# podtyazhki1337/3d-mask-r-cnn

Hardware: AMD Instinct MI355X
Metric: volumes/sec fwd+bwd @128³ & 256³, 1/2/4/8 MI355X; 3D ROIAlign GB/s vs HBM peak (higher is better)
Workload: dtype f32; 1 GPU; configs[1]: RPN training step, ResNet50-3D+FPN+RPN fwd+bwd+SGD + ProposalLayer(3D NMS 15000->6000), 128^3 x1 volume per GPU; size=128, batch_per_gpu=1, parallelism=dp1, anchors=523776, hip_graph=True

## Files before the change

### 3d-mask-r-cnn_amd/csrc/conv3d.hip

```cpp
#include "common.h"
#include <stdlib.h>

namespace m3d {

typedef float floatx16 __attribute__((ext_vector_type(16)));
typedef float floatx4 __attribute__((ext_vector_type(4)));

struct ConvP {
    const float* a;
    int B, H, W, D, C;
    int OH, OW, OD;
    int kh, kw, kd;
    int sy, sx, sz;
    int py, px, pz;
    int64_t M;
    int K;
    const float* w;
    int N;
    int flip;
    int64_t bsa, bsw, bsy;
    int dly = 1, dlx = 1, dlz = 1;
    int nbatch = 1;
    const float* halo = nullptr;
    int hnlo = 0, hdl = 0, hr = 0;
// ... 691 lines not shown
                            const float4 o = pf ? pre[u] : ld4(e.y + m * e.ldy + n);
                            t.x += o.x; t.y += o.y; t.z += o.z; t.w += o.w;
                        }
                        epi_bnbwd4(e, m, n, t, fy4[u], fz4[u], fbn4, fs);
                    } else if (pf) {
                        epi_store4_pre(p, e, m, n, v, pre[u]);
                    } else {
                        epi_store4(p, e, m, n, v);
                    }
                }
            }
        }
        e.y = y_next;
    }
    if constexpr (FBN) {
        if (e.fpart) {
            __syncthreads();
            float* red = Ts;
#pragma unroll
            for (int a = 0; a < 3; ++a)
#pragma unroll
                for (int q = 0; q < 4; ++q) red[tid * 12 + a * 4 + q] = fs[a][q];
            __syncthreads();
            if (tid < C4T) {
                float r[12];
#pragma unroll
                for (int k = 0; k < 12; ++k) r[k] = red[tid * 12 + k];
                for (int o = tid + C4T; o < 256; o += C4T)
#pragma unroll
                    for (int k = 0; k < 12; ++k) r[k] += red[o * 12 + k];
                const int n = n0c + tid * 4;
                const int64_t row = m0c / BM;
                if (n < p.N)
#pragma unroll
                    for (int a = 0; a < 3; ++a)
                        st4(e.fpart + ((int64_t)a * e.fprows + row) * p.N + n,
                            make_float4(r[a * 4], r[a * 4 + 1], r[a * 4 + 2], r[a * 4 + 3]));
            }
        }
    }
    if (!more) break;
    L = Ln;
    __syncthreads();
    store_tile(0);
    __syncthreads();
    }
}

struct WgOut {
    float* part;
    int64_t pstride;
    int plain;
    int store;
};

__device__ __forceinline__ void wg_put(const WgOut& o, float* C, float* P, int64_t idx, float v) {
    if (P) P[idx] = v;
    else if (o.store) C[idx] = v;
    else if (o.plain) C[idx] += v;
    else unsafeAtomicAdd(C + idx, v);
}

__global__ __launch_bounds__(256) void wg_reduce_kernel(const float* __restrict__ part, int splits,
                                                        int64_t pstride, int64_t kn, int64_t bsc,
                                                        float* __restrict__ C) {
    const int64_t i = (int64_t)blockIdx.x * 256 + threadIdx.x;
    if (i >= pstride) return;
    float s = part[i];
    for (int q = 1; q < splits; ++q) s += part[q * pstride + i];
    const int64_t b = i / kn, r = i - b * kn;
    C[b * bsc + r] += s;
}

static WgOut wg_out(int64_t& splits, int64_t nbatch, int64_t K, int64_t N) {
    WgOut o{nullptr, 0, 0, 0};
    const DetState d = det();
    if (!d.on) return o;
    const int64_t per = nbatch * K * N;
    const int64_t fit = (int64_t)(d.bytes / sizeof(float)) / per;
    if (splits <= 1 || fit < 2) {
        splits = 1;
        o.plain = 1;
        return o;
    }
    if (splits > fit) splits = fit;
    o.part = static_cast<float*>(d.scratch);
    o.pstride = per;
    return o;
}

static void wg_finish(const WgOut& o, int64_t splits, int64_t nbatch, int64_t K, int64_t N, int64_t bsc,
                      float* C, hipStream_t s) {
    if (!o.part) return;
    hipLaunchKernelGGL(wg_reduce_kernel, dim3(grid_for(o.pstride, 256)), dim3(256), 0, s, o.part, (int)splits,
                       o.pstride, K * N, nbatch > 1 ? bsc : K * N, C);
}

static hipError_t wg_settle(WgOut& o, int64_t splits, bool fresh, float* C, int64_t nbatch, int64_t K, int64_t N,
                            hipStream_t s) {
    if (!fresh) return hipSuccess;
    if (splits == 1 && !o.part) {
        o.store = 1;
        return hipSuccess;
    }
    return hipMemsetAsync(C, 0, sizeof(float) * (size_t)(nbatch * K * N), s);
}

template <int BI, int BJ, int WI, int WJ, bool AVEC, bool HALO = false>
__global__ __launch_bounds__(256, 2) void conv_wgrad_kernel(ConvP p, const float* __restrict__ dz,
                                                            float* __restrict__ dw,
                                                            int64_t m_per_split, WgOut wo) {
    constexpr int BKM = 32;
    constexpr int TI = BI / (WI * 32), TJ = BJ / (WJ * 32);
    static_assert(WI * WJ == 4, "4 waves");
    constexpr int X_SZ = BKM * BI, G_SZ = BKM * BJ;
    constexpr int XQ = AVEC ? BI / 32 : BI / 8;
    constexpr int GQ = BJ / 32;
    __shared__ __attribute__((aligned(16))) float smem[2 * (X_SZ + G_SZ)];

    const int tid = threadIdx.x, lane = tid & 63, wave = tid >> 6;
    const int wi = wave / WJ, wj = wave % WJ;
    const int64_t gxy = (int64_t)gridDim.x * gridDim.y;
    const int64_t total = gxy * gridDim.z;
    const int64_t Lb = blockIdx.x + (int64_t)gridDim.x * (blockIdx.y + (int64_t)gridDim.y * blockIdx.z);
    const int64_t xcd = Lb % 8, q8 = total / 8, r8 = total % 8;
    const int64_t Lt = (xcd < r8 ? xcd * (q8 + 1) : r8 * (q8 + 1) + (xcd - r8) * q8) + Lb / 8;
    const int bz_ = (int)(Lt / gxy), rem = (int)(Lt % gxy);
    const int k0 = (rem % gridDim.x) * BI;
    const int n0 = (rem / gridDim.x) * BJ;
    const int64_t nsplit = (p.M + m_per_split - 1) / m_per_split;
    const int64_t batch = bz_ / nsplit;
    float* const wp = wo.part ? wo.part + (bz_ % nsplit) * wo.pstride + batch * (int64_t)p.K * p.N : nullptr;
    if (batch) {
        p.a += batch * p.bsa;
        dz += batch * p.bsw;
        dw += batch * p.bsy;
    }
    const int64_t ms = (int64_t)(bz_ % nsplit) * m_per_split;
    int64_t me = ms + m_per_split;
    if (me > p.M) me = p.M;
    if (ms >= me) return;
    const int taps_kd = p.kd, taps_kwkd = p.kw * p.kd;

    constexpr int XC = AVEC ? BI / 4 : BI;
    const int xcol = tid % XC;
    const int xrow0 = tid / XC;
    constexpr int XRSTEP = 256 / XC;
    const int kcol = k0 + (AVEC ? xcol * 4 : xcol);
// ... 201 lines not shown
        return;
    }
    hipLaunchKernelGGL((conv_gemm_kernel<BM, BN, WM, WN, BT, AVEC, BK, 2>), grid, dim3(256), 0, s, p, e);
}

template <bool BT, bool AVEC>
static void dispatch_gemm(const ConvP& p, const Epi& e, hipStream_t s, int nbatch = 1) {
    if (p.N <= 32) {
        launch_gemm<128, 32, 4, 1, BT, AVEC, 32>(p, e, s, nbatch);
    } else if (p.N <= 64) {
        launch_gemm<128, 64, 4, 1, BT, AVEC, 32>(p, e, s, nbatch);
    } else {
        const int64_t blocks128 = ((p.M + 127) / 128) * ((p.N + 127) / 128) * nbatch;
        if (blocks128 < 512) launch_gemm<64, 128, 2, 2, BT, AVEC, 32>(p, e, s, nbatch);
        else launch_gemm<128, 128, 2, 2, BT, AVEC, 32>(p, e, s, nbatch);
    }
}

static int wgrad_minm_env() {
    static constexpr int v = M3D_TUNE_WGRAD_MINM;
    return v;
}

template <int BI, int BJ, int WI, int WJ, bool AVEC, bool HALO = false>
static int launch_wgrad(const ConvP& p, const float* dz, float* dw, hipStream_t s, int nbatch = 1,
                        bool fresh = false) {
    const int64_t tiles = (int64_t)((p.K + BI - 1) / BI) * ((p.N + BJ - 1) / BJ) * nbatch;
    int64_t splits = (1024 + tiles - 1) / tiles;
    int64_t minm = wgrad_minm_env() > 32 ? wgrad_minm_env() : 32;
    const int64_t max_splits = (p.M + minm - 1) / minm;
    if (splits > max_splits) splits = max_splits;
    if (splits < 1) splits = 1;
    WgOut wo = wg_out(splits, nbatch, p.K, p.N);
    int64_t mper = (p.M + splits - 1) / splits;
    mper = (mper + 31) / 32 * 32;
    splits = (p.M + mper - 1) / mper;
    const hipError_t fe = wg_settle(wo, splits, fresh, dw, nbatch, p.K, p.N, s);
    if (fe != hipSuccess) return (int)fe;
    dim3 grid((unsigned)((p.K + BI - 1) / BI), (unsigned)((p.N + BJ - 1) / BJ),
              (unsigned)(splits * nbatch));
    hipLaunchKernelGGL((conv_wgrad_kernel<BI, BJ, WI, WJ, AVEC, HALO>), grid, dim3(256), 0, s, p, dz, dw,
                       mper, wo);
    wg_finish(wo, splits, nbatch, p.K, p.N, p.bsy, dw, s);
    return 0;
}


template <int OCC>
__global__ __launch_bounds__(256, OCC) void x3_wgrad_kernel(const float* __restrict__ A,
                                                            const float* __restrict__ Bm,
                                                            float* __restrict__ C, int64_t M, int K, int N,
                                                            int64_t m_per_split, int64_t bsa, int64_t bsb,
                                                            int64_t bsc, WgOut wo) {
    constexpr int BI = 128, BJ = 128, TI = 2, TJ = 2, BKM = 32;
    constexpr int PL = 128 * BKM * 2;
    __shared__ __attribute__((aligned(16))) char smem[6 * PL];
    const int tid = threadIdx.x, lane = tid & 63, wave = tid >> 6;
    const int wi = wave >> 1, wj = wave & 1, h = lane >> 5, l32 = lane & 31;
    const int64_t gxy = (int64_t)gridDim.x * gridDim.y;
    const int64_t total = gxy * gridDim.z;
    const int64_t Lb = blockIdx.x + (int64_t)gridDim.x * (blockIdx.y + (int64_t)gridDim.y * blockIdx.z);
    const int64_t xcd = Lb % 8, q8 = total / 8, r8 = total % 8;
    const int64_t Lt = (xcd < r8 ? xcd * (q8 + 1) : r8 * (q8 + 1) + (xcd - r8) * q8) + Lb / 8;
    const int bz = (int)(Lt / gxy), rem = (int)(Lt % gxy);
    const int k0 = (rem % gridDim.x) * BI;
    const int n0 = (rem / gridDim.x) * BJ;
    const int64_t nsplit = (M + m_per_split - 1) / m_per_split;
    const int64_t batch = bz / nsplit;
    float* const wp = wo.part ? wo.part + (bz % nsplit) * wo.pstride + batch * (int64_t)K * N : nullptr;
    A += batch * bsa;
    Bm += batch * bsb;
    C += batch * bsc;
    const int64_t ms = (int64_t)(bz % nsplit) * m_per_split;
    const int64_t me = ms + m_per_split < M ? ms + m_per_split : M;
    if (ms >= me) return;
    const bool isB = __builtin_amdgcn_readfirstlane(tid) >= 128;
    const int lt = tid & 127, c4 = lt & 31, grp = lt >> 5;
    const int ld = isB ? N : K;
    const int col = (isB ? n0 : k0) + c4 * 4;
    const bool colok = col < ld;
    const __amdgpu_buffer_rsrc_t rs = make_rsrc(isB ? (const void*)Bm : (const void*)A, (uint64_t)M * ld * 4);
    char* const Pb = smem + (isB ? 3 * PL : 0);
    float4 v[8];
    auto load = [&](int64_t mb) {
#pragma unroll
        for (int r = 0; r < 8; ++r) {
            const int64_t m = mb + grp * 8 + r;
            v[r] = bload4(rs, (colok && m < me) ? (uint32_t)(m * ld + col) * 4u : M3D_OOB);
        }
    };
    auto store = [&]() {
#pragma unroll
        for (int c = 0; c < 4; ++c) {
            uint32_t hh[8], mm[8], ll[8];
#pragma unroll
            for (int r = 0; r < 8; ++r) split3(f4get(v[r], c), hh[r], mm[r], ll[r]);
            const int off = x3_off(c4 * 4 + c, grp * 8);
            *reinterpret_cast<uint4*>(Pb + off) =
                make_uint4(hh[0] | (hh[1] << 16), hh[2] | (hh[3] << 16), hh[4] | (hh[5] << 16), hh[6] | (hh[7] << 16));
            *reinterpret_cast<uint4*>(Pb + PL + off) =
                make_uint4(mm[0] | (mm[1] << 16), mm[2] | (mm[3] << 16), mm[4] | (mm[5] << 16), mm[6] | (mm[7] << 16));
            *reinterpret_cast<uint4*>(Pb + 2 * PL + off) =
                make_uint4(ll[0] | (ll[1] << 16), ll[2] | (ll[3] << 16), ll[4] | (ll[5] << 16), ll[6] | (ll[7] << 16));
        }
    };
    floatx16 acc[TI][TJ];
// ... 4 lines not shown
#pragma unroll
            for (int r = 0; r < 16; ++r) acc[i][j][r] = 0.0f;
    const char* const As = smem;
    const char* const Bs = smem + 3 * PL;
    const int nchunks = (int)((me - ms + BKM - 1) / BKM);
    load(ms);
    store();
    __syncthreads();
    for (int t = 0; t < nchunks; ++t) {
        if (t + 1 < nchunks) load(ms + (int64_t)(t + 1) * BKM);
#pragma unroll 2
        for (int s16 = 0; s16 < 2; ++s16) {
            bf16x8 af[TI][3], bfr[TJ][3];
#pragma unroll
            for (int i = 0; i < TI; ++i) {
                const int off = x3_off(wi * TI * 32 + i * 32 + l32, 16 * s16 + 8 * h);
#pragma unroll
                for (int pl = 0; pl < 3; ++pl) af[i][pl] = *reinterpret_cast<const bf16x8*>(As + pl * PL + off);
            }
#pragma unroll
            for (int j = 0; j < TJ; ++j) {
                const int off = x3_off(wj * TJ * 32 + j * 32 + l32, 16 * s16 + 8 * h);
#pragma unroll
                for (int pl = 0; pl < 3; ++pl) bfr[j][pl] = *reinterpret_cast<const bf16x8*>(Bs + pl * PL + off);
            }
            x3_mac_tiles<TI, TJ>(acc, af, bfr);
        }
        __syncthreads();
        if (t + 1 < nchunks) {
            store();
            __syncthreads();
        }
    }
#pragma unroll
    for (int i = 0; i < TI; ++i)
#pragma unroll
        for (int j = 0; j < TJ; ++j) {
            const int n = n0 + wj * TJ * 32 + j * 32 + l32;
            if (n >= N) continue;
#pragma unroll
            for (int r = 0; r < 16; ++r) {
                const int k = k0 + wi * TI * 32 + i * 32 + (r & 3) + 8 * (r >> 2) + 4 * h;
                if (k < K) wg_put(wo, C, wp, (int64_t)k * N + n, acc[i][j][r]);
            }
        }
}

template <int OCC>
__global__ __launch_bounds__(256, OCC) void x3_wgrad64_kernel(const float* __restrict__ A,
                                                              const float* __restrict__ Bm,
                                                              float* __restrict__ C, int64_t M, int K, int N,
                                                              int64_t m_per_split, int64_t bsa, int64_t bsb,
                                                              int64_t bsc, WgOut wo) {
    constexpr int TI = 2, TJ = 2, BKM = 64;
    constexpr int SUB = 64 * 64;
    constexpr int PL = 2 * SUB;
    constexpr int RED = 4 * 64 * 64 * 4;
    constexpr int SMEM = RED > 6 * PL ? RED : 6 * PL;
    __shared__ __attribute__((aligned(16))) char smem[SMEM];
    const int tid = threadIdx.x, lane = tid & 63, wave = tid >> 6, h = lane >> 5, l32 = lane & 31;
    const int64_t total = gridDim.x;
    const int64_t Lb = blockIdx.x;
    const int64_t xcd = Lb % 8, q8 = total / 8, r8 = total % 8;
    const int64_t Lt = (xcd < r8 ? xcd * (q8 + 1) : r8 * (q8 + 1) + (xcd - r8) * q8) + Lb / 8;
    const int tk = (K + 63) / 64, tiles = tk * ((N + 63) / 64);
    const int tile = (int)(Lt % tiles);
    const int k0 = (tile % tk) * 64, n0 = (tile / tk) * 64;
    const int64_t bz = Lt / tiles;
    const int64_t nsplit = (M + m_per_split - 1) / m_per_split;
    const int64_t batch = bz / nsplit;
    float* const wp = wo.part ? wo.part + (bz % nsplit) * wo.pstride + batch * (int64_t)K * N : nullptr;
    A += batch * bsa;
    Bm += batch * bsb;
    C += batch * bsc;
    const int64_t ms = (bz % nsplit) * m_per_split;
    const int64_t me = ms + m_per_split < M ? ms + m_per_split : M;
    if (ms >= me) return;
    const bool isB = __builtin_amdgcn_readfirstlane(tid) >= 128;
    const int lt = tid & 127, c4 = lt & 15, grp = lt >> 4;
    const int ld = isB ? N : K;
    const int col = (isB ? n0 : k0) + c4 * 4;
    const bool colok = col < ld;
    const __amdgpu_buffer_rsrc_t rs = make_rsrc(isB ? (const void*)Bm : (const void*)A, (uint64_t)M * ld * 4);
    char* const Pb = smem + (isB ? 3 * PL : 0);
    const int soff = (grp >> 2) * SUB;
    const int lrow = c4 * 4;
    float4 v[8];
    auto load = [&](int64_t mb) {
#pragma unroll
        for (int r = 0; r < 8; ++r) {
            const int64_t m = mb + grp * 8 + r;
            v[r] = bload4(rs, (colok && m < me) ? (uint32_t)(m * ld + col) * 4u : M3D_OOB);
        }
    };
    auto store = [&]() {
#pragma unroll
        for (int c = 0; c < 4; ++c) {
            uint32_t hh[8], mm[8], ll[8];
#pragma unroll
            for (int r = 0; r < 8; ++r) split3(f4get(v[r], c), hh[r], mm[r], ll[r]);
            const int off = soff + x3_off(lrow + c, (grp & 3) * 8);
            *reinterpret_cast<uint4*>(Pb + off) =
                make_uint4(hh[0] | (hh[1] << 16), hh[2] | (hh[3] << 16), hh[4] | (hh[5] << 16), hh[6] | (hh[7] << 16));
            *reinterpret_cast<uint4*>(Pb + PL + off) =
                make_uint4(mm[0] | (mm[1] << 16), mm[2] | (mm[3] << 16), mm[4] | (mm[5] << 16), mm[6] | (mm[7] << 16));
            *reinterpret_cast<uint4*>(Pb + 2 * PL + off) =
// ... 150 lines not shown
            if (DBG == 2 || DBG == 5) {
#pragma unroll
                for (int j = 0; j < 2; ++j)
                    acc[i][j][0] += (float)(af[0][0] ^ af[1][1] ^ af[2][2] ^ bfr[j][0][3] ^ bfr[j][1][4] ^ bfr[j][2][5]);
                continue;
            }
            x3_mac_pair(acc[i][0], acc[i][1], af[0], af[1], af[2], bfr[0][0], bfr[0][1], bfr[0][2],
                                  bfr[1][0], bfr[1][1], bfr[1][2]);
        }
    };
    float4 xa[2], xb[2], ya[2], yb[2];
    load(0, xa, xb);
    split_store(0, xa, xb);
    load(1, xa, xb);
    __syncthreads();
    for (int kt = 0; kt < nk; kt += 2) {
        load(kt + 2, ya, yb);
        __builtin_amdgcn_sched_barrier(0);
        mfma_step(kt);
        split_store((kt + 1) & 1, xa, xb);
        __syncthreads();
        load(kt + 3, xa, xb);
        __builtin_amdgcn_sched_barrier(0);
        mfma_step(kt + 1);
        split_store(kt & 1, ya, yb);
        __syncthreads();
    }
#pragma unroll
    for (int i = 0; i < 4; ++i)
#pragma unroll
        for (int j = 0; j < 2; ++j) {
            const int n = n0 + wn * 64 + j * 32 + l32;
            if (n >= N) continue;
#pragma unroll
            for (int r = 0; r < 16; ++r) {
                const int k = k0 + wk * 128 + i * 32 + (r & 3) + 8 * (r >> 2) + 4 * h;
                if (k < K) wg_put(wo, C, wp, (int64_t)k * N + n, acc[i][j][r]);
            }
        }
}

struct X3wSK {
    int64_t units = 0;
    int nk = 0, tk = 0, tn = 0;
};

template <int DBG, bool SK = false>
__global__ __launch_bounds__(512, 1) void x3_wgrad_tr_kernel(const float* __restrict__ A,
                                                             const float* __restrict__ Bm,
                                                             float* __restrict__ C, int64_t M, int K,
                                                             int N, int64_t m_per_split, int64_t bsa,
                                                             int64_t bsb, int64_t bsc, WgOut wo, X3wSK sk) {
    __shared__ __attribute__((aligned(16))) char smem[2 * W2_STAGE];
    if constexpr (SK) {
        const int64_t G = gridDim.x, L = blockIdx.x;
        const int64_t xcd = L % 8, q8 = G / 8, r8 = G % 8;
        const int64_t g = (xcd < r8 ? xcd * (q8 + 1) : r8 * (q8 + 1) + (xcd - r8) * q8) + L / 8;
        const int64_t Gg = G / sk.tn, grp = g / sk.tn;
        const int nj = (int)(g - grp * sk.tn);
        const int64_t ug = sk.units / sk.tn;
        int64_t u = grp * ug / Gg;
        const int64_t ue = (grp + 1) * ug / Gg;
        while (u < ue) {
            const int64_t t = u / sk.nk;
            const int64_t s0 = u - t * sk.nk;
            const int64_t s1 = s0 + (ue - u) < sk.nk ? s0 + (ue - u) : sk.nk;
            const int64_t batch = t / sk.tk;
            const int kt = (int)(t - batch * sk.tk);
            const int64_t me = s1 * W2_BK < M ? s1 * W2_BK : M;
            x3w_segment<DBG>(smem, A + batch * bsa, Bm + batch * bsb, C + batch * bsc, M, K, N, s0 * W2_BK, me,
                             kt * 256, nj * 256, wo, nullptr, 0);
            u += s1 - s0;
        }
        return;
    }
    const int64_t gxy = (int64_t)gridDim.x * gridDim.y;
    const int64_t total = gxy * gridDim.z;
    const int64_t Lb = blockIdx.x + (int64_t)gridDim.x * (blockIdx.y + (int64_t)gridDim.y * blockIdx.z);
    const int64_t xcd = Lb % 8, q8 = total / 8, r8 = total % 8;
    const int64_t Lt = (xcd < r8 ? xcd * (q8 + 1) : r8 * (q8 + 1) + (xcd - r8) * q8) + Lb / 8;
    const int bz = (int)(Lt / gxy), rem = (int)(Lt % gxy);
    const int k0 = (rem % gridDim.x) * 256;
    const int n0 = (rem / gridDim.x) * 256;
    const int64_t nsplit = (M + m_per_split - 1) / m_per_split;
    const int64_t batch = bz / nsplit;
    float* const wp = wo.part ? wo.part + (bz % nsplit) * wo.pstride + batch * (int64_t)K * N : nullptr;
    const int64_t ms = (int64_t)(bz % nsplit) * m_per_split;
    const int64_t me = ms + m_per_split < M ? ms + m_per_split : M;
    x3w_segment<DBG>(smem, A + batch * bsa, Bm + batch * bsb, C + batch * bsc, M, K, N, ms, me, k0, n0, wo, wp, bz);
}

static int wgrad_tr_env() {
    static constexpr int v = M3D_TUNE_X3W_TR;
    return v;
}

static int launch_wgrad_tr(const float* A, const float* Bm, float* C, int64_t M, int K, int N, int nbatch,
                           int64_t bsa, int64_t bsb, int64_t bsc, hipStream_t s, bool fresh) {
    const int64_t tiles = (int64_t)((K + 255) / 256) * ((N + 255) / 256) * nbatch;
    const int64_t cus = num_cus();
    static constexpr int64_t minm = M3D_TUNE_X3W_TR_MINM;
    if (M3D_TUNE_X3W_SK && !det().on && M >= (int64_t)M3D_TUNE_X3W_SK_MIN_STEPS * W2_BK) {
        X3wSK sk{};
        sk.nk = (int)((M + W2_BK - 1) / W2_BK);
        sk.tk = (K + 255) / 256;
        sk.tn = (N + 255) / 256;
        sk.units = tiles * sk.nk;
        const int64_t min_steps = (minm + W2_BK - 1) / W2_BK;
        int64_t G = (sk.units + min_steps - 1) / min_steps;
        if (G > cus) G = cus;
        G = G / sk.tn * sk.tn;
        if (G < sk.tn) G = sk.tn;
        WgOut wo{nullptr, 0, 0, 0};
        const hipError_t fe = wg_settle(wo, 2, fresh, C, nbatch, K, N, s);
        if (fe != hipSuccess) return (int)fe;
        hipLaunchKernelGGL((x3_wgrad_tr_kernel<0, true>), dim3((unsigned)G), dim3(512), 0, s, A, Bm, C, M, K, N,
                           (int64_t)0, bsa, bsb, bsc, wo, sk);
        return 0;
    }
    int64_t splits = (cus + tiles - 1) / tiles;
    const int64_t max_splits = (M + minm - 1) / minm;
    if (splits > max_splits) splits = max_splits;
    if (splits < 1) splits = 1;
    WgOut wo = wg_out(splits, nbatch, K, N);
    int64_t mper = (M + splits - 1) / splits;
    mper = (mper + W2_BK - 1) / W2_BK * W2_BK;
    splits = (M + mper - 1) / mper;
    const hipError_t fe = wg_settle(wo, splits, fresh, C, nbatch, K, N, s);
    if (fe != hipSuccess) return (int)fe;
    dim3 grid((unsigned)((K + 255) / 256), (unsigned)((N + 255) / 256), (unsigned)(splits * nbatch));
    hipLaunchKernelGGL(x3_wgrad_tr_kernel<0>, grid, dim3(512), 0, s, A, Bm, C, M, K, N, mper, bsa, bsb, bsc, wo,
                       X3wSK{});
    wg_finish(wo, splits, nbatch, K, N, bsc, C, s);
    return 0;
}

static int wgrad_x3_env() { return (x3_mask() >> 2) & 1; }

static int launch_wgrad_x3(const float* A, const float* Bm, float* C, int64_t M, int K, int N, int nbatch,
                           int64_t bsa, int64_t bsb, int64_t bsc, hipStream_t s, bool fresh = false) {
    if (wgrad_tr_env() && K >= 192 && N >= 192)
        return launch_wgrad_tr(A, Bm, C, M, K, N, nbatch, bsa, bsb, bsc, s, fresh);
    if (K <= 64 || N <= 64) {
        const int64_t tiles = (int64_t)((K + 63) / 64) * ((N + 63) / 64);
        int64_t splits = (1024 + tiles * nbatch - 1) / (tiles * nbatch);
        const int64_t minm = wgrad_minm_env() > 64 ? wgrad_minm_env() : 64;
        const int64_t max_splits = (M + minm - 1) / minm;
        if (splits > max_splits) splits = max_splits;
        if (splits < 1) splits = 1;
        WgOut wo = wg_out(splits, nbatch, K, N);
        int64_t mper = (M + splits - 1) / splits;
        mper = (mper + 63) / 64 * 64;
        splits = (M + mper - 1) / mper;
        const hipError_t fe = wg_settle(wo, splits, fresh, C, nbatch, K, N, s);
        if (fe != hipSuccess) return (int)fe;
        hipLaunchKernelGGL((x3_wgrad64_kernel<2>), dim3((unsigned)(tiles * splits * nbatch)), dim3(256), 0, s, A, Bm, C, M,
                           K, N, mper, bsa, bsb, bsc, wo);
        wg_finish(wo, splits, nbatch, K, N, bsc, C, s);
        return 0;
    }
    const int64_t tiles = (int64_t)((K + 127) / 128) * ((N + 127) / 128) * nbatch;
    int64_t splits = (1024 + tiles - 1) / tiles;
    const int64_t minm = wgrad_minm_env() > 32 ? wgrad_minm_env() : 32;
    const int64_t max_splits = (M + minm - 1) / minm;
    if (splits > max_splits) splits = max_splits;
    if (splits < 1) splits = 1;
    WgOut wo = wg_out(splits, nbatch, K, N);
    int64_t mper = (M + splits - 1) / splits;
    mper = (mper + 31) / 32 * 32;
    splits = (M + mper - 1) / mper;
    const hipError_t fe = wg_settle(wo, splits, fresh, C, nbatch, K, N, s);
    if (fe != hipSuccess) return (int)fe;
    dim3 grid((unsigned)((K + 127) / 128), (unsigned)((N + 127) / 128), (unsigned)(splits * nbatch));
    hipLaunchKernelGGL((x3_wgrad_kernel<2>), grid, dim3(256), 0, s, A, Bm, C, M, K, N, mper, bsa, bsb, bsc, wo);
    wg_finish(wo, splits, nbatch, K, N, bsc, C, s);
    return 0;
}

struct WinoGeom {
    int B, H, W, D, Din, pz, TY, TX, TZ;
    int64_t T;
    const float* halo;
    int hlo, hhi;
    int tz_mode;
    int xcd;
};

__device__ __forceinline__ int64_t wino_block(const WinoGeom& g) {
    const unsigned nb = gridDim.x, b = blockIdx.x;
    if (g.xcd && (nb & 7u) == 0) return (int64_t)(b & 7u) * (nb >> 3) + (b >> 3);
    return b;
}

__device__ __forceinline__ void bt4(float& a0, float& a1, float& a2, float& a3) {
    const float t0 = a0 - a2, t1 = a1 + a2, t2 = a2 - a1, t3 = a1 - a3;
    a0 = t0; a1 = t1; a2 = t2; a3 = t3;
}
__device__ __forceinline__ void g3(float g0, float g1, float g2, float* o) {
    o[0] = g0;
    o[1] = (g0 + g1 + g2) * 0.5f;
    o[2] = (g0 - g1 + g2) * 0.5f;
    o[3] = g2;
}
__device__ __forceinline__ void at4(float m0, float m1, float m2, float m3, float& o0, float& o1) {
    o0 = m0 + m1 + m2;
    o1 = m1 - m2 - m3;
}
__device__ __forceinline__ void a4(float e0, float e1, float* o) {
    o[0] = e0; o[1] = e0 + e1; o[2] = e0 - e1; o[3] = -e1;
}
__device__ __forceinline__ void gt4(float v0, float v1, float v2, float v3, float* o) {
    o[0] = v0 + (v1 + v2) * 0.5f;
    o[1] = (v1 - v2) * 0.5f;
    o[2] = (v1 + v2) * 0.5f + v3;
}

__device__ __forceinline__ void wino_st(float* p, float v) {
    __builtin_nontemporal_store(v, p);
}
__device__ __forceinline__ float wino_ld(const float* p) {
    return __builtin_nontemporal_load(p);
}

template <int NZ> struct ZT;
template <> struct ZT<2> {
    static constexpr int P = 4;
    __device__ static void bt(float* d) { bt4(d[0], d[1], d[2], d[3]); }
    __device__ static void g(const float* w, float* o) { g3(w[0], w[1], w[2], o); }
    __device__ static void at(const float* m, float* o) { at4(m[0], m[1], m[2], m[3], o[0], o[1]); }
    __device__ static void a(const float* e, float* o) { a4(e[0], e[1], o); }
    __device__ static void gt(const float* v, float* o) { gt4(v[0], v[1], v[2], v[3], o); }
};
template <> struct ZT<4> {
    static constexpr int P = 6;
    __device__ static void bt(float* d) {
        const float d0 = d[0], d1 = d[1], d2 = d[2], d3 = d[3], d4 = d[4], d5 = d[5];
        d[0] = d0 * 0.25f - d2 * 1.25f + d4;
        d[1] = -(d1 + d2) * 0.25f + d3 + d4;
// ... 2 lines not shown
        d[4] = d1 * 0.5f - d2 - d3 * 0.5f + d4;
        d[5] = d1 * 0.25f - d3 * 1.25f + d5;
    }
    __device__ static void g(const float* w, float* o) {
        const float c23 = 2.0f / 3.0f;
        o[0] = 4.0f * w[0];
        o[1] = c23 * (w[0] + w[1] + w[2]);
        o[2] = c23 * (w[0] - w[1] + w[2]);
        o[3] = -(8.0f / 3.0f) * w[0] - (4.0f / 3.0f) * w[1] - c23 * w[2];
        o[4] = -(8.0f / 3.0f) * w[0] + (4.0f / 3.0f) * w[1] - c23 * w[2];
        o[5] = w[2];
    }
    __device__ static void at(const float* m, float* o) {
        const float s12 = m[1] + m[2], d12 = m[1] - m[2], s34 = m[3] + m[4], d34 = m[3] - m[4];
        o[0] = m[0] + s12 + s34;
        o[1] = d12 + d34 * 0.5f;
        o[2] = s12 + s34 * 0.25f;
        o[3] = d12 + d34 * 0.125f + m[5];
    }
    __device__ static void a(const float* e, float* o) {
        o[0] = e[0];
        o[1] = e[0] + e[1] + e[2] + e[3];
        o[2] = e[0] - e[1] + e[2] - e[3];
        o[3] = e[0] + e[1] * 0.5f + e[2] * 0.25f + e[3] * 0.125f;
        o[4] = e[0] - e[1] * 0.5f + e[2] * 0.25f - e[3] * 0.125f;
        o[5] = e[3];
    }
    __device__ static void gt(const float* v, float* o) {
        const float c23 = 2.0f / 3.0f;
        o[0] = 4.0f * v[0] + c23 * (v[1] + v[2]) - (8.0f / 3.0f) * (v[3] + v[4]);
        o[1] = c23 * (v[1] - v[2]) - (4.0f / 3.0f) * (v[3] - v[4]);
        o[2] = c23 * (v[1] + v[2]) - c23 * (v[3] + v[4]) + v[5];
    }
};

constexpr int WNY = M3D_TUNE_WINO_NY;
using YT = ZT<WNY>;
constexpr int PY = YT::P;

__device__ __forceinline__ void tile_coords(int64_t t, const WinoGeom& g, int& b, int& ty, int& tx,
                                            int& tz) {
    tz = (int)(t % g.TZ);
    int64_t r = t / g.TZ;
    tx = (int)(r % g.TX);
    r /= g.TX;
    ty = (int)(r % g.TY);
    b = (int)(r / g.TY);
}

template <int NZ, bool X3O = false, bool HALO = false, int NYT = WNY>
__global__ __launch_bounds__(256) void wino_input_kernel(const float* __restrict__ x, WinoGeom g,
                                                         int C, float* __restrict__ U) {
    constexpr int P = ZT<NZ>::P, PYt = ZT<NYT>::P;
    const int64_t i = wino_block(g) * blockDim.x + threadIdx.x;
    if (i >= g.T * C) return;
    const int c = (int)(i % C);
    const int64_t t = i / C;
    int b, ty, tx, tz;
    tile_coords(t, g, b, ty, tx, tz);
    if (g.tz_mode) {
        const bool edge = tz == 0 || tz == g.TZ - 1;
        if ((g.tz_mode == 1) == edge) return;
    }
    float d[PYt][4][P];
    const __amdgpu_buffer_rsrc_t rs = make_rsrc(x, (uint64_t)g.B * g.H * g.W * g.Din * C * 4);
    __amdgpu_buffer_rsrc_t rh;
    if constexpr (HALO) rh = make_rsrc(g.halo, (uint64_t)g.B * g.H * g.W * 2 * C * 4);
#pragma unroll
    for (int a = 0; a < PYt; ++a) {
        const int y = NYT * ty - 1 + a;
#pragma unroll
        for (int bb = 0; bb < 4; ++bb) {
            const int xx = 2 * tx - 1 + bb;
            const bool ok = (unsigned)y < (unsigned)g.H && (unsigned)xx < (unsigned)g.W;
            const uint32_t row = (uint32_t)((((b * g.H + y) * g.W + xx) * g.Din) * C + c);
#pragma unroll
            for (int k = 0; k < P; ++k) {
                const int z = NZ * tz - g.pz + k;
                const bool in = ok && (unsigned)z < (unsigned)g.Din;
                d[a][bb][k] = __builtin_bit_cast(
                    float, __builtin_amdgcn_raw_buffer_load_b32(rs, in ? (row + (uint32_t)z * C) * 4u : M3D_OOB, 0, 0));
                if constexpr (HALO) {
                    if (k == 0 || k == P - 1) {
                        const int q = z < 0 ? 0 : 1;
                        const bool hz = ok && ((z == -1 && g.hlo) || (z == g.Din && g.hhi));
                        const uint32_t hoff = (uint32_t)((((b * g.H + y) * g.W + xx) * 2 + q) * C + c) * 4u;
                        const float hv = __builtin_bit_cast(
                            float, __builtin_amdgcn_raw_buffer_load_b32(rh, hz ? hoff : M3D_OOB, 0, 0));
                        d[a][bb][k] = hz ? hv : d[a][bb][k];
                    }
                }
            }
        }
    }
#pragma unroll
    for (int a = 0; a < PYt; ++a)
#pragma unroll
        for (int bb = 0; bb < 4; ++bb) ZT<NZ>::bt(d[a][bb]);
#pragma unroll
    for (int a = 0; a < PYt; ++a)
#pragma unroll
        for (int k = 0; k < P; ++k) bt4(d[a][0][k], d[a][1][k], d[a][2][k], d[a][3][k]);
#pragma unroll
    for (int bb = 0; bb < 4; ++bb)
#pragma unroll
        for (int k = 0; k < P; ++k) {
// ... 78 lines not shown
#pragma unroll
        for (int b = 0; b < 3; ++b) ZT<NZ>::g(gw[a][b], t1[a][b]);
    float t2[3][4][P];
#pragma unroll
    for (int a = 0; a < 3; ++a)
#pragma unroll
        for (int k = 0; k < P; ++k) {
            float o[4];
            g3(t1[a][0][k], t1[a][1][k], t1[a][2][k], o);
#pragma unroll
            for (int b = 0; b < 4; ++b) t2[a][b][k] = o[b];
        }
    if constexpr (X3O) {
        unsigned short* out = reinterpret_cast<unsigned short*>(V) + (int64_t)np_ * (KN / Np) + kp;
        const int64_t pstride = (int64_t)PYt * 4 * P * KN;
#pragma unroll
        for (int b = 0; b < 4; ++b)
#pragma unroll
            for (int k = 0; k < P; ++k) {
                float o[PYt];
                const float gy[3] = {t2[0][b][k], t2[1][b][k], t2[2][b][k]};
                ZT<NYT>::g(gy, o);
#pragma unroll
                for (int a = 0; a < PYt; ++a) {
                    uint32_t hh, mm, ll;
                    split3(o[a], hh, mm, ll);
                    unsigned short* q = out + (int64_t)((a * 4 + b) * P + k) * KN;
                    q[0] = (unsigned short)hh;
                    q[pstride] = (unsigned short)mm;
                    q[2 * pstride] = (unsigned short)ll;
                }
            }
        return;
    }
    float* out = V + (int64_t)kp * Np + np_;
#pragma unroll
    for (int b = 0; b < 4; ++b)
#pragma unroll
        for (int k = 0; k < P; ++k) {
            float o[PYt];
            const float gy[3] = {t2[0][b][k], t2[1][b][k], t2[2][b][k]};
            ZT<NYT>::g(gy, o);
#pragma unroll
            for (int a = 0; a < PYt; ++a) out[(int64_t)((a * 4 + b) * P + k) * KN] = o[a];
        }
}

template <int NZ, bool HALO, int NYT>
__device__ __forceinline__ void wino_output_body(const float* __restrict__ Mt, const WinoGeom& g,
                                                 int N, const Epi& e);
template <int NZ, int NYT = WNY>
__global__ __launch_bounds__(256) void wino_output_kernel(const float* __restrict__ Mt, WinoGeom g,
                                                          int N, Epi e) {
    wino_output_body<NZ, false, NYT>(Mt, g, N, e);
}
template <int NZ, int NYT = WNY>
__global__ __launch_bounds__(256) void wino_output_halo_kernel(const float* __restrict__ Mt, WinoGeom g,
                                                               int N, Epi e) {
    wino_output_body<NZ, true, NYT>(Mt, g, N, e);
}

template <int NZ, bool HALO, int NYT>
__device__ __forceinline__ void wino_output_body(const float* __restrict__ Mt, const WinoGeom& g,
                                                 int N, const Epi& e) {
    constexpr int P = ZT<NZ>::P, PYt = ZT<NYT>::P;
    const int64_t i = wino_block(g) * blockDim.x + threadIdx.x;
    if (i >= g.T * N) return;
    const int n = (int)(i % N);
    const int64_t t = i / N;
    int b, ty, tx, tz;
    tile_coords(t, g, b, ty, tx, tz);
    const int64_t stride = g.T * N;
    const float* src = Mt + t * N + n;
    float m[PYt][4][P];
#pragma unroll
    for (int a = 0; a < PYt; ++a)
#pragma unroll
        for (int bb = 0; bb < 4; ++bb)
#pragma unroll
            for (int k = 0; k < P; ++k) m[a][bb][k] = wino_ld(src + (int64_t)((a * 4 + bb) * P + k) * stride);
    float r1[PYt][4][NZ];
#pragma unroll
    for (int a = 0; a < PYt; ++a)
#pragma unroll
        for (int bb = 0; bb < 4; ++bb) ZT<NZ>::at(m[a][bb], r1[a][bb]);
    float r2[PYt][2][NZ];
#pragma unroll
    for (int a = 0; a < PYt; ++a)
#pragma unroll
        for (int k = 0; k < NZ; ++k)
            at4(r1[a][0][k], r1[a][1][k], r1[a][2][k], r1[a][3][k], r2[a][0][k], r2[a][1][k]);
    float o[NYT][2][NZ];
#pragma unroll
    for (int bb = 0; bb < 2; ++bb)
#pragma unroll
        for (int k = 0; k < NZ; ++k) {
            float col[PYt], oy[NYT];
#pragma unroll
            for (int a = 0; a < PYt; ++a) col[a] = r2[a][bb][k];
            ZT<NYT>::at(col, oy);
#pragma unroll
            for (int a = 0; a < NYT; ++a) o[a][bb][k] = oy[a];
        }
    const float bias = e.bias ? e.bias[n] : 0.0f;
    const float sc = e.scale ? e.scale[n] : 1.0f, sh = e.scale ? e.shift[n] : 0.0f;
#pragma unroll
// ... 98 lines not shown
                    yv[bb][k] = in[bb][k] && e.frelu ? e.fy[off] : 1.0f;
                    zv[bb][k] = in[bb][k] && e.fz ? e.fz[off] : 0.0f;
                }
#pragma unroll
            for (int bb = 0; bb < 2; ++bb)
#pragma unroll
                for (int k = 0; k < NZ; ++k) {
                    if (!in[bb][k]) continue;
                    const int64_t off = obase + (a * (int64_t)g.W + bb) * ostr + k * e.ldy;
                    float gv = o[a][bb][k];
                    if (e.accumulate) gv += ov[bb][k];
                    if (e.frelu && !(yv[bb][k] > 0.f)) gv = 0.f;
                    const float d = gv * sc;
                    sp += gv;
                    sx += gv * ((zv[bb][k] - mu) * rs);
                    sz += d;
                    e.y[off] = d;
                    if (e.fdres) e.fdres[off] = gv;
                }
        }
    }
    if (!e.fpart) return;
    if (N % 256 == 0) {
        if (valid) {
            e.fpart[(0 * e.fprows + t) * N + n] = sp;
            e.fpart[(1 * e.fprows + t) * N + n] = sx;
            e.fpart[(2 * e.fprows + t) * N + n] = sz;
        }
        return;
    }
    __shared__ float red[3][256];
    red[0][tid] = sp;
    red[1][tid] = sx;
    red[2][tid] = sz;
    __syncthreads();
    if (tid < N) {
        float a0 = 0.f, a1 = 0.f, a2 = 0.f;
        for (int q = tid; q < 256; q += N) {
            a0 += red[0][q];
            a1 += red[1][q];
            a2 += red[2][q];
        }
        const int64_t row = blockIdx.x;
        e.fpart[(0 * e.fprows + row) * N + tid] = a0;
        e.fpart[(1 * e.fprows + row) * N + tid] = a1;
        e.fpart[(2 * e.fprows + row) * N + tid] = a2;
    }
}

template <int NZ>
__global__ __launch_bounds__(256) void wino_grad_kernel(const float* __restrict__ dz, WinoGeom g,
                                                        int N, float* __restrict__ DY) {
    constexpr int P = ZT<NZ>::P;
    const int64_t i = (int64_t)blockIdx.x * blockDim.x + threadIdx.x;
    if (i >= g.T * N) return;
    const int n = (int)(i % N);
    const int64_t t = i / N;
    int b, ty, tx, tz;
    tile_coords(t, g, b, ty, tx, tz);
    float ev[WNY][2][NZ];
#pragma unroll
    for (int a = 0; a < WNY; ++a)
#pragma unroll
        for (int bb = 0; bb < 2; ++bb)
#pragma unroll
            for (int k = 0; k < NZ; ++k) {
                const int y = WNY * ty + a, xx = 2 * tx + bb, z = NZ * tz + k;
                ev[a][bb][k] = (y < g.H && xx < g.W && z < g.D)
                                   ? dz[((((int64_t)b * g.H + y) * g.W + xx) * g.D + z) * N + n]
                                   : 0.0f;
            }
    float t1[WNY][2][P];
#pragma unroll
    for (int a = 0; a < WNY; ++a)
#pragma unroll
        for (int bb = 0; bb < 2; ++bb) ZT<NZ>::a(ev[a][bb], t1[a][bb]);
    float t2[WNY][4][P];
#pragma unroll
    for (int a = 0; a < WNY; ++a)
#pragma unroll
        for (int k = 0; k < P; ++k) {
            float o[4];
            a4(t1[a][0][k], t1[a][1][k], o);
#pragma unroll
            for (int bb = 0; bb < 4; ++bb) t2[a][bb][k] = o[bb];
        }
    const int64_t stride = g.T * N;
    float* out = DY + t * N + n;
#pragma unroll
    for (int bb = 0; bb < 4; ++bb)
#pragma unroll
        for (int k = 0; k < P; ++k) {
            float ey[WNY], o[PY];
#pragma unroll
            for (int a = 0; a < WNY; ++a) ey[a] = t2[a][bb][k];
            YT::a(ey, o);
#pragma unroll
            for (int a = 0; a < PY; ++a) wino_st(out + (int64_t)((a * 4 + bb) * P + k) * stride, o[a]);
        }
}

template <int NZ>
__global__ __launch_bounds__(256) void wino_wgrad_out_kernel(const float* __restrict__ dWh, int C,
                                                             int N, float* __restrict__ dw) {
    constexpr int P = ZT<NZ>::P;
    const int64_t i = (int64_t)blockIdx.x * blockDim.x + threadIdx.x;
    const int64_t CN = (int64_t)C * N;
    if (i >= CN) return;
    float v[PY][4][P];
#pragma unroll
    for (int a = 0; a < PY; ++a)
#pragma unroll
        for (int b = 0; b < 4; ++b)
#pragma unroll
            for (int k = 0; k < P; ++k) v[a][b][k] = dWh[(int64_t)((a * 4 + b) * P + k) * CN + i];
    float t1[PY][4][3];
#pragma unroll
    for (int a = 0; a < PY; ++a)
#pragma unroll
        for (int b = 0; b < 4; ++b) ZT<NZ>::gt(v[a][b], t1[a][b]);
    float t2[PY][3][3];
#pragma unroll
    for (int a = 0; a < PY; ++a)
#pragma unroll
        for (int k = 0; k < 3; ++k) {
            float o[3];
            gt4(t1[a][0][k], t1[a][1][k], t1[a][2][k], t1[a][3][k], o);
#pragma unroll
            for (int b = 0; b < 3; ++b) t2[a][b][k] = o[b];
        }
#pragma unroll
    for (int b = 0; b < 3; ++b)
#pragma unroll
        for (int k = 0; k < 3; ++k) {
            float vy[PY], o[3];
#pragma unroll
            for (int a = 0; a < PY; ++a) vy[a] = t2[a][b][k];
            YT::gt(vy, o);
#pragma unroll
            for (int a = 0; a < 3; ++a) dw[(int64_t)((a * 3 + b) * 3 + k) * CN + i] += o[a];
        }
}

struct X3Epi {
    const float* bias = nullptr;
    const float* scale = nullptr;
    const float* shift = nullptr;
    const float* res = nullptr;
    float* z = nullptr;
    int act = 0;
    int on = 0;
    const float* fy = nullptr;
    const float* fz = nullptr;
    const float* fscale = nullptr;
    const float* fmean = nullptr;
    const float* frstd = nullptr;
    float* fdres = nullptr;
    float* fpart = nullptr;
    int64_t fprows = 0;
    int frelu = 0;
    int facc = 0;
};

struct X3G {
    const unsigned short* a = nullptr;
    const float* af = nullptr;
    const unsigned short* b = nullptr;
    float* c = nullptr;
    int64_t M = 0;
    int K = 0, N = 0, nbatch = 0;
    int64_t psa = 0, psb = 0;
    int64_t bsa = 0, bsb = 0, bsc = 0;
    X3Epi ep = {};
};

__device__ __forceinline__ int x3_off16(int row, int kc) {
    return row * 32 + (((kc ^ (row >> 3)) & 1) << 4);
}

template <int BK>
__device__ __forceinline__ int x3_soff(int row, int kc) {
    if constexpr (BK == 16) return x3_off16(row, kc);
    else return x3_off(row, kc * 8);
}

template <int BK, bool PERSIST, int OCC = (BK == 16 ? 3 : 2), bool AF32 = false, int BNT = 128>
__global__ __launch_bounds__(256, OCC) void x3_gemm_kernel(X3G g) {
    static_assert(BK == 16 || BK == 32, "BK");
    static_assert(BNT == 128 || BNT == 64, "BNT");
    constexpr int BM = 128, BN = BNT, TM = 2, TN = BNT / 64;
    constexpr int NBUF = BK == 16 ? 2 : 1;
    constexpr int KCH = BK / 8, CPT = BM * KCH / 256;
    constexpr int CPTB = BN * KCH / 256;
    constexpr int PLA = BM * BK * 2, PLB = BN * BK * 2;
    constexpr int STAGE = 3 * (PLA + PLB);
    constexpr int LDT = BN + 8, HR = 64;
    static_assert(HR * LDT * 4 <= NBUF * STAGE, "staging fits");
    __shared__ __attribute__((aligned(16))) char smem[NBUF * STAGE];
    const int tid = threadIdx.x, lane = tid & 63, wave = tid >> 6;
    const int wm = wave >> 1, wn = wave & 1, h = lane >> 5, l32 = lane & 31;
    const int64_t nbx = (g.M + BM - 1) / BM, nby = (g.N + BN - 1) / BN;
    const int64_t per_batch = nbx * nby, total = per_batch * g.nbatch;
    int64_t L = PERSIST ? (int64_t)blockIdx.x : (int64_t)blockIdx.x + (int64_t)gridDim.x * blockIdx.y;
    const int64_t Lstep = PERSIST ? (int64_t)gridDim.x : total;
    const int nk = g.K / BK;
    float* const Ts = reinterpret_cast<float*>(smem);
    int soff[CPT];
    uint32_t lrow[CPT];
#pragma unroll
    for (int u = 0; u < CPT; ++u) {
        const int c = tid + 256 * u;
        soff[u] = x3_soff<BK>(c / KCH, c % KCH);
    }
    for (; L < total; L += Lstep) {
        const int64_t xcd = L % 8, q8 = total / 8, r8 = total % 8;
        const int64_t T = (xcd < r8 ? xcd * (q8 + 1) : r8 * (q8 + 1) + (xcd - r8) * q8) + L / 8;
        const int64_t bz = T / per_batch, Tt = T - bz * per_batch;
        const int64_t m0 = (Tt / nby) * BM;
        const int n0 = (int)(Tt % nby) * BN;
        __amdgpu_buffer_rsrc_t ra[3], rb[3];
#pragma unroll
        for (int pl = 0; pl < 3; ++pl) {
            if constexpr (AF32) {
                if (pl == 0) ra[0] = make_rsrc(g.af + bz * g.bsa + m0 * g.K, (uint64_t)(g.M - m0) * g.K * 4);
            } else {
                ra[pl] = make_rsrc(g.a + pl * g.psa + bz * g.bsa + m0 * g.K, (uint64_t)(g.M - m0) * g.K * 2);
            }
            rb[pl] = make_rsrc(g.b + pl * g.psb + bz * g.bsb + (int64_t)n0 * g.K, (uint64_t)(g.N - n0) * g.K * 2);
        }
#pragma unroll
        for (int u = 0; u < CPT; ++u) {
            const int c = tid + 256 * u;
            lrow[u] = (uint32_t)((c / KCH) * g.K + (c % KCH) * 8) * 2u;
        }
        uint4 va[AF32 ? 1 : 3][CPT], vb[3][CPTB];
        float4 fa[AF32 ? CPT : 1][2];
        auto load = [&](int kt) {
#pragma unroll
            for (int q = 0; q < 3; ++q)
#pragma unroll
                for (int u = 0; u < CPT; ++u) {
                    const int off = (int)(lrow[u] + (uint32_t)kt * (BK * 2));
                    if constexpr (AF32) {
                        if (q == 0) {
                            fa[u][0] = bload4(ra[0], (uint32_t)off * 2u);
                            fa[u][1] = bload4(ra[0], (uint32_t)off * 2u + 16u);
                        }
                    } else {
                        va[q][u] = __builtin_bit_cast(uint4, __builtin_amdgcn_raw_buffer_load_b128(ra[q], off, 0, 0));
                    }
                    if (u < CPTB)
                        vb[q][u] = __builtin_bit_cast(uint4, __builtin_amdgcn_raw_buffer_load_b128(rb[q], off, 0, 0));
                }
        };
        auto store = [&](int buf) {
            char* As = smem + buf * STAGE;
            char* Bs = As + 3 * PLA;
#pragma unroll
            for (int u = 0; u < CPT; ++u) {
                if constexpr (AF32) {
                    uint2 lo4[3], hi4[3];
                    split3x4(fa[u][0], lo4);
                    split3x4(fa[u][1], hi4);
#pragma unroll
                    for (int q = 0; q < 3; ++q)
                        *reinterpret_cast<uint4*>(As + q * PLA + soff[u]) =
                            make_uint4(lo4[q].x, lo4[q].y, hi4[q].x, hi4[q].y);
                } else {
#pragma unroll
                    for (int q = 0; q < 3; ++q) *reinterpret_cast<uint4*>(As + q * PLA + soff[u]) = va[q][u];
                }
                if (u < CPTB) {
// ... 41 lines not shown
                if (kt + 1 < nk) {
                    store(0);
                    __syncthreads();
                }
            }
        }
        float* const cb = g.c + bz * g.bsc;
        for (int hf = 0; hf < 2; ++hf) {
            if (hf) __syncthreads();
            if (wm == hf) {
#pragma unroll
                for (int i = 0; i < TM; ++i)
#pragma unroll
                    for (int j = 0; j < TN; ++j)
#pragma unroll
                        for (int r = 0; r < 16; ++r)
                            Ts[(i * 32 + (r & 3) + 8 * (r >> 2) + 4 * h) * LDT + wn * TN * 32 + j * 32 + l32] =
                                acc[i][j][r];
            }
            __syncthreads();
#pragma unroll
            for (int q = 0; q < HR * (BN / 4) / 256; ++q) {
                const int idx = tid + 256 * q;
                const int row = idx / (BN / 4), c4 = idx % (BN / 4);
                const int64_t m = m0 + hf * HR + row;
                const int n = n0 + c4 * 4;
                if (m < g.M && n < g.N)
                    st4(cb + m * g.N + n, *reinterpret_cast<const float4*>(Ts + row * LDT + c4 * 4));
            }
        }
        __syncthreads();
    }
}

constexpr int G2_BK = 16;
constexpr int G2_PL = 256 * G2_BK * 2;
constexpr int G2_STAGE = 6 * G2_PL;
constexpr int G2_NST = 3;

__device__ __forceinline__ void g2_dma(__amdgpu_buffer_rsrc_t r, char* lds, uint32_t voff) {
    __builtin_amdgcn_raw_ptr_buffer_load_lds(r, (__attribute__((address_space(3))) void*)lds, 16, (int)voff,
                                             0, 0, 0);
}

template <int DBG>
__global__ __launch_bounds__(512, 1) void x3_gemm256_kernel(X3G g) {
    __shared__ __attribute__((aligned(16))) char smem[G2_NST * G2_STAGE];
    const int tid = threadIdx.x, lane = tid & 63, wave = tid >> 6;
    const int wm = wave >> 2, wn = wave & 3, h = lane >> 5, l32 = lane & 31;
    const int64_t nbx = (g.M + 255) / 256, nby = g.N / 256;
    const int64_t per_batch = nbx * nby, total = per_batch * g.nbatch;
    const int64_t L = (int64_t)blockIdx.x + (int64_t)gridDim.x * blockIdx.y;
    if (L >= total) return;
    const int64_t xcd = L % 8, q8 = total / 8, r8 = total % 8;
    const int64_t T = (xcd < r8 ? xcd * (q8 + 1) : r8 * (q8 + 1) + (xcd - r8) * q8) + L / 8;
    const int64_t bz = T / per_batch, Tt = T - bz * per_batch;
    const int64_t m0 = (Tt / nby) * 256;
    const int64_t n0 = (Tt % nby) * 256;
    __amdgpu_buffer_rsrc_t rs[6];
#pragma unroll
    for (int pl = 0; pl < 3; ++pl) {
        rs[pl] = make_rsrc(g.a + pl * g.psa + bz * g.bsa + m0 * g.K, (uint64_t)(g.M - m0) * g.K * 2);
        rs[3 + pl] = make_rsrc(g.b + pl * g.psb + bz * g.bsb + n0 * g.K, (uint64_t)256 * g.K * 2);
    }
    const int lrow = 32 * wave + (lane >> 1);
    const uint32_t lsrc = (uint32_t)lrow * (uint32_t)g.K * 2u + (uint32_t)(((lane & 1) ^ ((lrow >> 3) & 1)) << 4);
    const int nk = g.K / G2_BK;
    auto issue = [&](int kt) {
        char* S = smem + (kt % G2_NST) * G2_STAGE + wave * 1024;
        const uint32_t off = lsrc + (uint32_t)kt * (G2_BK * 2);
        if (DBG == 3) return;
#pragma unroll
        for (int pl = 0; pl < 6; ++pl) g2_dma(rs[pl], S + pl * G2_PL, off);
    };
    floatx16 acc[4][2];
#pragma unroll
    for (int i = 0; i < 4; ++i)
#pragma unroll
        for (int j = 0; j < 2; ++j)
#pragma unroll
            for (int r = 0; r < 16; ++r) acc[i][j][r] = 0.0f;
    issue(0);
    if (nk > 1) issue(1);
    for (int kt = 0; kt < nk; ++kt) {
        if (kt + 1 < nk) asm volatile("s_waitcnt vmcnt(6)" ::: "memory");
        else asm volatile("s_waitcnt vmcnt(0)" ::: "memory");
        __builtin_amdgcn_s_barrier();
        if (kt + 2 < nk) issue(kt + 2);
        const char* S = smem + (kt % G2_NST) * G2_STAGE;
        bf16x8 bfr[2][3];
#pragma unroll
        for (int j = 0; j < 2; ++j) {
            const int off = x3_off16(wn * 64 + j * 32 + l32, h);
#pragma unroll
            for (int pl = 0; pl < 3; ++pl)
                bfr[j][pl] = *reinterpret_cast<const bf16x8*>(S + (3 + pl) * G2_PL + off);
        }
#pragma unroll
        for (int i = 0; i < 4; ++i) {
            const int off = x3_off16(wm * 128 + i * 32 + l32, h);
            bf16x8 af[3];
#pragma unroll
            for (int pl = 0; pl < 3; ++pl) af[pl] = *reinterpret_cast<const bf16x8*>(S + pl * G2_PL + off);
            if (DBG == 2 || DBG == 4) {
#pragma unroll
                for (int j = 0; j < 2; ++j)
                    acc[i][j][0] += (float)(af[0][0] ^ af[1][1] ^ af[2][2] ^ bfr[j][0][3] ^ bfr[j][1][4] ^ bfr[j][2][5]);
                continue;
            }
            x3_mac_pair(acc[i][0], acc[i][1], af[0], af[1], af[2], bfr[0][0], bfr[0][1], bfr[0][2],
                                    bfr[1][0], bfr[1][1], bfr[1][2]);
// ... 4 lines not shown
#pragma unroll
        for (int i = 0; i < 4; ++i)
#pragma unroll
            for (int j = 0; j < 2; ++j)
#pragma unroll
                for (int r = 0; r < 16; ++r) t += acc[i][j][r];
        if (t == 1.2345f) g.c[0] = t;
        return;
    }
    const __amdgpu_buffer_rsrc_t rc = make_rsrc(g.c + bz * g.bsc + m0 * g.N, (uint64_t)(g.M - m0) * g.N * 4);
#pragma unroll
    for (int i = 0; i < 4; ++i)
#pragma unroll
        for (int j = 0; j < 2; ++j) {
            const int col = (int)n0 + wn * 64 + j * 32 + l32;
#pragma unroll
            for (int r = 0; r < 16; ++r) {
                const int row = wm * 128 + i * 32 + (r & 3) + 8 * (r >> 2) + 4 * h;
                const float v = acc[i][j][r];
                __builtin_amdgcn_raw_buffer_store_b32(__float_as_uint(v), rc,
                                                      (int)(((uint32_t)row * (uint32_t)g.N + (uint32_t)col) * 4u),
                                                      0, 0);
            }
        }
}

template <int N_> struct IC { static constexpr int v = N_; };
template <int EPI>
#ifndef M3D_X3AF_STAMP
#define M3D_X3AF_STAMP 0
#endif
__global__ __launch_bounds__(512, 1) void x3_gemm256_af_kernel(X3G g) {
#if M3D_X3AF_STAMP
    __shared__ __attribute__((aligned(16))) char sAll[18 * G2_PL + 256];
    uint32_t* const stampbuf = reinterpret_cast<uint32_t*>(sAll + 18 * G2_PL);
    char* const sA0 = sAll;
    char* const sA1 = sAll + 3 * G2_PL;
    char* const sA2 = sAll + 6 * G2_PL;
    char* const sB0 = sAll + 9 * G2_PL;
    char* const sB1 = sAll + 12 * G2_PL;
    char* const sB2 = sAll + 15 * G2_PL;
    const uint32_t st_t0 = (uint32_t)__builtin_amdgcn_s_memtime();
    const uint32_t st_r0 = (uint32_t)__builtin_amdgcn_s_memrealtime();
#else
    __shared__ __attribute__((aligned(16))) char sA0[3 * G2_PL], sA1[3 * G2_PL], sA2[3 * G2_PL];
    __shared__ __attribute__((aligned(16))) char sB0[3 * G2_PL], sB1[3 * G2_PL], sB2[3 * G2_PL];
#endif
    const int tid = threadIdx.x, lane = tid & 63, wave = tid >> 6;
    const int wm = wave >> 2, wn = wave & 3, h = lane >> 5, l32 = lane & 31;
    const int64_t nbx = (g.M + 255) / 256, nby = g.N / 256;
    const int64_t per_batch = nbx * nby, total = per_batch * g.nbatch;
    const int64_t L = (int64_t)blockIdx.x + (int64_t)gridDim.x * blockIdx.y;
    if (L >= total) return;
    const int64_t xcd = L % 8, q8 = total / 8, r8 = total % 8;
    const int64_t T = (xcd < r8 ? xcd * (q8 + 1) : r8 * (q8 + 1) + (xcd - r8) * q8) + L / 8;
    const int64_t bz = T / per_batch, Tt = T - bz * per_batch;
    const int64_t m0 = (Tt / nby) * 256;
    const int64_t n0 = (Tt % nby) * 256;
    const int nk = g.K / G2_BK;
    const __amdgpu_buffer_rsrc_t ra = make_rsrc(g.af + bz * g.bsa + m0 * g.K, (uint64_t)(g.M - m0) * g.K * 4);
    const int arow = tid >> 1, ach = tid & 1;
    const uint32_t aoff0 = ((uint32_t)arow * (uint32_t)g.K + (uint32_t)ach * 8u) * 4u;
    const int awr = x3_off16(arow, ach);
    __amdgpu_buffer_rsrc_t rb[3];
#pragma unroll
    for (int pl = 0; pl < 3; ++pl)
        rb[pl] = make_rsrc(g.b + pl * g.psb + bz * g.bsb + n0 * g.K, (uint64_t)256 * g.K * 2);
    const int lrow = 32 * wave + (lane >> 1);
    const uint32_t lsrc = (uint32_t)lrow * (uint32_t)g.K * 2u + (uint32_t)(((lane & 1) ^ ((lrow >> 3) & 1)) << 4);
    auto stA = [&](auto st) -> char* {
        if constexpr (decltype(st)::v == 0) return sA0;
        else if constexpr (decltype(st)::v == 1) return sA1;
        else return sA2;
    };
    auto stB = [&](auto st) -> char* {
        if constexpr (decltype(st)::v == 0) return sB0;
        else if constexpr (decltype(st)::v == 1) return sB1;
        else return sB2;
    };
    using AReg = float4;
    auto load_a = [&](int kt, float4 (&v)[2]) {
        const bool in = kt < nk;
        const uint32_t o = aoff0 + (uint32_t)kt * (G2_BK * 4);
        v[0] = bload4(ra, in ? o : M3D_OOB);
        v[1] = bload4(ra, in ? o + 16u : M3D_OOB);
    };
    auto dma_b = [&](auto st, int kt) {
        char* S = stB(st) + wave * 1024;
        const uint32_t off = kt < nk ? lsrc + (uint32_t)kt * (G2_BK * 2) : M3D_OOB;
#pragma unroll
        for (int pl = 0; pl < 3; ++pl) g2_dma(rb[pl], S + pl * G2_PL, off);
    };
    auto split_a = [&](auto st, const AReg (&v)[2]) {
        char* S = stA(st) + awr;
        uint2 lo4[3], hi4[3];
        split3x4(make_float4(v[0][0], v[0][1], v[0][2], v[0][3]), lo4);
        split3x4(make_float4(v[1][0], v[1][1], v[1][2], v[1][3]), hi4);
#pragma unroll
        for (int q = 0; q < 3; ++q)
            *reinterpret_cast<uint4*>(S + q * G2_PL) = make_uint4(lo4[q].x, lo4[q].y, hi4[q].x, hi4[q].y);
    };
    floatx16 acc[4][2];
#pragma unroll
    for (int i = 0; i < 4; ++i)
#pragma unroll
        for (int j = 0; j < 2; ++j)
#pragma unroll
            for (int r = 0; r < 16; ++r) acc[i][j][r] = 0.0f;
    AReg xa[2], ya[2], za[2];
    load_a(0, xa);
    load_a(1, ya);
// ... 1105 lines not shown
                                          int64_t OH, int64_t OW, int64_t OD, int32_t sy, int32_t sx, int32_t sz,
                                          int32_t py, int32_t px, int32_t pz, float* dw, const m3d_det_t* det, m3d_stream_t s) {
    M3D_DET_SCOPE(det);
    int rc = conv_check(B, H, W, Dl, Cin, kh, kw, kd, Cout, OH, OW, OD, sy, sx, sz);
    if (rc) return rc;
    if (B * H * W * (Dl + 2 * r) * Cin >= op_lim() || B * OH * OW * OD * Cout >= op_lim())
        return einval("conv3d_bwd_weight_halo: operand larger than 4 GiB (32-bit buffer offsets)");
    ConvP p{x, (int)B, (int)H, (int)W, (int)Dl, (int)Cin, (int)OH, (int)OW, (int)OD, kh, kw, kd,
            sy, sx, sz, py, px, pz, B * OH * OW * OD, (int)(kh * kw * kd * Cin), nullptr,
            (int)Cout, 0, 0, 0, 0};
    if ((rc = conv_halo_geom(p, halo, has_lo, has_hi, r, Dl, kd, sz, pz, OD))) return rc;
    if (stem_ok(Cin, kh, kw, kd, Cout, sy, sx, sz, 1, 1, 1, 0, 0, 0))
        return launch_stem_wgrad(p, dz, dw, st(s));
    const bool vec = (Cin % 4) == 0;
    if (Cout <= 64) {
        if (vec) launch_wgrad<128, 64, 2, 2, true, true>(p, dz, dw, st(s));
        else launch_wgrad<128, 64, 2, 2, false, true>(p, dz, dw, st(s));
    } else {
        if (vec) launch_wgrad<128, 128, 2, 2, true, true>(p, dz, dw, st(s));
        else launch_wgrad<128, 128, 2, 2, false, true>(p, dz, dw, st(s));
    }
    return check_launch("conv_wgrad_kernel<halo>");
}

static int wino_check(int64_t B, int64_t H, int64_t W, int64_t D, int64_t OD, int32_t pz,
                      int64_t Cin, int64_t Cout) {
    if (B <= 0 || H <= 0 || W <= 0 || D <= 0 || OD <= 0 || Cin <= 0 || Cout <= 0)
        return einval("conv3d winograd: tensor dimensions must be positive");
    if (Cin % 32 || Cout % 32) return einval("conv3d winograd: Cin and Cout must be multiples of 32");
    if (pz < 0 || pz > 1 || D - OD < 0 || D - OD > 2)
        return einval("conv3d winograd: z geometry must be pz in {0,1} and 0 <= D - OD <= 2");
    if (H * W * (D > OD ? D : OD) > 0x7FFFFFFF) return einval("conv3d winograd: more than 2^31 voxels");
    if (H * W * (D > OD ? D : OD) * (Cin > Cout ? Cin : Cout) >= op_lim())
        return einval("conv3d winograd: operand of one batch item larger than 4 GiB (32-bit buffer offsets)");
    return M3D_OK;
}

static bool wino_per_item(int64_t B, int64_t H, int64_t W, int64_t D, int64_t OD, int64_t Cin, int64_t Cout) {
    return per_item(B, H * W * (D > OD ? D : OD), Cin > Cout ? Cin : Cout, 0, 0);
}
#define WINO_LAUNCH_NZ(nz, kern, ...)                                            \
    do {                                                                         \
        if ((nz) == 4) hipLaunchKernelGGL(kern<4>, __VA_ARGS__);                 \
        else hipLaunchKernelGGL(kern<2>, __VA_ARGS__);                           \
    } while (0)
#define WINO_LAUNCH(kern, ...) WINO_LAUNCH_NZ(wino_nz(), kern, __VA_ARGS__)

extern "C" int32_t m3d_conv3d_wino_tile_z(void) { return wino_nz(); }
extern "C" int32_t m3d_conv3d_wino_wgrad_tile_z(void) { return wino_wgrad_nz(); }
extern "C" int32_t m3d_conv3d_wino_tile_y(void) { return WNY; }
extern "C" int32_t m3d_conv3d_wino_dgrad_tile_y(void) { return wino_dgrad_ny(); }
extern "C" int32_t m3d_conv3d_wino_dgrad_tile_z(void) { return wino_dgrad_nz(); }

extern "C" size_t m3d_conv3d_wino_workspace_bytes(int64_t B, int64_t H, int64_t W, int64_t D,
                                                  int64_t OD, int64_t Cin, int64_t Cout) {
    auto al = [](size_t b) { return (b + 255) & ~(size_t)255; };
    if (wino_per_item(B, H, W, D, OD, Cin, Cout)) B = 1;
    size_t best = 0;
    const int tiles[4][2] = {{wino_nz(), WNY}, {wino_wgrad_nz(), WNY}, {wino_dgrad_nz(), 2}, {wino_dgrad_nz(), 4}};
    for (const auto& zy : tiles) {
        const int nz = zy[0], ny = zy[1];
        const WinoGeom g = wino_geom(B, H, W, D > OD ? D : OD, D, 1, nz, ny);
        const size_t P = (size_t)wino_points(nz, ny);
        const size_t eb = gemm_x3_env() ? 6 : 4;
        const size_t wt = gemm_x3_env() ? al(sizeof(float) * 27 * (size_t)Cin * Cout) : 0;
        const size_t um1 = al(eb * P * (size_t)g.T * Cin) + al(4 * P * (size_t)g.T * Cout);
        const size_t um2 = al(eb * P * (size_t)g.T * Cout) + al(4 * P * (size_t)g.T * Cin);
        const size_t b = wt + al(eb * P * (size_t)Cin * Cout) + (um1 > um2 ? um1 : um2);
        best = b > best ? b : best;
    }
    return best;
}

struct WinoWs { float *V, *U, *M, *WT; };
static size_t wino_ws_need(const WinoGeom& g, int64_t C1, int64_t C2, int nz, int ny) {
    auto al = [](size_t b) { return (b + 255) & ~(size_t)255; };
    const size_t P = (size_t)wino_points(nz, ny);
    const size_t eb = gemm_x3_env() ? 6 : 4;
    const size_t wt = gemm_x3_env() ? al(sizeof(float) * 27 * (size_t)C1 * C2) : 0;
    return wt + al(eb * P * (size_t)C1 * C2) + al(eb * P * (size_t)g.T * C1) + al(4 * P * (size_t)g.T * C2);
}
extern "C" size_t m3d_conv3d_wino_dgrad_workspace_bytes(int64_t B, int64_t H, int64_t W, int64_t D, int64_t OD,
                                                        int64_t Cin, int64_t Cout, int32_t tile_y) {
    if (tile_y != 0 && tile_y != 2 && tile_y != 4) return 0;
    if (wino_per_item(B, H, W, D, OD, Cin, Cout)) B = 1;
    const int nz = wino_dgrad_nz(), ny = tile_y ? tile_y : wino_dgrad_ny();
    return wino_ws_need(wino_geom(B, H, W, D, OD, 1, nz, ny), Cout, Cin, nz, ny);
}
static WinoWs wino_ws(void* ws, const WinoGeom& g, int64_t Cin, int64_t Cout, int nz = -1, int ny = WNY) {
    auto al = [](size_t b) { return (b + 255) & ~(size_t)255; };
    const size_t P = (size_t)wino_points(nz < 0 ? wino_nz() : nz, ny);
    char* p = (char*)ws;
    WinoWs w{};
    w.WT = (float*)p;
    if (gemm_x3_env()) p += al(sizeof(float) * 27 * (size_t)Cin * Cout);
    const size_t eb = gemm_x3_env() ? 6 : 4;
    w.V = (float*)p; p += al(eb * P * (size_t)Cin * Cout);
    w.U = (float*)p; p += al(eb * P * (size_t)g.T * Cin);
    w.M = (float*)p;
    return w;
}

#define WINO_LAUNCH_NZ_X3(nz, kern, ...)                                         \
    do {                                                                         \
        if ((nz) == 4) hipLaunchKernelGGL((kern<4, true>), __VA_ARGS__);         \
        else hipLaunchKernelGGL((kern<2, true>), __VA_ARGS__);                   \
    } while (0)
#define WINO_INPUT(nz, x3o, grid, s, x, g, C, U)                                                          \
    do {                                                                                                   \
        const bool h_ = (g).halo != nullptr;                                                               \
        if ((nz) == 4) {                                                                                   \
            if (x3o) { if (h_) hipLaunchKernelGGL((wino_input_kernel<4, true, true>), grid, dim3(256), 0, s, x, g, C, U); \
                       else hipLaunchKernelGGL((wino_input_kernel<4, true, false>), grid, dim3(256), 0, s, x, g, C, U); } \
            else { if (h_) hipLaunchKernelGGL((wino_input_kernel<4, false, true>), grid, dim3(256), 0, s, x, g, C, U); \
                   else hipLaunchKernelGGL((wino_input_kernel<4, false, false>), grid, dim3(256), 0, s, x, g, C, U); } \
        } else {                                                                                           \
            if (x3o) { if (h_) hipLaunchKernelGGL((wino_input_kernel<2, true, true>), grid, dim3(256), 0, s, x, g, C, U); \
                       else hipLaunchKernelGGL((wino_input_kernel<2, true, false>), grid, dim3(256), 0, s, x, g, C, U); } \
            else { if (h_) hipLaunchKernelGGL((wino_input_kernel<2, false, true>), grid, dim3(256), 0, s, x, g, C, U); \
                   else hipLaunchKernelGGL((wino_input_kernel<2, false, false>), grid, dim3(256), 0, s, x, g, C, U); } \
        }                                                                                                  \
    } while (0)

static int x3_af32_env() { return (x3_mask() >> 4) & 1; }

static void wino_gemm_x3(const WinoWs& ws, int64_t T, int K, int N, int P, hipStream_t s,
                         bool af32 = false) {
    X3G q{};
    q.a = reinterpret_cast<const unsigned short*>(ws.U);
    q.af = ws.U;
    q.b = reinterpret_cast<const unsigned short*>(ws.V);
    q.c = ws.M;
    q.M = T; q.K = K; q.N = N; q.nbatch = P;
    q.psa = (int64_t)P * T * K; q.psb = (int64_t)P * K * N;
    q.bsa = T * K; q.bsb = (int64_t)K * N; q.bsc = T * N;
    if (N % 256 == 0 && T >= 256) {
        const int64_t t256 = ((T + 255) / 256) * (N / 256) * P;
        const dim3 grid((unsigned)(t256 < 65536 ? t256 : 65536), (unsigned)((t256 + 65535) / 65536));
        if (af32) hipLaunchKernelGGL(x3_gemm256_af_kernel<0>, grid, dim3(512), 0, s, q);
        else hipLaunchKernelGGL(x3_gemm256_kernel<0>, grid, dim3(512), 0, s, q);
        return;
    }
    if (N == 64) {
        const int64_t tiles = ((T + 127) / 128) * P;
        if (af32) hipLaunchKernelGGL((x3_gemm_kernel<32, false, 2, true, 64>), dim3((unsigned)tiles), dim3(256), 0, s, q);
        else hipLaunchKernelGGL((x3_gemm_kernel<32, false, 3, false, 64>), dim3((unsigned)tiles), dim3(256), 0, s, q);
        return;
    }
    const int64_t tiles = ((T + 127) / 128) * ((N + 127) / 128) * P;
    if (af32) hipLaunchKernelGGL((x3_gemm_kernel<32, false, 2, true>), dim3((unsigned)tiles), dim3(256), 0, s, q);
    else hipLaunchKernelGGL((x3_gemm_kernel<32, false, 3>), dim3((unsigned)tiles), dim3(256), 0, s, q);
}

__global__ __launch_bounds__(256) void split3_kernel(const float* __restrict__ x, int64_t n,
                                                     unsigned short* __restrict__ x3) {
    const int64_t i = (int64_t)blockIdx.x * blockDim.x + threadIdx.x;
    if (i >= n) return;
    uint32_t h, m, l;
    split3(x[i], h, m, l);
    x3[i] = (unsigned short)h;
    x3[n + i] = (unsigned short)m;
    x3[2 * n + i] = (unsigned short)l;
}

extern "C" int m3d_split3_f32(const float* x, int64_t n, uint16_t* x3, m3d_stream_t s) {
    if (n <= 0) return einval("split3: n must be positive");
    hipLaunchKernelGGL(split3_kernel, dim3(grid_for(n, 256)), dim3(256), 0, st(s), x, n,
                       reinterpret_cast<unsigned short*>(x3));
    return check_launch("split3_kernel");
}

extern "C" int m3d_gemm_x3(const uint16_t* A3, const uint16_t* B3, float* C, int64_t batch, int64_t M,
                           int64_t K, int64_t N, m3d_stream_t s) {
    if (batch <= 0 || M <= 0 || K <= 0 || N <= 0) return einval("gemm_x3: dimensions must be positive");
    if (K % 32 || N % 4) return einval("gemm_x3: K must be a multiple of 32 and N of 4");
    if (M > 0x7FFFFFFF || M * K * 2 >= 0xFFFFFFF0LL || N * K * 2 >= 0xFFFFFFF0LL || M * N * 4 >= 0xFFFFFFF0LL)
        return einval("gemm_x3: operand larger than 4 GiB (32-bit buffer offsets)");
    WinoWs ws{};
    ws.U = (float*)const_cast<uint16_t*>(A3);
    ws.V = (float*)const_cast<uint16_t*>(B3);
    ws.M = C;
// ... 232 lines not shown
        WINO_LAUNCH(wino_output_kernel, dim3(grid_for(g.T * Cout, 256)), dim3(256), 0, s, ws.M,
                    g, (int)Cout, o);
        return check_launch("conv3d winograd fwd (x3)");
    }
    if (u_keep) ws.U = u_keep;
    if (phase != 2)
        WINO_LAUNCH(wino_weight_kernel, dim3(grid_for(Cin * Cout, 256)), dim3(256), 0, s, w,
                           (int)Cin, (int)Cout, 0, ws.V);
    if (phase == 1) {
        WINO_INPUT(wino_nz(), false, dim3(grid_for(g.T * Cin, 256)), s, x, gi, (int)Cin, ws.U);
        return check_launch("conv3d winograd fwd (phase 1)");
    }
    WINO_INPUT(wino_nz(), false, dim3(grid_for(g.T * Cin, 256)), s, x, phase == 2 ? ge : g, (int)Cin, ws.U);
    ConvP p = wino_gemm_p(ws.U, g.T, (int)Cin, ws.V, (int)Cout);
    Epi e{};
    e.y = ws.M; e.ldy = Cout; e.simple = 1; e.YH = 1; e.YW = 1; e.YD = (int)g.T;
    e.ysy = e.ysx = e.ysz = 1;
    dispatch_gemm<false, true>(p, e, s, wino_points());
    Epi o{};
    o.bias = bias; o.scale = bn_scale; o.shift = bn_shift; o.res = residual;
    o.res_mode = residual ? 1 : 0; o.relu = relu; o.z = z_out; o.y = y; o.ldy = Cout;
    WINO_LAUNCH(wino_output_kernel, dim3(grid_for(g.T * Cout, 256)), dim3(256), 0, s, ws.M,
                       g, (int)Cout, o);
    return check_launch("conv3d winograd fwd");
}

extern "C" int m3d_conv3d_fwd_wino(const float* x, int64_t B, int64_t H, int64_t W, int64_t D,
                                   int64_t Cin, const float* w, int64_t Cout, int64_t OD,
                                   int32_t pz, const float* bias, const float* bn_scale,
                                   const float* bn_shift, const float* residual, int32_t relu,
                                   float* z_out, float* y, void* workspace, size_t ws_bytes,
                                   m3d_stream_t s) {
    return fwd_wino(x, B, H, W, D, Cin, w, Cout, OD, pz, bias, bn_scale, bn_shift, residual, relu,
                    z_out, y, nullptr, workspace, ws_bytes, st(s));
}

extern "C" int m3d_conv3d_fwd_wino_keep(const float* x, int64_t B, int64_t H, int64_t W, int64_t D,
                                        int64_t Cin, const float* w, int64_t Cout, int64_t OD,
                                        int32_t pz, const float* bias, const float* bn_scale,
                                        const float* bn_shift, const float* residual, int32_t relu,
                                        float* z_out, float* y, float* u_keep, void* workspace,
                                        size_t ws_bytes, m3d_stream_t s) {
    if (!u_keep) return einval("conv3d winograd: u_keep must not be NULL");
    if (wino_nz() != wino_wgrad_nz())
        return einval("conv3d winograd: forward and weight-gradient tiles differ (m3d_conv3d_wino_u_bytes == 0)");
    return fwd_wino(x, B, H, W, D, Cin, w, Cout, OD, pz, bias, bn_scale, bn_shift, residual, relu,
                    z_out, y, u_keep, workspace, ws_bytes, st(s));
}

static int bwd_data_wino(const float* dz, const float* w, int64_t B, int64_t H, int64_t W, int64_t D,
                         int64_t Cin, int64_t Cout, int64_t OD, int32_t pz, float* dx, int32_t accumulate,
                         void* workspace, size_t ws_bytes, hipStream_t s, float* dx_halo = nullptr,
                         int hlo = 0, bool v_ready = false, const Epi* fb = nullptr, int ny = 0,
                         const void* v_ext = nullptr);

extern "C" int m3d_conv3d_fwd_wino_v(const float* x, int64_t B, int64_t H, int64_t W, int64_t D, int64_t Cin,
                                     const float* w, int64_t Cout, int64_t OD, int32_t pz, const float* bias,
                                     const float* bn_scale, const float* bn_shift, const float* residual,
                                     int32_t relu, float* z_out, float* y, void* workspace, size_t ws_bytes,
                                     int32_t v_ready, m3d_stream_t s) {
    return fwd_wino(x, B, H, W, D, Cin, w, Cout, OD, pz, bias, bn_scale, bn_shift, residual, relu, z_out, y,
                    nullptr, workspace, ws_bytes, st(s), nullptr, 0, 0, v_ready != 0);
}
extern "C" int m3d_conv3d_bwd_data_wino_v(const float* dz, const float* w, int64_t B, int64_t H, int64_t W,
                                          int64_t D, int64_t Cin, int64_t Cout, int64_t OD, int32_t pz, float* dx,
                                          int32_t accumulate, void* workspace, size_t ws_bytes, int32_t v_ready,
                                          m3d_stream_t s) {
    return bwd_data_wino(dz, w, B, H, W, D, Cin, Cout, OD, pz, dx, accumulate, workspace, ws_bytes, st(s), nullptr,
                         0, v_ready != 0);
}

static int dgrad_tile_arg(int32_t tile_y, int& ny) {
    if (tile_y != 0 && tile_y != 2 && tile_y != 4) return einval("conv3d winograd bwd-data: tile_y must be 0, 2 or 4");
    ny = tile_y ? tile_y : wino_dgrad_ny();
    return M3D_OK;
}

extern "C" int m3d_conv3d_bwd_data_wino_vy(const float* dz, const float* w, int64_t B, int64_t H, int64_t W,
                                           int64_t D, int64_t Cin, int64_t Cout, int64_t OD, int32_t pz, float* dx,
                                           int32_t accumulate, void* workspace, size_t ws_bytes, int32_t v_ready,
                                           int32_t tile_y, m3d_stream_t s) {
    int ny;
    int rc = dgrad_tile_arg(tile_y, ny);
    if (rc) return rc;
    return bwd_data_wino(dz, w, B, H, W, D, Cin, Cout, OD, pz, dx, accumulate, workspace, ws_bytes, st(s), nullptr,
                         0, v_ready != 0, nullptr, ny);
}

extern "C" int m3d_conv3d_bwd_data_wino(const float* dz, const float* w, int64_t B, int64_t H,
                                        int64_t W, int64_t D, int64_t Cin, int64_t Cout,
                                        int64_t OD, int32_t pz, float* dx, int32_t accumulate,
                                        void* workspace, size_t ws_bytes, m3d_stream_t s) {
    return bwd_data_wino(dz, w, B, H, W, D, Cin, Cout, OD, pz, dx, accumulate, workspace, ws_bytes, st(s));
}

static int bwd_data_wino_bn(const float* dz, const float* w, int64_t B, int64_t H, int64_t W, int64_t D,
                            int64_t Cin, int64_t Cout, int64_t OD, int32_t pz, float* dx, int32_t accumulate,
                            void* workspace, size_t ws_bytes, int32_t v_ready, const m3d_bn_bwd_t* bn, void* bn_ws,
                            size_t bn_ws_bytes, int ny, hipStream_t hs, const void* v_ext = nullptr) {
    if (Cin % 256 != 0 && 256 % Cin != 0)
        return einval("conv3d winograd bwd-data (fused BN backward): Cin must divide 256 or be a multiple of it");
    if (wino_per_item(B, H, W, D, OD, Cin, Cout))
        return einval("conv3d winograd bwd-data (fused BN backward): batch past the 32-bit operand bound");
    const WinoGeom g = wino_geom(B, H, W, D, OD, 2 - pz, wino_dgrad_nz(), ny);
    const int64_t rows = Cin % 256 == 0 ? g.T : (g.T * Cin + 255) / 256;
    Epi e{};
    int rc = bn_fuse_epi(bn, Cin, bn_ws, bn_ws_bytes, rows, e);
// ... 42 lines not shown
}
extern "C" int m3d_conv3d_wino_weight_v(const float* w, int64_t Cin, int64_t Cout, int32_t dgrad, int32_t tile_y,
                                        void* v, size_t v_bytes, m3d_stream_t s) {
    int ny;
    if (Cin <= 0 || Cout <= 0) return einval("conv3d winograd: channel counts must be positive");
    if (int rc = wino_v_tile(dgrad, tile_y, ny)) return rc;
    if (!w || !v || v_bytes < m3d_conv3d_wino_v_bytes(Cin, Cout, dgrad, tile_y))
        return einval("conv3d winograd: transformed-weight buffer missing or too small (m3d_conv3d_wino_v_bytes)");
    const dim3 grid(grid_for(Cin * Cout, 256));
    if (!dgrad) {
        float* wt = reinterpret_cast<float*>(static_cast<char*>(v) + wino_v_planes_bytes(Cin, Cout, 0, ny));
        hipLaunchKernelGGL(x3_wt_kernel, dim3((unsigned)((Cout + 31) / 32), (unsigned)((Cin + 31) / 32), 27),
                           dim3(256), 0, st(s), w, (int)Cin, (int)Cout, wt);
        WINO_LAUNCH_NZ_X3(wino_nz(), wino_weight_kernel, grid, dim3(256), 0, st(s), wt, (int)Cin, (int)Cout, 0,
                          static_cast<float*>(v));
        return check_launch("conv3d winograd weight transform (fwd)");
    }
    const int nz = wino_dgrad_nz();
    float* V = static_cast<float*>(v);
    if (nz == 4 && ny == 4) hipLaunchKernelGGL((wino_weight_kernel<4, true, 4>), grid, dim3(256), 0, st(s), w, (int)Cin, (int)Cout, 1, V);
    else if (nz == 4) hipLaunchKernelGGL((wino_weight_kernel<4, true, 2>), grid, dim3(256), 0, st(s), w, (int)Cin, (int)Cout, 1, V);
    else if (ny == 4) hipLaunchKernelGGL((wino_weight_kernel<2, true, 4>), grid, dim3(256), 0, st(s), w, (int)Cin, (int)Cout, 1, V);
    else hipLaunchKernelGGL((wino_weight_kernel<2, true, 2>), grid, dim3(256), 0, st(s), w, (int)Cin, (int)Cout, 1, V);
    return check_launch("conv3d winograd weight transform (dgrad)");
}
extern "C" int m3d_conv3d_fwd_wino_kv(const float* x, int64_t B, int64_t H, int64_t W, int64_t D, int64_t Cin,
                                      const float* w, int64_t Cout, int64_t OD, int32_t pz, const float* bias,
                                      const float* bn_scale, const float* bn_shift, const float* residual,
                                      int32_t relu, float* z_out, float* y, float* u_keep, const void* v,
                                      void* workspace, size_t ws_bytes, m3d_stream_t s) {
    int ny;
    if (int rc = wino_v_tile(0, 0, ny)) return rc;
    if (!v) return einval("conv3d winograd: v must not be NULL (m3d_conv3d_wino_weight_v)");
    if (u_keep && wino_nz() != wino_wgrad_nz())
        return einval("conv3d winograd: forward and weight-gradient tiles differ (m3d_conv3d_wino_u_bytes == 0)");
    return fwd_wino(x, B, H, W, D, Cin, w, Cout, OD, pz, bias, bn_scale, bn_shift, residual, relu, z_out, y, u_keep,
                    workspace, ws_bytes, st(s), nullptr, 0, 0, false, 0, v);
}
extern "C" int m3d_conv3d_bwd_data_wino_xv(const float* dz, const float* w, int64_t B, int64_t H, int64_t W,
                                           int64_t D, int64_t Cin, int64_t Cout, int64_t OD, int32_t pz, float* dx,
                                           int32_t accumulate, void* workspace, size_t ws_bytes, const void* v,
                                           int32_t tile_y, const m3d_bn_bwd_t* bn, void* bn_ws, size_t bn_ws_bytes,
                                           m3d_stream_t s) {
    int ny;
    if (int rc = wino_v_tile(1, tile_y, ny)) return rc;
    if (!v) return einval("conv3d winograd bwd-data: v must not be NULL (m3d_conv3d_wino_weight_v)");
    if (bn)
        return bwd_data_wino_bn(dz, w, B, H, W, D, Cin, Cout, OD, pz, dx, accumulate, workspace, ws_bytes, 0, bn, bn_ws,
                                bn_ws_bytes, ny, st(s), v);
    return bwd_data_wino(dz, w, B, H, W, D, Cin, Cout, OD, pz, dx, accumulate, workspace, ws_bytes, st(s), nullptr, 0,
                         false, nullptr, ny, v);
}

template <int NZ, int NY>
static void wino_dgrad_out(const float* Mt, const WinoGeom& g, int C, float* dx, int accumulate,
                           float* dx_halo, int hlo, int dl, hipStream_t hs, const Epi* fb) {
    Epi o{};
    if (fb) o = *fb;
    o.y = dx; o.ldy = C; o.accumulate = accumulate;
    const dim3 grid(grid_for(g.T * C, 256));
    if (fb) {
        hipLaunchKernelGGL((wino_output_bn_kernel<NZ, NY>), grid, dim3(256), 0, hs, Mt, g, C, o);
        return;
    }
    if (dx_halo) {
        o.yh = dx_halo; o.hlo = hlo; o.dl = dl;
        hipLaunchKernelGGL((wino_output_halo_kernel<NZ, NY>), grid, dim3(256), 0, hs, Mt, g, C, o);
        return;
    }
    hipLaunchKernelGGL((wino_output_kernel<NZ, NY>), grid, dim3(256), 0, hs, Mt, g, C, o);
}

template <int NZ, int NY>
static void bwd_data_wino_launch(const float* dz, const float* w, const WinoGeom& g, const WinoWs& ws, int Cin,
                                 int Cout, float* dx, int32_t accumulate, float* dx_halo, int hlo, int dl,
                                 bool v_ready, const Epi* fb, hipStream_t hs) {
    const int P = wino_points(NZ, NY);
    const dim3 wgrid(grid_for((int64_t)Cin * Cout, 256)), igrid(grid_for(g.T * Cout, 256));
    if (gemm_x3_env()) {
        if (!v_ready)
            hipLaunchKernelGGL((wino_weight_kernel<NZ, true, NY>), wgrid, dim3(256), 0, hs, w, Cin, Cout, 1, ws.V);
        const bool af32 = x3_af32_env();
        if (af32)
            hipLaunchKernelGGL((wino_input_kernel<NZ, false, false, NY>), igrid, dim3(256), 0, hs, dz, g, Cout, ws.U);
        else
            hipLaunchKernelGGL((wino_input_kernel<NZ, true, false, NY>), igrid, dim3(256), 0, hs, dz, g, Cout, ws.U);
        wino_gemm_x3(ws, g.T, Cout, Cin, P, hs, af32);
    } else {
        hipLaunchKernelGGL((wino_weight_kernel<NZ, false, NY>), wgrid, dim3(256), 0, hs, w, Cin, Cout, 1, ws.V);
        hipLaunchKernelGGL((wino_input_kernel<NZ, false, false, NY>), igrid, dim3(256), 0, hs, dz, g, Cout, ws.U);
        ConvP p = wino_gemm_p(ws.U, g.T, Cout, ws.V, Cin);
        Epi e{};
        e.y = ws.M; e.ldy = Cin; e.simple = 1; e.YH = 1; e.YW = 1; e.YD = (int)g.T;
        e.ysy = e.ysx = e.ysz = 1;
        dispatch_gemm<false, true>(p, e, hs, P);
    }
    wino_dgrad_out<NZ, NY>(ws.M, g, Cin, dx, accumulate, dx_halo, hlo, dl, hs, fb);
}

static int bwd_data_wino(const float* dz, const float* w, int64_t B, int64_t H, int64_t W, int64_t D,
                         int64_t Cin, int64_t Cout, int64_t OD, int32_t pz, float* dx, int32_t accumulate,
                         void* workspace, size_t ws_bytes, hipStream_t hs, float* dx_halo, int hlo, bool v_ready,
                         const Epi* fb, int ny_arg, const void* v_ext) {
    int rc = wino_check(B, H, W, D, OD, pz, Cin, Cout);
    if (rc) return rc;
    if (wino_per_item(B, H, W, D, OD, Cin, Cout)) {
        const int64_t dxd = dx_halo ? OD : D;
        for (int64_t b = 0; b < B; ++b) {
            rc = bwd_data_wino(dz + b * H * W * OD * Cout, w, 1, H, W, D, Cin, Cout, OD, pz, dx + b * H * W * dxd * Cin,
                               accumulate, workspace, ws_bytes, hs,
                               dx_halo ? dx_halo + b * H * W * 2 * Cin : nullptr, hlo, v_ready || b > 0, nullptr,
                               ny_arg, v_ext);
            if (rc) return rc;
        }
        return M3D_OK;
    }
    const int nz = wino_dgrad_nz(), ny = ny_arg ? ny_arg : wino_dgrad_ny();
    const WinoGeom g = wino_geom(B, H, W, D, OD, 2 - pz, nz, ny);
    if (ws_bytes < wino_ws_need(g, Cout, Cin, nz, ny))
        return einval("conv3d winograd: workspace too small");
    WinoWs ws = wino_ws(workspace, g, Cout, Cin, nz, ny);
    if (v_ext) {
        ws.V = static_cast<float*>(const_cast<void*>(v_ext));
        v_ready = true;
    }
    const int ci = (int)Cin, co = (int)Cout, dl = (int)OD;
    if (nz == 4 && ny == 4)
        bwd_data_wino_launch<4, 4>(dz, w, g, ws, ci, co, dx, accumulate, dx_halo, hlo, dl, v_ready, fb, hs);
    else if (nz == 4)
        bwd_data_wino_launch<4, 2>(dz, w, g, ws, ci, co, dx, accumulate, dx_halo, hlo, dl, v_ready, fb, hs);
    else if (ny == 4)
        bwd_data_wino_launch<2, 4>(dz, w, g, ws, ci, co, dx, accumulate, dx_halo, hlo, dl, v_ready, fb, hs);
    else
        bwd_data_wino_launch<2, 2>(dz, w, g, ws, ci, co, dx, accumulate, dx_halo, hlo, dl, v_ready, fb, hs);
    return check_launch("conv3d winograd bwd-data");
}

static int bwd_weight_wino(const float* x, const float* u_in, const float* dz, int64_t B,
                           int64_t H, int64_t W, int64_t D, int64_t Cin, int64_t Cout, int64_t OD,
                           int32_t pz, float* dw, void* workspace, size_t ws_bytes, m3d_stream_t s,
                           const float* halo = nullptr, int hlo = 0, int hhi = 0) {
    int rc = wino_check(B, H, W, D, OD, pz, Cin, Cout);
    if (rc) return rc;
    if (ws_bytes < m3d_conv3d_wino_workspace_bytes(B, H, W, D, OD, Cin, Cout))
        return einval("conv3d winograd: workspace too small");
    if (wino_per_item(B, H, W, D, OD, Cin, Cout)) {
        if (u_in) return einval("conv3d winograd: kept U with a batch past the 32-bit operand bound");
        for (int64_t b = 0; b < B; ++b) {
            rc = bwd_weight_wino(x + b * H * W * D * Cin, nullptr, dz + b * H * W * OD * Cout, 1, H, W, D, Cin, Cout,
                                 OD, pz, dw, workspace, ws_bytes, s, halo ? halo + b * H * W * 2 * Cin : nullptr, hlo,
                                 hhi);
            if (rc) return rc;
        }
        return M3D_OK;
    }
    const int nz = wino_wgrad_nz();
    WinoGeom g = wino_geom(B, H, W, OD, D, pz, nz);
    g.halo = halo; g.hlo = hlo; g.hhi = hhi;
    WinoWs ws = wino_ws(workspace, g, Cin, Cout, nz);
    if (u_in)
        ws.U = const_cast<float*>(u_in);
    else
        WINO_INPUT(nz, false, dim3(grid_for(g.T * Cin, 256)), st(s), x, g, (int)Cin, ws.U);
        WINO_LAUNCH_NZ(nz, wino_grad_kernel, dim3(grid_for(g.T * Cout, 256)), dim3(256), 0, st(s), dz, g,
                       (int)Cout, ws.M);
    int fe = 0;
    if (wgrad_x3_env() && (Cout > 64 || Cin <= 64)) {
        fe = launch_wgrad_x3(ws.U, ws.M, ws.V, g.T, (int)Cin, (int)Cout, wino_points(nz), g.T * Cin, g.T * Cout,
                             (int64_t)Cin * Cout, st(s), true);
    } else {
        ConvP p = wino_gemm_p(ws.U, g.T, (int)Cin, nullptr, (int)Cout);
        p.bsw = g.T * Cout;
        p.bsy = (int64_t)Cin * Cout;
        if (Cout <= 64) fe = launch_wgrad<128, 64, 2, 2, true>(p, ws.M, ws.V, st(s), wino_points(nz), true);
        else fe = launch_wgrad<128, 128, 2, 2, true>(p, ws.M, ws.V, st(s), wino_points(nz), true);
    }
    if (fe) {
        set_error("memset dW_hat: %s", hipGetErrorString((hipError_t)fe));
        return M3D_EHIP;
    }
    WINO_LAUNCH_NZ(nz, wino_wgrad_out_kernel, dim3(grid_for(Cin * Cout, 256)), dim3(256), 0, st(s),
                       ws.V, (int)Cin, (int)Cout, dw);
    return check_launch("conv3d winograd bwd-weight");
}

extern "C" int m3d_conv3d_bwd_weight_wino(const float* x, const float* dz, int64_t B, int64_t H,
                                          int64_t W, int64_t D, int64_t Cin, int64_t Cout,
                                          int64_t OD, int32_t pz, float* dw, void* workspace,
                                          size_t ws_bytes, const m3d_det_t* det, m3d_stream_t s) {
    M3D_DET_SCOPE(det);
    return bwd_weight_wino(x, nullptr, dz, B, H, W, D, Cin, Cout, OD, pz, dw, workspace, ws_bytes, s);
}

static int halo_check(const void* x_halo, int32_t has_lo, int32_t has_hi) {
    if ((has_lo | has_hi) & ~1) return einval("conv3d winograd halo: has_lo / has_hi must be 0 or 1");
    if ((has_lo || has_hi) && !x_halo) return einval("conv3d winograd halo: halo planes missing");
    return M3D_OK;
}

extern "C" int m3d_conv3d_fwd_wino_halo(const float* x, const float* x_halo, int32_t has_lo, int32_t has_hi,
                                        int64_t B, int64_t H, int64_t W, int64_t Dl, int64_t Cin,
                                        const float* w, int64_t Cout, const float* bias, const float* bn_scale,
                                        const float* bn_shift, const float* residual, int32_t relu, float* z_out,
                                        float* y, float* u_keep, void* workspace, size_t ws_bytes,
                                        m3d_stream_t s) {
    int rc = halo_check(x_halo, has_lo, has_hi);
    if (rc) return rc;
    if (u_keep && wino_nz() != wino_wgrad_nz())
        return einval("conv3d winograd: forward and weight-gradient tiles differ (m3d_conv3d_wino_u_bytes == 0)");
    return fwd_wino(x, B, H, W, Dl, Cin, w, Cout, Dl, 1, bias, bn_scale, bn_shift, residual, relu, z_out, y,
                    u_keep, workspace, ws_bytes, st(s), x_halo, has_lo, has_hi);
}

extern "C" int m3d_conv3d_fwd_wino_halo_phase(const float* x, const float* x_halo, int32_t has_lo, int32_t has_hi,
                                              int64_t B, int64_t H, int64_t W, int64_t Dl, int64_t Cin,
                                              const float* w, int64_t Cout, const float* bias, const float* bn_scale,
                                              const float* bn_shift, const float* residual, int32_t relu,
                                              float* z_out, float* y, float* u_keep, void* workspace,
                                              size_t ws_bytes, int32_t phase, m3d_stream_t s) {
    if (phase != 1 && phase != 2) return einval("conv3d winograd halo: phase must be 1 or 2");
    int rc = phase == 2 ? halo_check(x_halo, has_lo, has_hi) : M3D_OK;
    if (rc) return rc;
    if (u_keep && wino_nz() != wino_wgrad_nz())
        return einval("conv3d winograd: forward and weight-gradient tiles differ (m3d_conv3d_wino_u_bytes == 0)");
    return fwd_wino(x, B, H, W, Dl, Cin, w, Cout, Dl, 1, bias, bn_scale, bn_shift, residual, relu, z_out, y,
                    u_keep, workspace, ws_bytes, st(s), phase == 2 ? x_halo : nullptr, has_lo, has_hi, false,
                    phase);
}

extern "C" int m3d_conv3d_bwd_data_wino_halo(const float* dz, const float* w, int32_t has_lo, int32_t has_hi,
                                             int64_t B, int64_t H, int64_t W, int64_t Dl, int64_t Cin,
                                             int64_t Cout, float* dx, float* dx_halo, int32_t accumulate,
                                             void* workspace, size_t ws_bytes, m3d_stream_t s) {
    int rc = halo_check(dx_halo, has_lo, has_hi);
    if (rc) return rc;
    return bwd_data_wino(dz, w, B, H, W, Dl + has_lo + has_hi, Cin, Cout, Dl, 1 - has_lo, dx, accumulate,
                         workspace, ws_bytes, st(s), (has_lo || has_hi) ? dx_halo : nullptr, has_lo);
}

extern "C" int m3d_conv3d_bwd_weight_wino_halo(const float* x, const float* x_halo, int32_t has_lo,
                                               int32_t has_hi, const float* dz, int64_t B, int64_t H, int64_t W,
                                               int64_t Dl, int64_t Cin, int64_t Cout, float* dw, void* workspace,
                                               size_t ws_bytes, const m3d_det_t* det, m3d_stream_t s) {
    M3D_DET_SCOPE(det);
    int rc = halo_check(x_halo, has_lo, has_hi);
    if (rc) return rc;
    return bwd_weight_wino(x, nullptr, dz, B, H, W, Dl, Cin, Cout, Dl, 1, dw, workspace, ws_bytes, s, x_halo,
                           has_lo, has_hi);
}

extern "C" int m3d_conv3d_bwd_weight_wino_u(const float* u, const float* dz, int64_t B, int64_t H,
                                            int64_t W, int64_t D, int64_t Cin, int64_t Cout,
                                            int64_t OD, int32_t pz, float* dw, void* workspace,
                                            size_t ws_bytes, const m3d_det_t* det, m3d_stream_t s) {
    M3D_DET_SCOPE(det);
    if (!u) return einval("conv3d winograd: u must not be NULL");
    return bwd_weight_wino(nullptr, u, dz, B, H, W, D, Cin, Cout, OD, pz, dw, workspace, ws_bytes, s);
}
```

### 3d-mask-r-cnn_amd/m3d/_lib.py

```python
from __future__ import annotations

import ctypes
import os

import torch

_HERE = os.path.dirname(os.path.abspath(__file__))
LIB_PATH = os.path.join(_HERE, os.environ.get("M3D_LIB_FILE", "libm3d.so"))

_lib = None

c_i32 = ctypes.c_int32
c_i64 = ctypes.c_int64
c_f = ctypes.c_float
c_p = ctypes.c_void_p
c_sz = ctypes.c_size_t


class Det(ctypes.Structure):
    _fields_ = [("on", ctypes.c_int32), ("scratch", ctypes.c_void_p), ("bytes", ctypes.c_size_t)]


class BnBwd(ctypes.Structure):
    _fields_ = [("y", ctypes.c_void_p), ("z", ctypes.c_void_p), ("scale", ctypes.c_void_p),
# ... 54 lines not shown
    "m3d_conv3d_fwd_wino_v": [c_p, c_i64, c_i64, c_i64, c_i64, c_i64, c_p, c_i64, c_i64, c_i32, c_p, c_p, c_p, c_p,
                              c_i32, c_p, c_p, c_p, c_sz, c_i32, c_p],
    "m3d_conv3d_bwd_data_wino_v": [c_p, c_p, c_i64, c_i64, c_i64, c_i64, c_i64, c_i64, c_i64, c_i32, c_p, c_i32, c_p,
                                   c_sz, c_i32, c_p],
    "m3d_conv3d_bwd_data_wino_vy": [c_p, c_p, c_i64, c_i64, c_i64, c_i64, c_i64, c_i64, c_i64, c_i32, c_p, c_i32,
                                    c_p, c_sz, c_i32, c_i32, c_p],
    "m3d_conv3d_bwd_data_wino_bny": [c_p, c_p, c_i64, c_i64, c_i64, c_i64, c_i64, c_i64, c_i64, c_i32, c_p, c_i32,
                                     c_p, c_sz, c_i32, c_p, c_p, c_sz, c_i32, c_p],
    "m3d_bn_bwd_fused_workspace_bytes": [c_i64, c_i64, c_i64, c_i64, c_i64],
    "m3d_conv3d_bwd_data_bn": [c_p, c_p, c_i64, c_i64, c_i64, c_i64, c_i64, c_i32, c_i32, c_i32,
                               c_i64, c_i64, c_i64, c_i64, c_i32, c_i32, c_i32, c_i32, c_i32, c_i32,
                               c_p, c_i32, c_p, c_p, c_sz, c_p],
    "m3d_conv3d_bwd_data_wino_bn": [c_p, c_p, c_i64, c_i64, c_i64, c_i64, c_i64, c_i64, c_i64, c_i32, c_p, c_i32,
                                    c_p, c_sz, c_i32, c_p, c_p, c_sz, c_p],
    "m3d_conv3d_bwd_data_splitk_bn": [c_p, c_p, c_i64, c_i64, c_i64, c_i64, c_i64, c_i64, c_p, c_i32, c_i32,
                                      c_p, c_sz, c_p, c_p, c_sz, c_p],
    "m3d_conv3d_bwd_data": [c_p, c_p, c_i64, c_i64, c_i64, c_i64, c_i64, c_i32, c_i32, c_i32,
                            c_i64, c_i64, c_i64, c_i64, c_i32, c_i32, c_i32, c_i32, c_i32, c_i32,
                            c_p, c_i32, c_p],
    "m3d_conv3d_bwd_weight": [c_p, c_p, c_i64, c_i64, c_i64, c_i64, c_i64, c_i32, c_i32, c_i32,
                              c_i64, c_i64, c_i64, c_i64, c_i32, c_i32, c_i32, c_i32, c_i32, c_i32,
                              c_p, c_p, c_p],
    "m3d_conv3d_fwd_wino_halo": [c_p, c_p, c_i32, c_i32, c_i64, c_i64, c_i64, c_i64, c_i64, c_p, c_i64, c_p, c_p,
                                 c_p, c_p, c_i32, c_p, c_p, c_p, c_p, c_sz, c_p],
    "m3d_conv3d_fwd_wino_halo_phase": [c_p, c_p, c_i32, c_i32, c_i64, c_i64, c_i64, c_i64, c_i64, c_p, c_i64, c_p,
                                       c_p, c_p, c_p, c_i32, c_p, c_p, c_p, c_p, c_sz, c_i32, c_p],
    "m3d_conv3d_bwd_data_wino_halo": [c_p, c_p, c_i32, c_i32, c_i64, c_i64, c_i64, c_i64, c_i64, c_i64, c_p,
                                      c_p, c_i32, c_p, c_sz, c_p],
    "m3d_conv3d_bwd_weight_wino_halo": [c_p, c_p, c_i32, c_i32, c_p, c_i64, c_i64, c_i64, c_i64, c_i64, c_i64,
                                        c_p, c_p, c_sz, c_p, c_p],
    "m3d_gemm_f32": [c_p, c_p, c_p, c_i64, c_i64, c_i64, c_i64, c_p, c_i32, c_i32, c_p],
    "m3d_gemm_wgrad_f32": [c_p, c_p, c_p, c_i64, c_i64, c_i64, c_i64, c_p, c_p],
    "m3d_split3_f32": [c_p, c_i64, c_p, c_p],
    "m3d_gemm_x3": [c_p, c_p, c_p, c_i64, c_i64, c_i64, c_i64, c_p],
    "m3d_gemm_x3_af": [c_p, c_p, c_p, c_i64, c_i64, c_i64, c_i64, c_p],
    "m3d_conv3d_wino_workspace_bytes": [c_i64, c_i64, c_i64, c_i64, c_i64, c_i64, c_i64],
    "m3d_conv3d_fwd_wino": [c_p, c_i64, c_i64, c_i64, c_i64, c_i64, c_p, c_i64, c_i64, c_i32, c_p,
                            c_p, c_p, c_p, c_i32, c_p, c_p, c_p, c_sz, c_p],
    "m3d_conv3d_bwd_data_wino": [c_p, c_p, c_i64, c_i64, c_i64, c_i64, c_i64, c_i64, c_i64, c_i32,
                                 c_p, c_i32, c_p, c_sz, c_p],
    "m3d_conv3d_bwd_weight_wino": [c_p, c_p, c_i64, c_i64, c_i64, c_i64, c_i64, c_i64, c_i64,
                                   c_i32, c_p, c_p, c_sz, c_p, c_p],
    "m3d_conv3d_wino_u_bytes": [c_i64, c_i64, c_i64, c_i64, c_i64],
    "m3d_conv3d_wino_tile_z": [],
    "m3d_conv3d_wino_wgrad_tile_z": [],
    "m3d_conv3d_wino_tile_y": [],
    "m3d_conv3d_wino_dgrad_workspace_bytes": [c_i64, c_i64, c_i64, c_i64, c_i64, c_i64, c_i64, c_i32],
    "m3d_conv3d_wino_dgrad_tile_y": [],
    "m3d_conv3d_wino_dgrad_tile_z": [],
    "m3d_conv3d_fwd_wino_keep": [c_p, c_i64, c_i64, c_i64, c_i64, c_i64, c_p, c_i64, c_i64, c_i32, c_p,
                                 c_p, c_p, c_p, c_i32, c_p, c_p, c_p, c_p, c_sz, c_p],
    "m3d_conv3d_bwd_weight_wino_u": [c_p, c_p, c_i64, c_i64, c_i64, c_i64, c_i64, c_i64, c_i64,
                                     c_i32, c_p, c_p, c_sz, c_p, c_p],
    "m3d_gemm_f32_ex": [c_p, c_i64, c_i64, c_p, c_i64, c_p, c_i64, c_i64, c_i64, c_i64, c_i64, c_p,
                        c_i32, c_i32, c_p],
    "m3d_splitk_reduce": [c_p, c_i32, c_i64, c_i64, c_p, c_p, c_p, c_i32, c_p, c_p],
    "m3d_conv3d_fwd_dil": [c_p, c_i64, c_i64, c_i64, c_i64, c_i64, c_p, c_i32, c_i32, c_i32, c_i64,
                           c_i64, c_i64, c_i64, c_i32, c_i32, c_i32, c_i32, c_i32, c_i32, c_i32,
                           c_i32, c_i32, c_p, c_p, c_p, c_p, c_i32, c_i32, c_p, c_p, c_i64, c_p,
                           c_i64, c_i64, c_p],
    "m3d_deconv3d_k2s2": [c_p, c_i64, c_i64, c_i64, c_i64, c_i64, c_p, c_i64, c_p, c_i32, c_p, c_p],
    "m3d_conv3d_bwd_data_dil": [c_p, c_p, c_i64, c_i64, c_i64, c_i64, c_i64, c_i32, c_i32, c_i32,
                                c_i64, c_i64, c_i64, c_i64, c_i32, c_i32, c_i32, c_i32, c_i32, c_i32,
                                c_i32, c_i32, c_i32, c_p, c_i32, c_p],
    "m3d_conv3d_bwd_weight_dil": [c_p, c_p, c_i64, c_i64, c_i64, c_i64, c_i64, c_i32, c_i32, c_i32,
                                  c_i64, c_i64, c_i64, c_i64, c_i32, c_i32, c_i32, c_i32, c_i32, c_i32,
                                  c_i32, c_i32, c_i32, c_p, c_p, c_p],
    "m3d_deconv3d_k2s2_bwd_data": [c_p, c_p, c_i64, c_i64, c_i64, c_i64, c_i64, c_i64, c_p, c_p],
    "m3d_deconv3d_k2s2_bwd_weight": [c_p, c_p, c_i64, c_i64, c_i64, c_i64, c_i64, c_i64, c_p, c_p, c_p],
    "m3d_add_f32": [c_p, c_p, c_p, c_i64, c_p],
    "m3d_mask_out_bwd_workspace_bytes": [c_i64, c_i64, c_i32],
    "m3d_mask_out_bwd": [c_p, c_p, c_p, c_p, c_i64, c_i64, c_i32, c_p, c_p, c_p, c_p, c_p, c_sz, c_p],
    "m3d_head_outputs": [c_p, c_i64, c_i64, c_i32, c_p, c_p, c_p, c_p],
    "m3d_head_outputs_bwd": [c_p, c_p, c_p, c_i64, c_i64, c_i32, c_p, c_p],
    "m3d_max_norm": [c_p, c_i64, c_i64, c_f, c_p],
    "m3d_refine_detections": [c_p, c_p, c_p, c_i64, c_i32, c_p, c_p, c_f, c_p, c_p, c_p, c_p],
    "m3d_detections_gather": [c_p, c_p, c_p, c_p, c_i32, c_p, c_p, c_p],
    "m3d_detection_targets_workspace_bytes": [c_i64],
    "m3d_detection_targets": [c_p, c_i64, c_p, c_p, c_i64, c_i32, c_f, c_f, c_f, c_p, c_i32, ctypes.c_uint32,
                              c_p, c_p, c_p, c_p, c_p, c_p, c_p, c_p, c_sz, c_p],
    "m3d_rpn_targets_workspace_bytes": [c_i64, c_i64, c_i64],
    "m3d_rpn_targets": [c_p, c_i64, c_p, c_i64, c_f, c_f, c_i32, c_f, c_i32, c_i32, c_p, ctypes.c_uint32, c_p,
                        c_p, c_i64, c_p, c_sz, c_p, c_p],
    "m3d_rpn_targets_async": [c_p, c_i64, c_p, c_i64, c_f, c_f, c_i32, c_f, c_i32, c_i32, c_p, ctypes.c_uint32,
                              c_p, c_p, c_i64, c_p, c_sz, c_p, c_p],
    "m3d_rpn_loss_workspace_bytes": [c_i64],
    "m3d_rpn_loss_fwd": [c_p, c_p, c_p, c_p, c_p, c_i64, c_i64, c_f, c_f, c_i64, c_i64, c_f, c_f, c_p, c_p, c_p,
                         c_p, c_p, c_p, c_p, c_sz, c_p],
    "m3d_rpn_loss_bwd": [c_p, c_p, c_i64, c_p, c_p, c_p],
    "m3d_head_loss_workspace_bytes": [c_i64, c_i64],
    "m3d_head_loss_fwd": [c_p, c_p, c_p, c_p, c_p, c_p, c_p, c_i64, c_i64, c_i64, c_i64, c_f, c_f, c_f, c_f, c_f,
                          c_p, c_p, c_p, c_p, c_p, c_p, c_sz, c_p],
    "m3d_head_loss_bwd": [c_p, c_p, c_p, c_p, c_p, c_p, c_p, c_i64, c_i64, c_i64, c_i64, c_f, c_f, c_p, c_p, c_p,
                          c_p, c_p, c_p],
    "m3d_unmold_prepare": [c_p, c_p, c_i64, c_i64, c_i64, c_i64, c_i64, c_i64, c_p, c_p, c_p, c_p, c_p],
    "m3d_unmold_overlaps": [c_p, c_p, c_p, c_p, c_i64, c_i64, c_i64, c_i64, c_i64, c_p, c_i64, c_p, c_p, c_p],
    "m3d_unmold_finalize": [c_p, c_p, c_i64, c_i64, c_p, c_p, c_p, c_p, c_p],
    "m3d_unmold_paste": [c_p, c_p, c_p, c_p, c_i64, c_i64, c_i64, c_i64, c_i64, c_p, c_p, c_p],
    "m3d_mask_areas": [c_p, c_i64, c_i64, c_i64, c_i64, c_p, c_p],
    "m3d_unmold_labels": [c_p, c_p, c_p, c_p, c_p, c_i64, c_i64, c_i64, c_i64, c_i64, c_p, c_p, c_p],
    "m3d_label_pixelwise": [c_p, c_p, c_i64, c_i64, c_i64, c_i64, c_p, c_p],
    "m3d_labels_stack": [c_p, c_i64, c_i64, c_i64, c_i64, c_p, c_p],
    "m3d_normalize_image_workspace_bytes": [c_i64, c_i64, c_i64, c_i32],
    "m3d_normalize_image": [c_p, c_i32, c_i64, c_i64, c_i64, c_i32, c_p, c_p, c_p, c_sz, c_p],
    "m3d_augment_image_workspace_bytes": [c_i64, c_i64, c_i64],
    "m3d_augment_image": [c_p, c_i64, c_i64, c_i64, c_i32, c_f, ctypes.c_double, ctypes.c_uint32, ctypes.c_uint32,
                          c_p, c_p, c_sz, c_p],
    "m3d_flip_masks_u8": [c_p, c_i64, c_i64, c_i64, c_i64, c_i32, c_p, c_p],
    "m3d_flip_boxes": [c_p, c_i64, c_i64, c_i64, c_i64, c_i32, c_p, c_p],
    "m3d_maxpool3d_fwd": [c_p, c_i64, c_i64, c_i64, c_i64, c_i64, c_i32, c_i32, c_i32, c_i32,
                          c_i32, c_i32, c_i32, c_i32, c_i32, c_i64, c_i64, c_i64, c_p, c_p, c_p],
    "m3d_maxpool3d_bwd": [c_p, c_p, c_i64, c_i64, c_i64, c_i64, c_i64, c_i32, c_i32, c_i32, c_i32,
                          c_i32, c_i32, c_i32, c_i32, c_i32, c_i64, c_i64, c_i64, c_p, c_p],
    "m3d_conv3d_fwd_halo": [c_p, c_p, c_i32, c_i32, c_i32, c_i64, c_i64, c_i64, c_i64, c_i64, c_p, c_i32, c_i32,
                            c_i32, c_i64, c_i64, c_i64, c_i64, c_i32, c_i32, c_i32, c_i32, c_i32, c_i32, c_p, c_p,
                            c_p, c_i32, c_p, c_p, c_p],
    "m3d_conv3d_bwd_weight_halo": [c_p, c_p, c_i32, c_i32, c_i32, c_p, c_i64, c_i64, c_i64, c_i64, c_i64, c_i32,
                                   c_i32, c_i32, c_i64, c_i64, c_i64, c_i64, c_i32, c_i32, c_i32, c_i32, c_i32,
                                   c_i32, c_p, c_p, c_p],
    "m3d_maxpool3d_fwd_halo": [c_p, c_p, c_i32, c_i32, c_i32, c_i64, c_i64, c_i64, c_i64, c_i64, c_i32, c_i32,
                               c_i32, c_i32, c_i32, c_i32, c_i32, c_i32, c_i32, c_i64, c_i64, c_i64, c_p, c_p,
                               c_p],
    "m3d_maxpool3d_bwd_halo": [c_p, c_p, c_i32, c_i32, c_i32, c_i64, c_i64, c_i64, c_i64, c_i64, c_i32, c_i32,
                               c_i32, c_i32, c_i32, c_i32, c_i32, c_i32, c_i32, c_i64, c_i64, c_i64, c_p, c_p,
                               c_p],
    "m3d_upsample221_bwd": [c_p, c_i64, c_i64, c_i64, c_i64, c_i64, c_p, c_i32, c_p],
    "m3d_subsample221_fwd": [c_p, c_i64, c_i64, c_i64, c_i64, c_i64, c_p, c_p],
    "m3d_subsample221_bwd": [c_p, c_i64, c_i64, c_i64, c_i64, c_i64, c_p, c_p],
    "m3d_bn_affine": [c_p, c_p, c_p, c_p, c_f, c_i64, c_p, c_p, c_p, c_p],
    "m3d_bn_affine_batched": [c_p, c_i32, c_i64, c_p],
    "m3d_bn_act_bwd_workspace_bytes": [c_i64, c_i64],
    "m3d_bn_act_bwd": [c_p, c_p, c_p, c_i64, c_i64, c_i32, c_p, c_p, c_p, c_p, c_p, c_i32, c_p,
                       c_p, c_p, c_p, c_sz, c_p],
    "m3d_bn_train_few_rows_max": [],
    "m3d_bn_train_workspace_bytes": [c_i64, c_i64],
    "m3d_bn_train_fwd": [c_p, c_i64, c_i64, c_p, c_p, c_f, c_f, c_i32, c_p, c_p, c_p, c_p, c_p, c_p, c_sz, c_p],
    "m3d_bn_train_bwd": [c_p, c_p, c_p, c_i64, c_i64, c_p, c_p, c_p, c_i32, c_p, c_p, c_p, c_p, c_sz, c_p],
    "m3d_col_sums_batched_workspace_bytes": [c_p, c_i32],
    "m3d_col_sums_batched": [c_p, c_i32, c_p, c_sz, c_p],
    "m3d_sgd_keras": [c_p, c_p, c_p, c_i64, c_p, c_p, c_i32, c_f, c_f, c_f, c_p, c_p, c_p],
    "m3d_adam_keras": [c_p, c_p, c_p, c_p, c_p, c_i64, c_p, c_p, c_i32, c_f, c_f, c_f, c_f, c_f, c_p,
                       c_p, c_p],
    "m3d_adadelta_keras": [c_p, c_p, c_p, c_p, c_i64, c_p, c_p, c_i32, c_f, c_f, c_f, c_f, c_p, c_p, c_p],
    "m3d_fork_event_create": [c_i32, ctypes.POINTER(c_p)],
    "m3d_fork_event_destroy": [c_p],
    "m3d_stream_fork": [c_p, c_p, c_p],
}
_RESTYPES = {"m3d_last_error": ctypes.c_char_p, "m3d_nms3d_workspace_bytes": c_sz,
             "m3d_topk_workspace_bytes": c_sz,
             "m3d_pyramid_roi_align3d_fwd_workspace_bytes": c_sz,
             "m3d_detection_targets_workspace_bytes": c_sz, "m3d_rpn_targets_workspace_bytes": c_sz,
             "m3d_rpn_loss_workspace_bytes": c_sz, "m3d_head_loss_workspace_bytes": c_sz,
             "m3d_bn_act_bwd_workspace_bytes": c_sz, "m3d_bn_bwd_fused_workspace_bytes": c_sz, "m3d_conv3d_splitk_count": c_i32, "m3d_conv3d_wino_workspace_bytes": c_sz, "m3d_conv3d_wino_dgrad_workspace_bytes": c_sz, "m3d_conv3d_wino_v_bytes": c_sz,
             "m3d_conv3d_wino_u_bytes": c_sz, "m3d_conv3d_wino_tile_z": c_i32, "m3d_conv3d_wino_wgrad_tile_z": c_i32,
             "m3d_conv3d_wino_tile_y": c_i32, "m3d_conv3d_wino_dgrad_tile_y": c_i32,
             "m3d_conv3d_wino_dgrad_tile_z": c_i32, "m3d_col_sums_batched_workspace_bytes": c_sz,
             "m3d_bn_train_few_rows_max": c_i64, "m3d_bn_train_workspace_bytes": c_sz,
             "m3d_mask_out_bwd_workspace_bytes": c_sz, "m3d_normalize_image_workspace_bytes": c_sz,
             "m3d_augment_image_workspace_bytes": c_sz}

EXPORTED = tuple(_SIGS)


class M3DError(RuntimeError):
    pass


def load(path: str = LIB_PATH):
    global _lib
    if _lib is not None:
        return _lib
    if not os.path.exists(path):
        raise M3DError(
            f"libm3d.so not found at {path}: build it with `make -C 3d-mask-r-cnn_amd` "
            "(or __graft_entry__.build()); there is no CPU fallback")
    lib = ctypes.CDLL(path)
    for name, args in _SIGS.items():
        fn = getattr(lib, name)
        fn.argtypes = args
        fn.restype = _RESTYPES.get(name, ctypes.c_int)
    _lib = _Lib(lib)
    return _lib


DET_ENTRY_POINTS = ("m3d_conv3d_bwd_weight", "m3d_conv3d_bwd_weight_halo", "m3d_conv3d_bwd_weight_wino",
                    "m3d_conv3d_bwd_weight_wino_u", "m3d_conv3d_bwd_weight_wino_halo", "m3d_gemm_wgrad_f32",
                    "m3d_conv3d_bwd_weight_dil", "m3d_deconv3d_k2s2_bwd_weight",
                    "m3d_sgd_keras", "m3d_adam_keras", "m3d_adadelta_keras")


class BnAffineItem(ctypes.Structure):
    _fields_ = [("gamma", ctypes.c_void_p), ("beta", ctypes.c_void_p), ("mean", ctypes.c_void_p),
                ("var", ctypes.c_void_p), ("out", ctypes.c_void_p), ("eps", ctypes.c_float),
                ("C", ctypes.c_int32)]


class X3PlanesItem(ctypes.Structure):
    _fields_ = [("w", ctypes.c_void_p), ("fwd", ctypes.c_void_p), ("bwd", ctypes.c_void_p),
                ("cin", ctypes.c_int32), ("cout", ctypes.c_int32)]


class ColSumsItem(ctypes.Structure):
    _fields_ = [("x", ctypes.c_void_p), ("M", ctypes.c_int64), ("C", ctypes.c_int64), ("out", ctypes.c_void_p)]


COL_SUMS_MAX = 16


class _Lib:

    def __init__(self, cdll):
        self._cdll = cdll
        for name in _SIGS:
            setattr(self, name, getattr(cdll, name))
        for name in DET_ENTRY_POINTS:
            fn = getattr(cdll, name)
            n = len(fn.argtypes)

            def call(*args, _fn=fn, _n=n):
                if len(args) == _n - 1:
                    args = args[:-1] + (det_arg(),) + args[-1:]
                return _fn(*args)
            setattr(self, name, call)

    def __getattr__(self, name):
        return getattr(self._cdll, name)


def check(rc: int, what: str = "") -> None:
    if rc == 0:
        return
    msg = load().m3d_last_error().decode()
    if rc == -1:
        raise ValueError(msg)
    raise M3DError(f"{what}: {msg}")


def ptr(t) -> int:
    if t is None:
# ... 38 lines not shown
```

### 3d-mask-r-cnn_amd/m3d/nn.py

```python
from __future__ import annotations

import contextlib
import ctypes
import os
import weakref
from dataclasses import dataclass

import torch

from . import _lib, slab
from ._lib import check, ptr, stream


LAYER_LOG = None
LAYER_TIMING = False


RELU_CAPTURE = None


GRAD_HOOK = None


WGRAD_STREAM = True
# ... 78 lines not shown
        if side is not None:
            _fork(torch.cuda.current_stream(), side)
            with torch.cuda.stream(side):
                h[0].done(h[1])
        else:
            h[0].done(h[1])


def _span():
    if LAYER_LOG is None or not LAYER_TIMING:
        return None
    e = torch.cuda.Event(enable_timing=True)
    e.record()
    return e


def _log(kind, direct_flops, exec_flops, nbytes, phase="fwd", name="", t0=None, engine="f32"):
    if LAYER_LOG is not None:
        t1 = None
        if t0 is not None:
            t1 = torch.cuda.Event(enable_timing=True)
            t1.record()
        LAYER_LOG.append((kind, float(direct_flops), float(exec_flops), float(nbytes), phase, name, t0, t1,
                          engine))


WGRAD1_STRIDED_X3 = True


def _wgrad1_x3(geo, cin, cout, in_sp):
    return (geo.k == (1, 1, 1) and geo.stride == (1, 1, 1) and geo.pad == (0, 0, 0)
            and tuple(geo.out) == tuple(in_sp) and cin % 4 == 0 and cout >= 65)


def _wino_exec(B, OH, OW, OD, cin, cout, nz, ny=None):
    if ny is None:
        ny = int(_L().m3d_conv3d_wino_tile_y())
    tiles = B * -(-OH // ny) * -(-OW // 2) * -(-OD // nz)
    return 2.0 * (ny + 2) * 4 * (nz + 2) * tiles * cin * cout


def _L():
    return _lib.load()


SLAB_HALO_PLANES = True

SLAB_OVERLAP = True

CONV1_X3 = True
SPLITK = True
WINO_KEEP_MAX_BYTES = 8 * 2**30
SHARE_WINO_MAX_BYTES = 6 * 2**30

WINOGRAD = True
WINO_MIN_C = 64
WINO_WGRAD_MIN_C = 64


WINO_DGRAD_Y4 = "res2a_branch2b+res2b_branch2b+res2c_branch2b"


def _dgrad_tile_y(name):
    if not WINO_DGRAD_Y4:
        return 0
    return 4 if WINO_DGRAD_Y4 == "*" or name in WINO_DGRAD_Y4.split("+") else 0


def use_winograd(geo, cin, cout, in_sp):
    return (WINOGRAD and geo.k == (3, 3, 3) and geo.stride == (1, 1, 1) and geo.pad[:2] == (1, 1)
            and tuple(geo.out[:2]) == tuple(in_sp[:2]) and geo.pad[2] in (0, 1)
            and 0 <= in_sp[2] - geo.out[2] <= 2
            and cin % 32 == 0 and cout % 32 == 0 and min(cin, cout) >= WINO_MIN_C)


def _splitk(xshape, geo, cin, cout, bwd_data):
    if geo.k != (1, 1, 1) or geo.pad != (0, 0, 0) or not SPLITK:
        return 1
    B, (OH, OW, OD) = xshape[0], geo.out
    sg = slab.current()
    if sg is not None:
        OD = sg.D
    K, N = (cout, cin) if bwd_data else (cin, cout)
    return int(_L().m3d_conv3d_splitk_count(B * OH * OW * OD, K, N))


CONV1_X3_FWD_TILES = 128
CONV1_X3_DGRAD_TILES = 256
CONV1_X3_MIN_K = 32
CONV1_X3_DGRAD_MIN_K = 256
CONV1_X3_DGRAD_FUSED_MIN_K = 256


def _conv1_x3(xshape, geo, K, N, bwd_data=False, fused=False):
    if not CONV1_X3 or geo.k != (1, 1, 1) or geo.stride != (1, 1, 1) or geo.pad != (0, 0, 0):
        return False
    B, H, W, D = xshape[:4]
    kmin = (CONV1_X3_DGRAD_FUSED_MIN_K if fused else CONV1_X3_DGRAD_MIN_K) if bwd_data else CONV1_X3_MIN_K
    if tuple(geo.out) != (H, W, D) or K % 32 or N % 256 or K < kmin:
        return False
    sg = slab.current()
    Dg = sg.D if sg is not None else D
    return -(-B * H * W * Dg // 256) * (N // 256) >= (CONV1_X3_DGRAD_TILES if bwd_data else CONV1_X3_FWD_TILES)


def _check_generations(ctx):
# ... 509 lines not shown
        if rec.buf is None or dy.data_ptr() != rec.buf.data_ptr() or dy.shape != rec.buf.shape:
            raise RuntimeError(f"{ctx.name}: fused BN-ReLU backward was applied by its consumer, but the "
                               "output gradient has another contribution (the unit is not the consumer's "
                               "sole producer-consumer pair; see nn.BNFuse)")
        dres = rec.dres
        rec.clear()
        return dy, dres
    if rec is not None:
        rec.clear()
    deferred = False
    if trivial:
        dz = dy
        dres = dy if need_res else None
        if grads.get("bias") is not None:
            deferred = bias_grad(dy, M, Cout, grads["bias"], grads, ctx.bias_batch)
    else:
        dz = torch.empty_like(dy)
        dres = torch.empty_like(dy) if need_res else None
        mean, rstd, scale = ctx.bn if ctx.bn is not None else (None, None, None)
        bn_act_bwd(dy, y, z, M, Cout, ctx.relu, scale, mean, rstd, dz, dres, grads.get("beta"),
                   grads.get("gamma") if z is not None else None, grads.get("bias"))
    if LAYER_LOG is not None and not deferred:
        nel = dy.numel() * (1 + (0 if trivial else 1 + (ctx.relu or ctx.bn is not None) +
                                 (z is not None) + (dres is not None)))
        _log("bn_act_bwd", 0, 0, 4.0 * nel, "bwd_bn", ctx.name, t0)
    return dz, dres


def _wgrad_gemm(x, dz, dw, geo, halo):
    L = _L()
    dims = (*x.shape, *geo.k, dz.shape[-1], *geo.out, *geo.stride, *geo.pad)
    if halo is not None:
        check(L.m3d_conv3d_bwd_weight_halo(ptr(x), ptr(halo[0]), halo[1], halo[2], halo[0].shape[3] // 2, ptr(dz),
                                           *dims, ptr(dw), stream()), "conv3d_bwd_weight_halo")
    else:
        check(L.m3d_conv3d_bwd_weight(ptr(x), ptr(dz), *dims, ptr(dw), stream()), "conv3d_bwd_weight")


def _wino_wgrad(ctx, x, dz, w, dw, side, direct):
    L = _L()
    B, H, W, D, Cin = x.shape
    Cout, geo, halo = w.shape[-1], ctx.geo, ctx.halo
    OH, OW, OD = geo.out
    with _on_side(side):
        tw = _span()
        small = min(Cin, Cout) < WINO_WGRAD_MIN_C
        if small:
            _wgrad_gemm(x, dz, dw, geo, halo)
        else:
            dext = D + (halo[1] + halo[2] if halo is not None else 0)
            wsw, wswb = _wino_ws(B, H, W, dext, OD, Cin, Cout, x.device)
            if ctx.u is not None:
                ctx.u.record_stream(torch.cuda.current_stream())
                check(L.m3d_conv3d_bwd_weight_wino_u(ptr(ctx.u), ptr(dz), B, H, W, D, Cin, Cout, OD, geo.pad[2],
                                                     ptr(dw), ptr(wsw), wswb, stream()), "conv3d_bwd_weight_wino_u")
            elif halo is not None:
                check(L.m3d_conv3d_bwd_weight_wino_halo(ptr(x), ptr(halo[0]), halo[1], halo[2], ptr(dz), B, H, W, D,
                                                        Cin, Cout, ptr(dw), ptr(wsw), wswb, stream()),
                      "conv3d_bwd_weight_wino_halo")
            else:
                check(L.m3d_conv3d_bwd_weight_wino(ptr(x), ptr(dz), B, H, W, D, Cin, Cout, OD, geo.pad[2],
                                                   ptr(dw), ptr(wsw), wswb, stream()), "conv3d_bwd_weight_wino")
        if LAYER_LOG is not None:
            exe = direct if small else \
                _wino_exec(B, OH, OW, OD, Cin, Cout, int(L.m3d_conv3d_wino_wgrad_tile_z()))
            _log("wino_wgrad", direct, exe, 4.0 * (x.numel() + dz.numel() + w.numel()), "bwd_weight", ctx.name, tw,
                 "f32" if small else "x3")
    ctx.u = None


def _wino_dgrad(ctx, x, dz, w, direct):
    L = _L()
    B, H, W, D, Cin = x.shape
    Cout, geo, halo = w.shape[-1], ctx.geo, ctx.halo
    OH, OW, OD = geo.out
    td = _span()
    dext = D + (halo[1] + halo[2] if halo is not None else 0)
    ws, wsb = _wino_ws(B, H, W, dext, OD, Cin, Cout, x.device)
    dx, acc = _link_take(ctx.link, x)
    if dx is None:
        dx = torch.empty(x.shape, device=x.device, dtype=torch.float32)
    fused_nel = 0
    if halo is not None:
        ty = 0
        dh = torch.empty_like(halo[0])
        check(L.m3d_conv3d_bwd_data_wino_halo(ptr(dz), ptr(w), halo[1], halo[2], B, H, W, D, Cin, Cout, ptr(dx),
                                              ptr(dh), acc, ptr(ws), wsb, stream()), "conv3d_bwd_data_wino_halo")
        slab.return_halo_grads(dx, dh)
    else:
        ty = _dgrad_tile_y(ctx.name)
        vd = ctx.vd
        if vd is not None:
            if vd[2] != WINO_V.gen:
                raise RuntimeError(f"{ctx.name}: conv backward after another model forward: the "
                                   "pre-transformed Winograd weights were refreshed (run each backward "
                                   "before the next forward)")
            torch.cuda.current_stream().wait_event(vd[1])
        else:
            ws, wsb, v_ready = _shared_wino_ws(ctx.wshare, "bwd", ws, wsb, (w.data_ptr(), Cin, Cout, ty))
        args = (ptr(dz), ptr(w), B, H, W, D, Cin, Cout, OD, geo.pad[2], ptr(dx), acc, ptr(ws), wsb)
        rec = ctx.fuse_in
        if (rec is not None and rec.armed and (Cin % 256 == 0 or 256 % Cin == 0)
                and not _per_item(B, H * W * max(D, OD), max(Cin, Cout), 0, 0)
                and _fuse_final(ctx.link, x, acc)):
            if vd is not None:
                fused_nel = _fused_handoff(rec, x, dx, lambda d, bws, bwsb: check(
                    L.m3d_conv3d_bwd_data_wino_xv(*args, ptr(vd[0]), ty, d, bws, bwsb, stream()),
                    "conv3d_bwd_data_wino_xv(bn)"))
            else:
                fused_nel = _fused_handoff(rec, x, dx, lambda d, bws, bwsb: check(
                    L.m3d_conv3d_bwd_data_wino_bny(*args, v_ready, d, bws, bwsb, ty, stream()),
                    "conv3d_bwd_data_wino_bn"))
        elif vd is not None:
            check(L.m3d_conv3d_bwd_data_wino_xv(*args, ptr(vd[0]), ty, None, None, 0, stream()),
                  "conv3d_bwd_data_wino_xv")
        else:
            check(L.m3d_conv3d_bwd_data_wino_vy(*args, v_ready, ty, stream()), "conv3d_bwd_data_wino")
        _shared_wino_release(ctx.wshare)
    if LAYER_LOG is not None:
        _log("wino_dgrad", direct, _wino_exec(B, OH, OW, OD, Cin, Cout, int(L.m3d_conv3d_wino_dgrad_tile_z()),
                                              ty or int(L.m3d_conv3d_wino_dgrad_tile_y())),
             4.0 * (dz.numel() + w.numel() + x.numel() * (1 + acc) + fused_nel), "bwd_data", ctx.name, td, "x3")
    return _link_park(ctx.link, dx, acc)


def _direct_wgrad(ctx, x, dz, w, dw, side, direct):
    L = _L()
    B, H, W, D, Cin = x.shape
    Cout, geo, halo = w.shape[-1], ctx.geo, ctx.halo
    OH, OW, OD = geo.out
    nb = 4.0 * (x.numel() + dz.numel() + w.numel())
    with _on_side(side):
        tw = _span()
        if (WGRAD1_STRIDED_X3 and halo is None and geo.stride == (2, 2, 1)
                and (OH, OW, OD) == ((H + 1) // 2, (W + 1) // 2, D)):
            sub = ConvGeom(geo.k, (1, 1, 1), geo.pad, geo.out)
            if _wgrad1_x3(sub, Cin, Cout, geo.out):
                xs = torch.empty((B, OH, OW, OD, Cin), device=x.device, dtype=torch.float32)
                check(L.m3d_subsample221_fwd(ptr(x), B, H, W, D, Cin, ptr(xs), stream()), "subsample221")
                x, geo = xs, sub
        _wgrad_gemm(x, dz, dw, geo, halo)
        if LAYER_LOG is not None:
            _log(f"conv{geo.k[0]}_wgrad", direct, direct, nb, "bwd_weight", ctx.name, tw,
                 "x3" if halo is None and _wgrad1_x3(geo, Cin, Cout, x.shape[1:4]) else "f32")


def _direct_dgrad(ctx, x, dz, w, direct):
    L = _L()
    B, H, W, D, Cin = x.shape
    Cout, geo, link, rec = w.shape[-1], ctx.geo, ctx.link, ctx.fuse_in
    kh, kw, kd = geo.k
    OH, OW, OD = geo.out
    td = _span()
    fused_nel = 0
    strided = any(s != 1 for s in geo.stride)
    dx, acc = _link_take(link, x)
    if dx is None:
        dx = (torch.zeros if strided else torch.empty)(x.shape, device=x.device, dtype=torch.float32)
    wd, dzd, cpad = w, dz, Cout
    if Cout % 32:
        cpad = -(-Cout // 32) * 32
        wd = torch.zeros((kh, kw, kd, Cin, cpad), device=w.device, dtype=torch.float32)
        wd[..., :Cout] = w
        dzd = torch.zeros((B, OH, OW, OD, cpad), device=dz.device, dtype=torch.float32)
        dzd[..., :Cout] = dz
    nsk = _splitk(x.shape, geo, Cin, cpad, 1)
    x3 = cpad == Cout and not acc and _conv1_x3(x.shape, geo, Cout, Cin, bwd_data=True)
    x3_fused = (cpad == Cout and X3_BN_FUSE and rec is not None and rec.armed and not acc
                and _conv1_x3(x.shape, geo, Cout, Cin, bwd_data=True, fused=True) and _fuse_final(link, x, acc))
    if x3 or x3_fused:
# ... 380 lines not shown
```

### include/m3d.h

```cpp
#ifndef M3D_H
#define M3D_H

#include <stddef.h>
#include <stdint.h>

#ifdef __cplusplus
extern "C" {
#endif

typedef struct ihipStream_t* m3d_stream_t;

#define M3D_OK 0
#define M3D_EINVAL (-1)
#define M3D_EHIP (-2)

const char* m3d_last_error(void);
int m3d_abi_version(void);

typedef struct m3d_det {
    int32_t on;
    void* scratch;
    size_t bytes;
} m3d_det_t;

// ... 109 lines not shown
                          const float* bn_scale, const float* bn_shift, const float* residual, int32_t relu,
                          float* z_out, float* y, void* workspace, size_t ws_bytes, int32_t v_ready,
                          m3d_stream_t s);
int m3d_conv3d_bwd_data_wino_v(const float* dz, const float* w, int64_t B, int64_t H, int64_t W, int64_t D,
                               int64_t Cin, int64_t Cout, int64_t OD, int32_t pz, float* dx, int32_t accumulate,
                               void* workspace, size_t ws_bytes, int32_t v_ready, m3d_stream_t s);
int m3d_conv3d_bwd_weight(const float* x, const float* dz, int64_t B, int64_t H, int64_t W,
                          int64_t D, int64_t Cin, int32_t kh, int32_t kw, int32_t kd,
                          int64_t Cout, int64_t OH, int64_t OW, int64_t OD, int32_t sy,
                          int32_t sx, int32_t sz, int32_t py, int32_t px, int32_t pz, float* dw,
                          const m3d_det_t* det, m3d_stream_t s);
int m3d_conv3d_fwd_halo(const float* x, const float* halo, int32_t has_lo, int32_t has_hi, int32_t r,
                        int64_t B, int64_t H, int64_t W, int64_t Dl, int64_t Cin, const float* w,
                        int32_t kh, int32_t kw, int32_t kd, int64_t Cout, int64_t OH, int64_t OW, int64_t OD,
                        int32_t sy, int32_t sx, int32_t sz, int32_t py, int32_t px, int32_t pz,
                        const float* bias, const float* bn_scale, const float* bn_shift, int32_t relu,
                        float* z_out, float* y, m3d_stream_t s);
int m3d_conv3d_bwd_weight_halo(const float* x, const float* halo, int32_t has_lo, int32_t has_hi, int32_t r,
                               const float* dz, int64_t B, int64_t H, int64_t W, int64_t Dl, int64_t Cin,
                               int32_t kh, int32_t kw, int32_t kd, int64_t Cout, int64_t OH, int64_t OW,
                               int64_t OD, int32_t sy, int32_t sx, int32_t sz, int32_t py, int32_t px,
                               int32_t pz, float* dw, const m3d_det_t* det, m3d_stream_t s);

size_t m3d_conv3d_wino_workspace_bytes(int64_t B, int64_t H, int64_t W, int64_t D, int64_t OD,
                                       int64_t Cin, int64_t Cout);
int m3d_conv3d_fwd_wino(const float* x, int64_t B, int64_t H, int64_t W, int64_t D, int64_t Cin,
                        const float* w, int64_t Cout, int64_t OD, int32_t pz, const float* bias,
                        const float* bn_scale, const float* bn_shift, const float* residual,
                        int32_t relu, float* z_out, float* y, void* workspace, size_t ws_bytes,
                        m3d_stream_t s);
int m3d_conv3d_bwd_data_wino(const float* dz, const float* w, int64_t B, int64_t H, int64_t W,
                             int64_t D, int64_t Cin, int64_t Cout, int64_t OD, int32_t pz,
                             float* dx, int32_t accumulate, void* workspace, size_t ws_bytes,
                             m3d_stream_t s);
int m3d_conv3d_bwd_weight_wino(const float* x, const float* dz, int64_t B, int64_t H, int64_t W,
                               int64_t D, int64_t Cin, int64_t Cout, int64_t OD, int32_t pz,
                               float* dw, void* workspace, size_t ws_bytes, const m3d_det_t* det, m3d_stream_t s);
int32_t m3d_conv3d_wino_tile_z(void);
int32_t m3d_conv3d_wino_wgrad_tile_z(void);
int32_t m3d_conv3d_wino_tile_y(void);
int32_t m3d_conv3d_wino_dgrad_tile_y(void);
int32_t m3d_conv3d_wino_dgrad_tile_z(void);
size_t m3d_conv3d_wino_dgrad_workspace_bytes(int64_t B, int64_t H, int64_t W, int64_t D, int64_t OD,
                                             int64_t Cin, int64_t Cout, int32_t tile_y);
size_t m3d_conv3d_wino_u_bytes(int64_t B, int64_t H, int64_t W, int64_t OD, int64_t Cin);
int m3d_conv3d_fwd_wino_keep(const float* x, int64_t B, int64_t H, int64_t W, int64_t D, int64_t Cin,
                             const float* w, int64_t Cout, int64_t OD, int32_t pz, const float* bias,
                             const float* bn_scale, const float* bn_shift, const float* residual,
                             int32_t relu, float* z_out, float* y, float* u_keep, void* workspace,
                             size_t ws_bytes, m3d_stream_t s);
int m3d_conv3d_bwd_weight_wino_u(const float* u, const float* dz, int64_t B, int64_t H, int64_t W,
                                 int64_t D, int64_t Cin, int64_t Cout, int64_t OD, int32_t pz,
                                 float* dw, void* workspace, size_t ws_bytes, const m3d_det_t* det, m3d_stream_t s);
int m3d_conv3d_fwd_wino_halo(const float* x, const float* x_halo, int32_t has_lo, int32_t has_hi, int64_t B,
                             int64_t H, int64_t W, int64_t Dl, int64_t Cin, const float* w, int64_t Cout,
                             const float* bias, const float* bn_scale, const float* bn_shift,
                             const float* residual, int32_t relu, float* z_out, float* y, float* u_keep,
                             void* workspace, size_t ws_bytes, m3d_stream_t s);
int m3d_conv3d_fwd_wino_halo_phase(const float* x, const float* x_halo, int32_t has_lo, int32_t has_hi,
                                   int64_t B, int64_t H, int64_t W, int64_t Dl, int64_t Cin, const float* w,
                                   int64_t Cout, const float* bias, const float* bn_scale, const float* bn_shift,
                                   const float* residual, int32_t relu, float* z_out, float* y, float* u_keep,
                                   void* workspace, size_t ws_bytes, int32_t phase, m3d_stream_t s);
int m3d_conv3d_bwd_data_wino_halo(const float* dz, const float* w, int32_t has_lo, int32_t has_hi, int64_t B,
                                  int64_t H, int64_t W, int64_t Dl, int64_t Cin, int64_t Cout, float* dx,
                                  float* dx_halo, int32_t accumulate, void* workspace, size_t ws_bytes,
                                  m3d_stream_t s);
int m3d_conv3d_bwd_weight_wino_halo(const float* x, const float* x_halo, int32_t has_lo, int32_t has_hi,
                                    const float* dz, int64_t B, int64_t H, int64_t W, int64_t Dl, int64_t Cin,
                                    int64_t Cout, float* dw, void* workspace, size_t ws_bytes, const m3d_det_t* det, m3d_stream_t s);

typedef struct m3d_bn_bwd {
    const float* y;
    const float* z;
    const float* scale;
    const float* mean;
    const float* rstd;
    int32_t relu;
    float* dres;
    float* sum_dpre;
    float* sum_dpre_xhat;
    float* sum_dz;
} m3d_bn_bwd_t;
size_t m3d_bn_bwd_fused_workspace_bytes(int64_t B, int64_t H, int64_t W, int64_t D, int64_t C);
int m3d_conv3d_bwd_data_bn(const float* dz, const float* w, int64_t B, int64_t H, int64_t W, int64_t D,
                           int64_t Cin, int32_t kh, int32_t kw, int32_t kd, int64_t Cout, int64_t OH,
                           int64_t OW, int64_t OD, int32_t sy, int32_t sx, int32_t sz, int32_t py,
                           int32_t px, int32_t pz, float* dx, int32_t accumulate, const m3d_bn_bwd_t* bn,
                           void* workspace, size_t ws_bytes, m3d_stream_t s);
int m3d_conv3d_bwd_data_wino_bn(const float* dz, const float* w, int64_t B, int64_t H, int64_t W, int64_t D,
                                int64_t Cin, int64_t Cout, int64_t OD, int32_t pz, float* dx, int32_t accumulate,
                                void* workspace, size_t ws_bytes, int32_t v_ready, const m3d_bn_bwd_t* bn,
                                void* bn_ws, size_t bn_ws_bytes, m3d_stream_t s);
int m3d_conv3d_bwd_data_wino_vy(const float* dz, const float* w, int64_t B, int64_t H, int64_t W, int64_t D,
                                int64_t Cin, int64_t Cout, int64_t OD, int32_t pz, float* dx, int32_t accumulate,
                                void* workspace, size_t ws_bytes, int32_t v_ready, int32_t tile_y, m3d_stream_t s);
int m3d_conv3d_bwd_data_wino_bny(const float* dz, const float* w, int64_t B, int64_t H, int64_t W, int64_t D,
                                 int64_t Cin, int64_t Cout, int64_t OD, int32_t pz, float* dx, int32_t accumulate,
                                 void* workspace, size_t ws_bytes, int32_t v_ready, const m3d_bn_bwd_t* bn, void* bn_ws,
                                 size_t bn_ws_bytes, int32_t tile_y, m3d_stream_t s);
size_t m3d_conv3d_wino_v_bytes(int64_t Cin, int64_t Cout, int32_t dgrad, int32_t tile_y);
int m3d_conv3d_wino_weight_v(const float* w, int64_t Cin, int64_t Cout, int32_t dgrad, int32_t tile_y, void* v,
                             size_t v_bytes, m3d_stream_t s);
int m3d_conv3d_fwd_wino_kv(const float* x, int64_t B, int64_t H, int64_t W, int64_t D, int64_t Cin, const float* w,
                           int64_t Cout, int64_t OD, int32_t pz, const float* bias, const float* bn_scale,
                           const float* bn_shift, const float* residual, int32_t relu, float* z_out, float* y,
// ... 248 lines not shown
```

Before: 42.90 volumes/s.

## Add row-sparse gradient path for Winograd conv backward with device-side gating

Adds a row-sparsity scheme for conv3d backward. A probe kernel samples dz rows to see whether the gradient is mostly zero. If it is, only the active rows are compacted and processed through a sparse path, and device-side gate and mlim flags let the dense Winograd and GEMM kernels exit early, so the choice can be made inside a HIP graph without a host sync. The ROWSPARSE flag defaults to 0 (auto), so a probe and flag pass run on large layers, and the extra workspace header and early-exit checks add overhead when gradients are dense.

After: 46.32 volumes/s, median of 6. 1.08x the previous value.

```diff
diff --git a/3d-mask-r-cnn_amd/csrc/conv3d.hip b/3d-mask-r-cnn_amd/csrc/conv3d.hip
--- a/3d-mask-r-cnn_amd/csrc/conv3d.hip
+++ b/3d-mask-r-cnn_amd/csrc/conv3d.hip
@@ -767,6 +767,7 @@
     int64_t pstride;
     int plain;
     int store;
+    const int* gate;
 };
 
 __device__ __forceinline__ void wg_put(const WgOut& o, float* C, float* P, int64_t idx, float v) {
@@ -778,7 +779,8 @@
 
 __global__ __launch_bounds__(256) void wg_reduce_kernel(const float* __restrict__ part, int splits,
                                                         int64_t pstride, int64_t kn, int64_t bsc,
-                                                        float* __restrict__ C) {
+                                                        float* __restrict__ C, const int* gate) {
+    if (gate && *gate) return;
     const int64_t i = (int64_t)blockIdx.x * 256 + threadIdx.x;
     if (i >= pstride) return;
     float s = part[i];
@@ -808,7 +810,7 @@
                       float* C, hipStream_t s) {
     if (!o.part) return;
     hipLaunchKernelGGL(wg_reduce_kernel, dim3(grid_for(o.pstride, 256)), dim3(256), 0, s, o.part, (int)splits,
-                       o.pstride, K * N, nbatch > 1 ? bsc : K * N, C);
+                       o.pstride, K * N, nbatch > 1 ? bsc : K * N, C, o.gate);
 }
 
 static hipError_t wg_settle(WgOut& o, int64_t splits, bool fresh, float* C, int64_t nbatch, int64_t K, int64_t N,
@@ -1116,6 +1118,7 @@
                                                             float* __restrict__ C, int64_t M, int K, int N,
                                                             int64_t m_per_split, int64_t bsa, int64_t bsb,
                                                             int64_t bsc, WgOut wo) {
+    if (wo.gate && *wo.gate) return;
     constexpr int BI = 128, BJ = 128, TI = 2, TJ = 2, BKM = 32;
     constexpr int PL = 128 * BKM * 2;
     __shared__ __attribute__((aligned(16))) char smem[6 * PL];
@@ -1226,6 +1229,7 @@
                                                               float* __restrict__ C, int64_t M, int K, int N,
                                                               int64_t m_per_split, int64_t bsa, int64_t bsb,
                                                               int64_t bsc, WgOut wo) {
+    if (wo.gate && *wo.gate) return;
     constexpr int TI = 2, TJ = 2, BKM = 64;
     constexpr int SUB = 64 * 64;
     constexpr int PL = 2 * SUB;
@@ -1482,6 +1486,7 @@
                                                              int N, int64_t m_per_split, int64_t bsa,
                                                              int64_t bsb, int64_t bsc, WgOut wo, X3wSK sk) {
     __shared__ __attribute__((aligned(16))) char smem[2 * W2_STAGE];
+    if (wo.gate && *wo.gate) return;
     if constexpr (SK) {
         const int64_t G = gridDim.x, L = blockIdx.x;
         const int64_t xcd = L % 8, q8 = G / 8, r8 = G % 8;
@@ -1526,7 +1531,7 @@
 }
 
 static int launch_wgrad_tr(const float* A, const float* Bm, float* C, int64_t M, int K, int N, int nbatch,
-                           int64_t bsa, int64_t bsb, int64_t bsc, hipStream_t s, bool fresh) {
+                           int64_t bsa, int64_t bsb, int64_t bsc, hipStream_t s, bool fresh, const int* gate) {
     const int64_t tiles = (int64_t)((K + 255) / 256) * ((N + 255) / 256) * nbatch;
     const int64_t cus = num_cus();
     static constexpr int64_t minm = M3D_TUNE_X3W_TR_MINM;
@@ -1542,6 +1547,7 @@
         G = G / sk.tn * sk.tn;
         if (G < sk.tn) G = sk.tn;
         WgOut wo{nullptr, 0, 0, 0};
+        wo.gate = gate;
         const hipError_t fe = wg_settle(wo, 2, fresh, C, nbatch, K, N, s);
         if (fe != hipSuccess) return (int)fe;
         hipLaunchKernelGGL((x3_wgrad_tr_kernel<0, true>), dim3((unsigned)G), dim3(512), 0, s, A, Bm, C, M, K, N,
@@ -1553,6 +1559,7 @@
     if (splits > max_splits) splits = max_splits;
     if (splits < 1) splits = 1;
     WgOut wo = wg_out(splits, nbatch, K, N);
+    wo.gate = gate;
     int64_t mper = (M + splits - 1) / splits;
     mper = (mper + W2_BK - 1) / W2_BK * W2_BK;
     splits = (M + mper - 1) / mper;
@@ -1568,9 +1575,10 @@
 static int wgrad_x3_env() { return (x3_mask() >> 2) & 1; }
 
 static int launch_wgrad_x3(const float* A, const float* Bm, float* C, int64_t M, int K, int N, int nbatch,
-                           int64_t bsa, int64_t bsb, int64_t bsc, hipStream_t s, bool fresh = false) {
+                           int64_t bsa, int64_t bsb, int64_t bsc, hipStream_t s, bool fresh = false,
+                           const int* gate = nullptr) {
     if (wgrad_tr_env() && K >= 192 && N >= 192)
-        return launch_wgrad_tr(A, Bm, C, M, K, N, nbatch, bsa, bsb, bsc, s, fresh);
+        return launch_wgrad_tr(A, Bm, C, M, K, N, nbatch, bsa, bsb, bsc, s, fresh, gate);
     if (K <= 64 || N <= 64) {
         const int64_t tiles = (int64_t)((K + 63) / 64) * ((N + 63) / 64);
         int64_t splits = (1024 + tiles * nbatch - 1) / (tiles * nbatch);
@@ -1579,6 +1587,7 @@
         if (splits > max_splits) splits = max_splits;
         if (splits < 1) splits = 1;
         WgOut wo = wg_out(splits, nbatch, K, N);
+        wo.gate = gate;
         int64_t mper = (M + splits - 1) / splits;
         mper = (mper + 63) / 64 * 64;
         splits = (M + mper - 1) / mper;
@@ -1596,6 +1605,7 @@
     if (splits > max_splits) splits = max_splits;
     if (splits < 1) splits = 1;
     WgOut wo = wg_out(splits, nbatch, K, N);
+    wo.gate = gate;
     int64_t mper = (M + splits - 1) / splits;
     mper = (mper + 31) / 32 * 32;
     splits = (M + mper - 1) / mper;
@@ -1614,6 +1624,7 @@
     int hlo, hhi;
     int tz_mode;
     int xcd;
+    const int* gate;
 };
 
 __device__ __forceinline__ int64_t wino_block(const WinoGeom& g) {
@@ -1722,6 +1733,7 @@
 __global__ __launch_bounds__(256) void wino_input_kernel(const float* __restrict__ x, WinoGeom g,
                                                          int C, float* __restrict__ U) {
     constexpr int P = ZT<NZ>::P, PYt = ZT<NYT>::P;
+    if (g.gate && *g.gate) return;
     const int64_t i = wino_block(g) * blockDim.x + threadIdx.x;
     if (i >= g.T * C) return;
     const int c = (int)(i % C);
@@ -1906,6 +1918,7 @@
 template <int NZ, int NYT = WNY>
 __global__ __launch_bounds__(256) void wino_output_kernel(const float* __restrict__ Mt, WinoGeom g,
                                                           int N, Epi e) {
+    if (g.gate && *g.gate) return;
     wino_output_body<NZ, false, NYT>(Mt, g, N, e);
 }
 template <int NZ, int NYT = WNY>
@@ -2110,6 +2123,7 @@
 __global__ __launch_bounds__(256) void wino_grad_kernel(const float* __restrict__ dz, WinoGeom g,
                                                         int N, float* __restrict__ DY) {
     constexpr int P = ZT<NZ>::P;
+    if (g.gate && *g.gate) return;
     const int64_t i = (int64_t)blockIdx.x * blockDim.x + threadIdx.x;
     if (i >= g.T * N) return;
     const int n = (int)(i % N);
@@ -2160,8 +2174,10 @@
 
 template <int NZ>
 __global__ __launch_bounds__(256) void wino_wgrad_out_kernel(const float* __restrict__ dWh, int C,
-                                                             int N, float* __restrict__ dw) {
+                                                             int N, float* __restrict__ dw,
+                                                             const int* gate) {
     constexpr int P = ZT<NZ>::P;
+    if (gate && *gate) return;
     const int64_t i = (int64_t)blockIdx.x * blockDim.x + threadIdx.x;
     const int64_t CN = (int64_t)C * N;
     if (i >= CN) return;
@@ -2230,6 +2246,8 @@
     int64_t psa = 0, psb = 0;
     int64_t bsa = 0, bsb = 0, bsc = 0;
     X3Epi ep = {};
+    const int* gate = nullptr;
+    const int* mlim = nullptr;
 };
 
 __device__ __forceinline__ int x3_off16(int row, int kc) {
@@ -2262,6 +2280,7 @@
     int64_t L = PERSIST ? (int64_t)blockIdx.x : (int64_t)blockIdx.x + (int64_t)gridDim.x * blockIdx.y;
     const int64_t Lstep = PERSIST ? (int64_t)gridDim.x : total;
     const int nk = g.K / BK;
+    if (g.gate && *g.gate) return;
     float* const Ts = reinterpret_cast<float*>(smem);
     int soff[CPT];
     uint32_t lrow[CPT];
@@ -2276,6 +2295,7 @@
         const int64_t bz = T / per_batch, Tt = T - bz * per_batch;
         const int64_t m0 = (Tt / nby) * BM;
         const int n0 = (int)(Tt % nby) * BN;
+        if (g.mlim && m0 >= *g.mlim) continue;
         __amdgpu_buffer_rsrc_t ra[3], rb[3];
 #pragma unroll
         for (int pl = 0; pl < 3; ++pl) {
@@ -2423,11 +2443,13 @@
     const int64_t per_batch = nbx * nby, total = per_batch * g.nbatch;
     const int64_t L = (int64_t)blockIdx.x + (int64_t)gridDim.x * blockIdx.y;
     if (L >= total) return;
+    if (g.gate && *g.gate) return;
     const int64_t xcd = L % 8, q8 = total / 8, r8 = total % 8;
     const int64_t T = (xcd < r8 ? xcd * (q8 + 1) : r8 * (q8 + 1) + (xcd - r8) * q8) + L / 8;
     const int64_t bz = T / per_batch, Tt = T - bz * per_batch;
     const int64_t m0 = (Tt / nby) * 256;
     const int64_t n0 = (Tt % nby) * 256;
+    if (g.mlim && m0 >= *g.mlim) return;
     __amdgpu_buffer_rsrc_t rs[6];
 #pragma unroll
     for (int pl = 0; pl < 3; ++pl) {
@@ -2538,11 +2560,13 @@
     const int64_t per_batch = nbx * nby, total = per_batch * g.nbatch;
     const int64_t L = (int64_t)blockIdx.x + (int64_t)gridDim.x * blockIdx.y;
     if (L >= total) return;
+    if (g.gate && *g.gate) return;
     const int64_t xcd = L % 8, q8 = total / 8, r8 = total % 8;
     const int64_t T = (xcd < r8 ? xcd * (q8 + 1) : r8 * (q8 + 1) + (xcd - r8) * q8) + L / 8;
     const int64_t bz = T / per_batch, Tt = T - bz * per_batch;
     const int64_t m0 = (Tt / nby) * 256;
     const int64_t n0 = (Tt % nby) * 256;
+    if (g.mlim && m0 >= *g.mlim) return;
     const int nk = g.K / G2_BK;
     const __amdgpu_buffer_rsrc_t ra = make_rsrc(g.af + bz * g.bsa + m0 * g.K, (uint64_t)(g.M - m0) * g.K * 4);
     const int arow = tid >> 1, ach = tid & 1;
@@ -3754,6 +3778,8 @@
 extern "C" int32_t m3d_conv3d_wino_dgrad_tile_y(void) { return wino_dgrad_ny(); }
 extern "C" int32_t m3d_conv3d_wino_dgrad_tile_z(void) { return wino_dgrad_nz(); }
 
+static size_t rs_hdr_bytes(int64_t rows);
+
 extern "C" size_t m3d_conv3d_wino_workspace_bytes(int64_t B, int64_t H, int64_t W, int64_t D,
                                                   int64_t OD, int64_t Cin, int64_t Cout) {
     auto al = [](size_t b) { return (b + 255) & ~(size_t)255; };
@@ -3771,16 +3797,19 @@
         const size_t b = wt + al(eb * P * (size_t)Cin * Cout) + (um1 > um2 ? um1 : um2);
         best = b > best ? b : best;
     }
-    return best;
+    return best + rs_hdr_bytes(B * H * W * (D > OD ? D : OD));
 }
 
 struct WinoWs { float *V, *U, *M, *WT; };
-static size_t wino_ws_need(const WinoGeom& g, int64_t C1, int64_t C2, int nz, int ny) {
+static size_t wino_ws_layout(const WinoGeom& g, int64_t C1, int64_t C2, int nz, int ny) {
     auto al = [](size_t b) { return (b + 255) & ~(size_t)255; };
     const size_t P = (size_t)wino_points(nz, ny);
     const size_t eb = gemm_x3_env() ? 6 : 4;
     const size_t wt = gemm_x3_env() ? al(sizeof(float) * 27 * (size_t)C1 * C2) : 0;
     return wt + al(eb * P * (size_t)C1 * C2) + al(eb * P * (size_t)g.T * C1) + al(4 * P * (size_t)g.T * C2);
+}
+static size_t wino_ws_need(const WinoGeom& g, int64_t C1, int64_t C2, int nz, int ny) {
+    return wino_ws_layout(g, C1, C2, nz, ny) + rs_hdr_bytes((int64_t)g.B * g.H * g.W * (g.D > g.Din ? g.D : g.Din));
 }
 extern "C" size_t m3d_conv3d_wino_dgrad_workspace_bytes(int64_t B, int64_t H, int64_t W, int64_t D, int64_t OD,
                                                         int64_t Cin, int64_t Cout, int32_t tile_y) {
@@ -3827,8 +3856,9 @@
 static int x3_af32_env() { return (x3_mask() >> 4) & 1; }
 
 static void wino_gemm_x3(const WinoWs& ws, int64_t T, int K, int N, int P, hipStream_t s,
-                         bool af32 = false) {
+                         bool af32 = false, const int* gate = nullptr, const int* mlim = nullptr) {
     X3G q{};
+    q.gate = gate; q.mlim = mlim;
     q.a = reinterpret_cast<const unsigned short*>(ws.U);
     q.af = ws.U;
     q.b = reinterpret_cast<const unsigned short*>(ws.V);
@@ -4167,7 +4197,7 @@
                          int64_t Cin, int64_t Cout, int64_t OD, int32_t pz, float* dx, int32_t accumulate,
                          void* workspace, size_t ws_bytes, hipStream_t s, float* dx_halo = nullptr,
                          int hlo = 0, bool v_ready = false, const Epi* fb = nullptr, int ny = 0,
-                         const void* v_ext = nullptr);
+                         const void* v_ext = nullptr, int rs_mode = 0);
 
 extern "C" int m3d_conv3d_fwd_wino_v(const float* x, int64_t B, int64_t H, int64_t W, int64_t D, int64_t Cin,
                                      const float* w, int64_t Cout, int64_t OD, int32_t pz, const float* bias,
@@ -4316,6 +4346,340 @@
                          false, nullptr, ny, v);
 }
 
+constexpr int RS_CAP_MAX = 4096;
+constexpr int RS_CAP_DIV = 32;
+constexpr int RS_PROBE_ROWS = 256;
+constexpr int RS_PROBE_DIV = 8;
+constexpr int RS_BLK = 64;
+constexpr double RS_MIN_FLOP = 9e11;
+enum { RS_STATE = 0, RS_SKIP_DENSE = 1, RS_SKIP_SPARSE = 2, RS_N = 3, RS_PROBE = 4, RS_HDR_INTS = 64 };
+enum { RS_UNDECIDED = 0, RS_DENSE = 1, RS_SPARSE = 2 };
+
+enum { RS_AUTO = 0, RS_OFF = 1, RS_ALWAYS = 2 };
+
+static size_t rs_al(size_t b) { return (b + 255) & ~(size_t)255; }
+static size_t rs_hdr_bytes(int64_t rows) {
+    return rs_al(sizeof(int) * (RS_HDR_INTS + RS_CAP_MAX)) + rs_al(sizeof(int) * (size_t)((rows + RS_BLK - 1) / RS_BLK)) +
+           rs_al(sizeof(int) * (size_t)rows);
+}
+struct RsHdr { int *h, *idx, *blk, *slot; };
+static RsHdr rs_hdr(void* base, int64_t rows) {
+    RsHdr r{};
+    char* p = static_cast<char*>(base);
+    r.h = reinterpret_cast<int*>(p);
+    r.idx = r.h + RS_HDR_INTS;
+    p += rs_al(sizeof(int) * (RS_HDR_INTS + RS_CAP_MAX));
+    r.blk = reinterpret_cast<int*>(p);
+    p += rs_al(sizeof(int) * (size_t)((rows + RS_BLK - 1) / RS_BLK));
+    r.slot = reinterpret_cast<int*>(p);
+    return r;
+}
+static int rs_cap(int64_t rows) {
+    const int64_t c = rows / RS_CAP_DIV;
+    return (int)(c > RS_CAP_MAX ? RS_CAP_MAX : c);
+}
+static bool rs_attempt(int mode, int64_t rows, int64_t Cin, int64_t Cout) {
+    if (mode == RS_OFF || !gemm_x3_env() || !wgrad_x3_env()) return false;
+    if (rs_cap(rows) < 1 || rows > 0x7FFFFFFF) return false;
+    return mode == RS_ALWAYS || 2.0 * 27.0 * (double)rows * (double)Cin * (double)Cout >= RS_MIN_FLOP;
+}
+
+__device__ __forceinline__ bool rs_lane_active(const float* __restrict__ row, int C, int lane) {
+    bool a = false;
+    for (int c = lane * 4; c < C; c += 256) {
+        const float4 v = *reinterpret_cast<const float4*>(row + c);
+        a |= (v.x != 0.0f) | (v.y != 0.0f) | (v.z != 0.0f) | (v.w != 0.0f);
+    }
+    return a;
+}
+
+__global__ __launch_bounds__(1024) void rs_probe_kernel(const float* __restrict__ dz, int64_t rows, int C,
+                                                        int* __restrict__ h) {
+    __shared__ int cnt[16];
+    const int lane = threadIdx.x & 63, wave = threadIdx.x >> 6;
+    const int ns = rows < RS_PROBE_ROWS ? (int)rows : RS_PROBE_ROWS;
+    unsigned m = 0;
+#pragma unroll
+    for (int k = 0; k < RS_PROBE_ROWS / 16; ++k) {
+        const int i = wave * (RS_PROBE_ROWS / 16) + k;
+        bool a = false;
+        if (i < ns) a = rs_lane_active(dz + (((int64_t)i * rows / ns + (int64_t)i * 37) % rows) * C, C, lane);
+        m |= (a ? 1u : 0u) << k;
+    }
+    int c = 0;
+#pragma unroll
+    for (int k = 0; k < RS_PROBE_ROWS / 16; ++k) c += __ballot((m >> k) & 1u) != 0ull ? 1 : 0;
+    if (lane == 0) cnt[wave] = c;
+    __syncthreads();
+    if (threadIdx.x == 0) {
+        int a = 0;
+        for (int w = 0; w < 16; ++w) a += cnt[w];
+        const bool dense = a * RS_PROBE_DIV > ns;
+        h[RS_PROBE] = dense ? 1 : 0;
+        h[RS_STATE] = dense ? RS_DENSE : RS_UNDECIDED;
+        h[RS_SKIP_DENSE] = 0;
+        h[RS_SKIP_SPARSE] = 1;
+        h[RS_N] = 0;
+    }
+}
+
+__global__ __launch_bounds__(256) void rs_flag_kernel(const float* __restrict__ dz, int64_t rows, int C,
+                                                      const int* __restrict__ h, int* __restrict__ blk,
+                                                      int* __restrict__ slot) {
+    if (h[RS_PROBE]) return;
+    __shared__ int cnt[4];
+    const int lane = threadIdx.x & 63, wave = threadIdx.x >> 6;
+    const int64_t r0 = (int64_t)blockIdx.x * RS_BLK + wave * 16;
+    unsigned m = 0;
+#pragma unroll
+    for (int k = 0; k < 16; ++k) {
+        bool a = false;
+        if (r0 + k < rows) a = rs_lane_active(dz + (r0 + k) * C, C, lane);
+        m |= (a ? 1u : 0u) << k;
+    }
+    int c = 0;
+#pragma unroll
+    for (int k = 0; k < 16; ++k) {
+        const int act = __ballot((m >> k) & 1u) != 0ull ? 1 : 0;
+        if (lane == 0 && r0 + k < rows) slot[r0 + k] = act;
+        c += act;
+    }
+    if (lane == 0) cnt[wave] = c;
+    __syncthreads();
+    if (threadIdx.x == 0) blk[blockIdx.x] = cnt[0] + cnt[1] + cnt[2] + cnt[3];
+}
+
+struct RsPack {
+    const float* dz = nullptr;
+    int64_t rows = 0;
+    int C = 0, cap = 0;
+    int* h = nullptr;
+    const int* blk = nullptr;
+    int* slot = nullptr;
+    int* idx = nullptr;
+    float* dzc = nullptr;
+    const float* x = nullptr;
+    float* xg = nullptr;
+    int H = 0, W = 0, D = 0, OD = 0, pz = 0, Cx = 0;
+    const float* w = nullptr;
+    unsigned short* wp = nullptr;
+    int64_t nw = 0;
+    unsigned nb_idx = 0, nb_zero = 0;
+};
+constexpr int RS_SPLIT_PER = 2048;
+
+__device__ __forceinline__ void rs_copy_row(const float* __restrict__ s, float* __restrict__ d, int C, int lane,
+                                            bool on) {
+    for (int c = lane * 4; c < C; c += 256) {
+        float4 v = make_float4(0.0f, 0.0f, 0.0f, 0.0f);
+        if (on) v = *reinterpret_cast<const float4*>(s + c);
+        *reinterpret_cast<float4*>(d + c) = v;
+    }
+}
+
+__global__ __launch_bounds__(256) void rs_pack_kernel(RsPack p) {
+    if (p.h[RS_PROBE]) return;
+    __shared__ int red[2][4];
+    const int tid = threadIdx.x, lane = tid & 63, wave = tid >> 6;
+    const int64_t nblk = (p.rows + RS_BLK - 1) / RS_BLK;
+    const bool ib = blockIdx.x < p.nb_idx;
+    const int64_t g0 = ib ? (int64_t)blockIdx.x * 4 : 0;
+    int tot = 0, pre = 0;
+    for (int64_t i = tid; i < nblk; i += 256) {
+        const int c = p.blk[i];
+        tot += c;
+        if (i < g0) pre += c;
+    }
+#pragma unroll
+    for (int o = 32; o; o >>= 1) {
+        tot += __shfl_xor(tot, o);
+        pre += __shfl_xor(pre, o);
+    }
+    if (lane == 0) { red[0][wave] = tot; red[1][wave] = pre; }
+    __syncthreads();
+    const int n = red[0][0] + red[0][1] + red[0][2] + red[0][3];
+    const bool sparse = n <= p.cap;
+    if (blockIdx.x == 0 && tid == 0) {
+        p.h[RS_STATE] = sparse ? RS_SPARSE : RS_DENSE;
+        p.h[RS_SKIP_DENSE] = sparse ? 1 : 0;
+        p.h[RS_SKIP_SPARSE] = sparse ? 0 : 1;
+        p.h[RS_N] = sparse ? n : 0;
+    }
+    if (!sparse) return;
+    if (ib) {
+        const int64_t g = g0 + wave;
+        if (g >= nblk) return;
+        int base = red[1][0] + red[1][1] + red[1][2] + red[1][3];
+        for (int q = 0; q < wave; ++q) base += p.blk[g0 + q];
+        const int64_t r = g * RS_BLK + lane;
+        const bool act = r < p.rows && p.slot[r] != 0;
+        unsigned long long m = __ballot(act);
+        const int s = base + __popcll(m & ((1ull << lane) - 1ull));
+        if (r < p.rows) p.slot[r] = act ? s : -1;
+        if (act) p.idx[s] = (int)r;
+        for (int k = 0; m; ++k) {
+            const int j = __ffsll(m) - 1;
+            m &= m - 1;
+            const int64_t row = g * RS_BLK + j;
+            const int sk = base + k;
+            if (!p.dzc) break;
+            rs_copy_row(p.dz + row * p.C, p.dzc + (int64_t)sk * p.C, p.C, lane, true);
+            if (!p.xg) continue;
+            int64_t t = row;
+            const int zo = (int)(t % p.OD); t /= p.OD;
+            const int xo = (int)(t % p.W); t /= p.W;
+            const int yo = (int)(t % p.H);
+            const int64_t b = t / p.H;
+            for (int c = lane * 4; c < p.Cx; c += 256) {
+                float4 v[27];
+#pragma unroll
+                for (int tap = 0; tap < 27; ++tap) {
+                    const int yi = yo + tap / 9 - 1, xi = xo + (tap / 3) % 3 - 1, zi = zo + tap % 3 - p.pz;
+                    const bool in = (unsigned)yi < (unsigned)p.H && (unsigned)xi < (unsigned)p.W &&
+                                    (unsigned)zi < (unsigned)p.D;
+                    v[tap] = make_float4(0.0f, 0.0f, 0.0f, 0.0f);
+                    if (in)
+                        v[tap] = *reinterpret_cast<const float4*>(
+                            p.x + (((b * p.H + yi) * p.W + xi) * p.D + zi) * p.Cx + c);
+                }
+#pragma unroll
+                for (int tap = 0; tap < 27; ++tap)
+                    *reinterpret_cast<float4*>(p.xg + ((int64_t)tap * p.cap + sk) * p.Cx + c) = v[tap];
+            }
+        }
+        return;
+    }
+    const unsigned bz = blockIdx.x - p.nb_idx;
+    if (bz < p.nb_zero) {
+        const int r = (int)bz * 4 + wave;
+        if (r < n || r >= p.cap) return;
+        rs_copy_row(p.dz, p.dzc + (int64_t)r * p.C, p.C, lane, false);
+        if (p.xg)
+            for (int tap = 0; tap < 27; ++tap)
+                rs_copy_row(p.x, p.xg + ((int64_t)tap * p.cap + r) * p.Cx, p.Cx, lane, false);
+        return;
+    }
+    const int64_t i0 = (int64_t)(bz - p.nb_zero) * RS_SPLIT_PER + tid;
+#pragma unroll
+    for (int k = 0; k < RS_SPLIT_PER / 256; ++k) {
+        const int64_t i = i0 + k * 256;
+        if (i >= p.nw) break;
+        uint32_t hi, mi, lo;
+        split3(p.w[i], hi, mi, lo);
+        p.wp[i] = (unsigned short)hi;
+        p.wp[p.nw + i] = (unsigned short)mi;
+        p.wp[2 * p.nw + i] = (unsigned short)lo;
+    }
+}
+
+static void rs_scan(const float* dz, int64_t rows, int C, int cap, const RsHdr& hd, RsPack q, hipStream_t s) {
+    const int64_t nblk = (rows + RS_BLK - 1) / RS_BLK;
+    q.dz = dz; q.rows = rows; q.C = C; q.cap = cap;
+    q.h = hd.h; q.blk = hd.blk; q.slot = hd.slot; q.idx = hd.idx;
+    q.nb_idx = (unsigned)((nblk + 3) / 4);
+    q.nb_zero = q.dzc ? (unsigned)((cap + 3) / 4) : 0;
+    const unsigned nb_split = (unsigned)((q.nw + RS_SPLIT_PER - 1) / RS_SPLIT_PER);
+    hipLaunchKernelGGL(rs_probe_kernel, dim3(1), dim3(1024), 0, s, dz, rows, C, hd.h);
+    hipLaunchKernelGGL(rs_flag_kernel, dim3((unsigned)nblk), dim3(256), 0, s, dz, rows, C, hd.h, hd.blk, hd.slot);
+    hipLaunchKernelGGL(rs_pack_kernel, dim3(q.nb_idx + q.nb_zero + nb_split), dim3(256), 0, s, q);
+}
+
+extern "C" size_t m3d_conv3d_rowsparse_scan_bytes(int64_t rows) { return rows > 0 ? rs_hdr_bytes(rows) : 0; }
+extern "C" int m3d_conv3d_rowsparse_scan(const float* dz, int64_t rows, int64_t C, int32_t cap, void* ws,
+                                         size_t ws_bytes, m3d_stream_t s) {
+    if (rows <= 0 || rows > 0x7FFFFFFF || C <= 0 || C % 4) return einval("rowsparse_scan: rows > 0 and C a positive multiple of 4");
+    if (cap < 0 || cap > RS_CAP_MAX) return einval("rowsparse_scan: cap must be in [0, 4096]");
+    if (!dz || !ws || ws_bytes < rs_hdr_bytes(rows)) return einval("rowsparse_scan: workspace missing or too small");
+    rs_scan(dz, rows, (int)C, cap, rs_hdr(ws, rows), RsPack{}, st(s));
+    return check_launch("rowsparse_scan");
+}
+
+constexpr int RS_VOX = 8;
+__global__ __launch_bounds__(256) void rs_dgrad_out_kernel(const float* __restrict__ ct, int64_t nvox, int H, int W,
+                                                           int D, int OD, int pz, int C, int accumulate,
+                                                           const int* __restrict__ h,
+                                                           const int* __restrict__ slot, float* __restrict__ dx) {
+    if (h[RS_SKIP_SPARSE]) return;
+    __shared__ int ss[RS_VOX * 27];
+    __shared__ int hit[RS_VOX];
+    const int tid = threadIdx.x;
+    const int64_t v0 = (int64_t)blockIdx.x * RS_VOX;
+    if (tid < RS_VOX) hit[tid] = 0;
+    __syncthreads();
+    if (tid < RS_VOX * 27) {
+        const int j = tid / 27, tap = tid % 27, ky = tap / 9, kx = (tap / 3) % 3, kz = tap % 3;
+        int sl = -1;
+        int64_t t = v0 + j;
+        if (t < nvox) {
+            const int z = (int)(t % D); t /= D;
+            const int xx = (int)(t % W); t /= W;
+            const int y = (int)(t % H);
+            const int64_t b = t / H;
+            const int yo = y - ky + 1, xo = xx - kx + 1, zo = z - kz + pz;
+            if ((unsigned)yo < (unsigned)H && (unsigned)xo < (unsigned)W && (unsigned)zo < (unsigned)OD)
+                sl = slot[((b * H + yo) * W + xo) * OD + zo];
+        }
+        ss[tid] = sl;
+        if (sl >= 0) hit[j] = 1;
+    }
+    __syncthreads();
+    const int L = C / 4;
+    for (int q = tid; q < RS_VOX * L; q += 256) {
+        const int j = q / L, c = (q % L) * 4;
+        if (v0 + j >= nvox) break;
+        float* o = dx + (v0 + j) * C + c;
+        if (!hit[j]) {
+            if (!accumulate) *reinterpret_cast<float4*>(o) = make_float4(0.0f, 0.0f, 0.0f, 0.0f);
+            continue;
+        }
+        float4 a = make_float4(0.0f, 0.0f, 0.0f, 0.0f);
+        if (accumulate) a = *reinterpret_cast<const float4*>(o);
+        for (int tap = 0; tap < 27; ++tap) {
+            const int sl = ss[j * 27 + tap];
+            if (sl < 0) continue;
+            const float4 v = *reinterpret_cast<const float4*>(ct + ((int64_t)sl * 27 + tap) * C + c);
+            a.x += v.x; a.y += v.y; a.z += v.z; a.w += v.w;
+        }
+        *reinterpret_cast<float4*>(o) = a;
+    }
+}
+
+static size_t rs_dgrad_bytes(int cap, int64_t Cin, int64_t Cout) {
+    return rs_al(4 * (size_t)cap * Cout) + rs_al(6 * 27 * (size_t)Cin * Cout) + rs_al(4 * (size_t)cap * 27 * Cin);
+}
+static size_t rs_wgrad_bytes(int cap, int64_t Cin, int64_t Cout) {
+    return rs_al(4 * (size_t)cap * Cout) + rs_al(4 * 27 * (size_t)cap * Cin);
+}
+
+static void rs_dgrad_launch(const float* dz, const float* w, int64_t B, int H, int W, int D, int OD, int pz, int Cin,
+                            int Cout, float* dx, int accumulate, char* um, int cap, const RsHdr& hd, hipStream_t s) {
+    float* dzc = reinterpret_cast<float*>(um);
+    unsigned short* wp = reinterpret_cast<unsigned short*>(um + rs_al(4 * (size_t)cap * Cout));
+    float* ct = reinterpret_cast<float*>(um + rs_al(4 * (size_t)cap * Cout) + rs_al(6 * 27 * (size_t)Cin * Cout));
+    RsPack q{};
+    q.dzc = dzc; q.w = w; q.wp = wp; q.nw = (int64_t)27 * Cin * Cout;
+    rs_scan(dz, B * H * W * OD, Cout, cap, hd, q, s);
+    WinoWs g{};
+    g.U = dzc;
+    g.V = reinterpret_cast<float*>(wp);
+    g.M = ct;
+    wino_gemm_x3(g, cap, Cout, 27 * Cin, 1, s, true, hd.h + RS_SKIP_SPARSE, hd.h + RS_N);
+    const int64_t nvox = B * H * W * D;
+    hipLaunchKernelGGL(rs_dgrad_out_kernel, dim3((unsigned)((nvox + RS_VOX - 1) / RS_VOX)), dim3(256), 0, s, ct, nvox,
+                       H, W, D, OD, pz, Cin, accumulate, hd.h, hd.slot, dx);
+}
+
+extern "C" int m3d_conv3d_bwd_data_wino_rs(const float* dz, const float* w, int64_t B, int64_t H, int64_t W,
+                                           int64_t D, int64_t Cin, int64_t Cout, int64_t OD, int32_t pz, float* dx,
+                                           int32_t accumulate, void* workspace, size_t ws_bytes, int32_t v_ready,
+                                           int32_t tile_y, const void* v, int32_t rs_mode, m3d_stream_t s) {
+    int ny;
+    if (int rc = v ? wino_v_tile(1, tile_y, ny) : dgrad_tile_arg(tile_y, ny)) return rc;
+    if (rs_mode < RS_AUTO || rs_mode > RS_ALWAYS) return einval("conv3d winograd bwd-data: rs_mode must be 0, 1 or 2");
+    return bwd_data_wino(dz, w, B, H, W, D, Cin, Cout, OD, pz, dx, accumulate, workspace, ws_bytes, st(s), nullptr, 0,
+                         v_ready != 0, nullptr, ny, v, rs_mode);
+}
+
 template <int NZ, int NY>
 static void wino_dgrad_out(const float* Mt, const WinoGeom& g, int C, float* dx, int accumulate,
                            float* dx_halo, int hlo, int dl, hipStream_t hs, const Epi* fb) {
@@ -4349,7 +4713,7 @@
             hipLaunchKernelGGL((wino_input_kernel<NZ, false, false, NY>), igrid, dim3(256), 0, hs, dz, g, Cout, ws.U);
         else
             hipLaunchKernelGGL((wino_input_kernel<NZ, true, false, NY>), igrid, dim3(256), 0, hs, dz, g, Cout, ws.U);
-        wino_gemm_x3(ws, g.T, Cout, Cin, P, hs, af32);
+        wino_gemm_x3(ws, g.T, Cout, Cin, P, hs, af32, g.gate);
     } else {
         hipLaunchKernelGGL((wino_weight_kernel<NZ, false, NY>), wgrid, dim3(256), 0, hs, w, Cin, Cout, 1, ws.V);
         hipLaunchKernelGGL((wino_input_kernel<NZ, false, false, NY>), igrid, dim3(256), 0, hs, dz, g, Cout, ws.U);
@@ -4365,7 +4729,7 @@
 static int bwd_data_wino(const float* dz, const float* w, int64_t B, int64_t H, int64_t W, int64_t D,
                          int64_t Cin, int64_t Cout, int64_t OD, int32_t pz, float* dx, int32_t accumulate,
                          void* workspace, size_t ws_bytes, hipStream_t hs, float* dx_halo, int hlo, bool v_ready,
-                         const Epi* fb, int ny_arg, const void* v_ext) {
+                         const Epi* fb, int ny_arg, const void* v_ext, int rs_mode) {
     int rc = wino_check(B, H, W, D, OD, pz, Cin, Cout);
     if (rc) return rc;
     if (wino_per_item(B, H, W, D, OD, Cin, Cout)) {
@@ -4374,21 +4738,33 @@
             rc = bwd_data_wino(dz + b * H * W * OD * Cout, w, 1, H, W, D, Cin, Cout, OD, pz, dx + b * H * W * dxd * Cin,
                                accumulate, workspace, ws_bytes, hs,
                                dx_halo ? dx_halo + b * H * W * 2 * Cin : nullptr, hlo, v_ready || b > 0, nullptr,
-                               ny_arg, v_ext);
+                               ny_arg, v_ext, RS_OFF);
             if (rc) return rc;
         }
         return M3D_OK;
     }
     const int nz = wino_dgrad_nz(), ny = ny_arg ? ny_arg : wino_dgrad_ny();
-    const WinoGeom g = wino_geom(B, H, W, D, OD, 2 - pz, nz, ny);
+    WinoGeom g = wino_geom(B, H, W, D, OD, 2 - pz, nz, ny);
     if (ws_bytes < wino_ws_need(g, Cout, Cin, nz, ny))
         return einval("conv3d winograd: workspace too small");
     WinoWs ws = wino_ws(workspace, g, Cout, Cin, nz, ny);
+    float* const ws_u = ws.U;
     if (v_ext) {
         ws.V = static_cast<float*>(const_cast<void*>(v_ext));
         v_ready = true;
     }
     const int ci = (int)Cin, co = (int)Cout, dl = (int)OD;
+    const int64_t rows = B * H * W * OD;
+    const int cap = rs_cap(rows);
+    const size_t lay = wino_ws_layout(g, Cout, Cin, nz, ny);
+    const size_t um = lay - (size_t)(reinterpret_cast<char*>(ws_u) - static_cast<char*>(workspace));
+    if (!dx_halo && !fb && rs_attempt(rs_mode, rows, Cin, Cout) && rs_dgrad_bytes(cap, Cin, Cout) <= um &&
+        (int64_t)cap * 27 * Cin * 4 < 0xFFFFFFF0LL && 27 * Cin * Cout * 2 < 0xFFFFFFF0LL) {
+        const RsHdr hd = rs_hdr(static_cast<char*>(workspace) + lay, rows);
+        g.gate = hd.h + RS_SKIP_DENSE;
+        rs_dgrad_launch(dz, w, B, (int)H, (int)W, (int)D, (int)OD, pz, ci, co, dx, accumulate,
+                        reinterpret_cast<char*>(ws_u), cap, hd, hs);
+    }
     if (nz == 4 && ny == 4)
         bwd_data_wino_launch<4, 4>(dz, w, g, ws, ci, co, dx, accumulate, dx_halo, hlo, dl, v_ready, fb, hs);
     else if (nz == 4)
@@ -4403,7 +4779,7 @@
 static int bwd_weight_wino(const float* x, const float* u_in, const float* dz, int64_t B,
                            int64_t H, int64_t W, int64_t D, int64_t Cin, int64_t Cout, int64_t OD,
                            int32_t pz, float* dw, void* workspace, size_t ws_bytes, m3d_stream_t s,
-                           const float* halo = nullptr, int hlo = 0, int hhi = 0) {
+                           const float* halo = nullptr, int hlo = 0, int hhi = 0, int rs_mode = 0) {
     int rc = wino_check(B, H, W, D, OD, pz, Cin, Cout);
     if (rc) return rc;
     if (ws_bytes < m3d_conv3d_wino_workspace_bytes(B, H, W, D, OD, Cin, Cout))
@@ -4413,7 +4789,7 @@
         for (int64_t b = 0; b < B; ++b) {
             rc = bwd_weight_wino(x + b * H * W * D * Cin, nullptr, dz + b * H * W * OD * Cout, 1, H, W, D, Cin, Cout,
                                  OD, pz, dw, workspace, ws_bytes, s, halo ? halo + b * H * W * 2 * Cin : nullptr, hlo,
-                                 hhi);
+                                 hhi, RS_OFF);
             if (rc) return rc;
         }
         return M3D_OK;
@@ -4422,6 +4798,24 @@
     WinoGeom g = wino_geom(B, H, W, OD, D, pz, nz);
     g.halo = halo; g.hlo = hlo; g.hhi = hhi;
     WinoWs ws = wino_ws(workspace, g, Cin, Cout, nz);
+    const int* gate = nullptr;
+    const int64_t rows = B * H * W * OD;
+    const int cap = rs_cap(rows);
+    const size_t lay = wino_ws_layout(g, Cin, Cout, nz, WNY);
+    const size_t um = lay - (size_t)(reinterpret_cast<char*>(ws.U) - static_cast<char*>(workspace));
+    if (x && !halo && wgrad_x3_env() && (Cout > 64 || Cin <= 64) && rs_attempt(rs_mode, rows, Cin, Cout) &&
+        rs_wgrad_bytes(cap, Cin, Cout) <= um) {
+        const RsHdr hd = rs_hdr(static_cast<char*>(workspace) + lay, rows);
+        gate = g.gate = hd.h + RS_SKIP_DENSE;
+        float* dzc = ws.U;
+        float* xg = reinterpret_cast<float*>(reinterpret_cast<char*>(ws.U) + rs_al(4 * (size_t)cap * Cout));
+        RsPack q{};
+        q.dzc = dzc; q.x = x; q.xg = xg;
+        q.H = (int)H; q.W = (int)W; q.D = (int)D; q.OD = (int)OD; q.pz = pz; q.Cx = (int)Cin;
+        rs_scan(dz, rows, (int)Cout, cap, hd, q, st(s));
+        launch_wgrad_x3(xg, dzc, dw, cap, (int)Cin, (int)Cout, 27, (int64_t)cap * Cin, 0, (int64_t)Cin * Cout, st(s),
+                        false, hd.h + RS_SKIP_SPARSE);
+    }
     if (u_in)
         ws.U = const_cast<float*>(u_in);
     else
@@ -4431,7 +4825,7 @@
     int fe = 0;
     if (wgrad_x3_env() && (Cout > 64 || Cin <= 64)) {
         fe = launch_wgrad_x3(ws.U, ws.M, ws.V, g.T, (int)Cin, (int)Cout, wino_points(nz), g.T * Cin, g.T * Cout,
-                             (int64_t)Cin * Cout, st(s), true);
+                             (int64_t)Cin * Cout, st(s), true, gate);
     } else {
         ConvP p = wino_gemm_p(ws.U, g.T, (int)Cin, nullptr, (int)Cout);
         p.bsw = g.T * Cout;
@@ -4444,7 +4838,7 @@
         return M3D_EHIP;
     }
     WINO_LAUNCH_NZ(nz, wino_wgrad_out_kernel, dim3(grid_for(Cin * Cout, 256)), dim3(256), 0, st(s),
-                       ws.V, (int)Cin, (int)Cout, dw);
+                       ws.V, (int)Cin, (int)Cout, dw, gate);
     return check_launch("conv3d winograd bwd-weight");
 }
 
@@ -4521,3 +4915,27 @@
     if (!u) return einval("conv3d winograd: u must not be NULL");
     return bwd_weight_wino(nullptr, u, dz, B, H, W, D, Cin, Cout, OD, pz, dw, workspace, ws_bytes, s);
 }
+
+extern "C" size_t m3d_conv3d_rowsparse_header_offset(int64_t B, int64_t H, int64_t W, int64_t D, int64_t OD,
+                                                     int32_t pz, int64_t Cin, int64_t Cout, int32_t pass,
+                                                     int32_t tile_y) {
+    if (wino_check(B, H, W, D, OD, pz, Cin, Cout) || wino_per_item(B, H, W, D, OD, Cin, Cout)) return (size_t)-1;
+    if (pass == 1) {
+        const int nz = wino_wgrad_nz();
+        return wino_ws_layout(wino_geom(B, H, W, OD, D, pz, nz), Cin, Cout, nz, WNY);
+    }
+    if (pass != 0 || (tile_y != 0 && tile_y != 2 && tile_y != 4)) return (size_t)-1;
+    const int nz = wino_dgrad_nz(), ny = tile_y ? tile_y : wino_dgrad_ny();
+    return wino_ws_layout(wino_geom(B, H, W, D, OD, 2 - pz, nz, ny), Cout, Cin, nz, ny);
+}
+
+extern "C" int m3d_conv3d_bwd_weight_wino_ux(const float* u, const float* x, const float* dz, int64_t B, int64_t H,
+                                             int64_t W, int64_t D, int64_t Cin, int64_t Cout, int64_t OD,
+                                             int32_t pz, float* dw, void* workspace, size_t ws_bytes,
+                                             int32_t rs_mode, const m3d_det_t* det, m3d_stream_t s) {
+    M3D_DET_SCOPE(det);
+    if (!x) return einval("conv3d winograd: x must not be NULL");
+    if (rs_mode < RS_AUTO || rs_mode > RS_ALWAYS) return einval("conv3d winograd bwd-weight: rs_mode must be 0, 1 or 2");
+    return bwd_weight_wino(x, u, dz, B, H, W, D, Cin, Cout, OD, pz, dw, workspace, ws_bytes, s, nullptr, 0, 0,
+                           rs_mode);
+}
diff --git a/3d-mask-r-cnn_amd/m3d/_lib.py b/3d-mask-r-cnn_amd/m3d/_lib.py
--- a/3d-mask-r-cnn_amd/m3d/_lib.py
+++ b/3d-mask-r-cnn_amd/m3d/_lib.py
@@ -130,6 +130,13 @@
                                  c_p, c_p, c_p, c_i32, c_p, c_p, c_p, c_p, c_sz, c_p],
     "m3d_conv3d_bwd_weight_wino_u": [c_p, c_p, c_i64, c_i64, c_i64, c_i64, c_i64, c_i64, c_i64,
                                      c_i32, c_p, c_p, c_sz, c_p, c_p],
+    "m3d_conv3d_bwd_weight_wino_ux": [c_p, c_p, c_p, c_i64, c_i64, c_i64, c_i64, c_i64, c_i64, c_i64,
+                                      c_i32, c_p, c_p, c_sz, c_i32, c_p, c_p],
+    "m3d_conv3d_bwd_data_wino_rs": [c_p, c_p, c_i64, c_i64, c_i64, c_i64, c_i64, c_i64, c_i64, c_i32,
+                                    c_p, c_i32, c_p, c_sz, c_i32, c_i32, c_p, c_i32, c_p],
+    "m3d_conv3d_rowsparse_scan_bytes": [c_i64],
+    "m3d_conv3d_rowsparse_header_offset": [c_i64, c_i64, c_i64, c_i64, c_i64, c_i32, c_i64, c_i64, c_i32, c_i32],
+    "m3d_conv3d_rowsparse_scan": [c_p, c_i64, c_i64, c_i32, c_p, c_sz, c_p],
     "m3d_gemm_f32_ex": [c_p, c_i64, c_i64, c_p, c_i64, c_p, c_i64, c_i64, c_i64, c_i64, c_i64, c_p,
                         c_i32, c_i32, c_p],
     "m3d_splitk_reduce": [c_p, c_i32, c_i64, c_i64, c_p, c_p, c_p, c_i32, c_p, c_p],
@@ -230,6 +237,7 @@
              "m3d_detection_targets_workspace_bytes": c_sz, "m3d_rpn_targets_workspace_bytes": c_sz,
              "m3d_rpn_loss_workspace_bytes": c_sz, "m3d_head_loss_workspace_bytes": c_sz,
              "m3d_bn_act_bwd_workspace_bytes": c_sz, "m3d_bn_bwd_fused_workspace_bytes": c_sz, "m3d_conv3d_splitk_count": c_i32, "m3d_conv3d_wino_workspace_bytes": c_sz, "m3d_conv3d_wino_dgrad_workspace_bytes": c_sz, "m3d_conv3d_wino_v_bytes": c_sz,
+             "m3d_conv3d_rowsparse_scan_bytes": c_sz, "m3d_conv3d_rowsparse_header_offset": c_sz,
              "m3d_conv3d_wino_u_bytes": c_sz, "m3d_conv3d_wino_tile_z": c_i32, "m3d_conv3d_wino_wgrad_tile_z": c_i32,
              "m3d_conv3d_wino_tile_y": c_i32, "m3d_conv3d_wino_dgrad_tile_y": c_i32,
              "m3d_conv3d_wino_dgrad_tile_z": c_i32, "m3d_col_sums_batched_workspace_bytes": c_sz,
@@ -262,7 +270,7 @@
 
 
 DET_ENTRY_POINTS = ("m3d_conv3d_bwd_weight", "m3d_conv3d_bwd_weight_halo", "m3d_conv3d_bwd_weight_wino",
-                    "m3d_conv3d_bwd_weight_wino_u", "m3d_conv3d_bwd_weight_wino_halo", "m3d_gemm_wgrad_f32",
+                    "m3d_conv3d_bwd_weight_wino_u", "m3d_conv3d_bwd_weight_wino_ux", "m3d_conv3d_bwd_weight_wino_halo", "m3d_gemm_wgrad_f32",
                     "m3d_conv3d_bwd_weight_dil", "m3d_deconv3d_k2s2_bwd_weight",
                     "m3d_sgd_keras", "m3d_adam_keras", "m3d_adadelta_keras")
 
diff --git a/3d-mask-r-cnn_amd/m3d/nn.py b/3d-mask-r-cnn_amd/m3d/nn.py
--- a/3d-mask-r-cnn_amd/m3d/nn.py
+++ b/3d-mask-r-cnn_amd/m3d/nn.py
@@ -154,6 +154,8 @@
 SPLITK = True
 WINO_KEEP_MAX_BYTES = 8 * 2**30
 SHARE_WINO_MAX_BYTES = 6 * 2**30
+
+ROWSPARSE = 0
 
 WINOGRAD = True
 WINO_MIN_C = 64
@@ -769,15 +771,22 @@
             wsw, wswb = _wino_ws(B, H, W, dext, OD, Cin, Cout, x.device)
             if ctx.u is not None:
                 ctx.u.record_stream(torch.cuda.current_stream())
-                check(L.m3d_conv3d_bwd_weight_wino_u(ptr(ctx.u), ptr(dz), B, H, W, D, Cin, Cout, OD, geo.pad[2],
-                                                     ptr(dw), ptr(wsw), wswb, stream()), "conv3d_bwd_weight_wino_u")
+                if halo is None:
+                    check(L.m3d_conv3d_bwd_weight_wino_ux(ptr(ctx.u), ptr(x), ptr(dz), B, H, W, D, Cin, Cout, OD,
+                                                          geo.pad[2], ptr(dw), ptr(wsw), wswb, ROWSPARSE, stream()),
+                          "conv3d_bwd_weight_wino_u")
+                else:
+                    check(L.m3d_conv3d_bwd_weight_wino_u(ptr(ctx.u), ptr(dz), B, H, W, D, Cin, Cout, OD,
+                                                         geo.pad[2], ptr(dw), ptr(wsw), wswb, stream()),
+                          "conv3d_bwd_weight_wino_u")
             elif halo is not None:
                 check(L.m3d_conv3d_bwd_weight_wino_halo(ptr(x), ptr(halo[0]), halo[1], halo[2], ptr(dz), B, H, W, D,
                                                         Cin, Cout, ptr(dw), ptr(wsw), wswb, stream()),
                       "conv3d_bwd_weight_wino_halo")
             else:
-                check(L.m3d_conv3d_bwd_weight_wino(ptr(x), ptr(dz), B, H, W, D, Cin, Cout, OD, geo.pad[2],
-                                                   ptr(dw), ptr(wsw), wswb, stream()), "conv3d_bwd_weight_wino")
+                check(L.m3d_conv3d_bwd_weight_wino_ux(None, ptr(x), ptr(dz), B, H, W, D, Cin, Cout, OD, geo.pad[2],
+                                                      ptr(dw), ptr(wsw), wswb, ROWSPARSE, stream()),
+                      "conv3d_bwd_weight_wino")
         if LAYER_LOG is not None:
             exe = direct if small else \
                 _wino_exec(B, OH, OW, OD, Cin, Cout, int(L.m3d_conv3d_wino_wgrad_tile_z()))
@@ -829,10 +838,11 @@
                     L.m3d_conv3d_bwd_data_wino_bny(*args, v_ready, d, bws, bwsb, ty, stream()),
                     "conv3d_bwd_data_wino_bn"))
         elif vd is not None:
-            check(L.m3d_conv3d_bwd_data_wino_xv(*args, ptr(vd[0]), ty, None, None, 0, stream()),
+            check(L.m3d_conv3d_bwd_data_wino_rs(*args, 0, ty, ptr(vd[0]), ROWSPARSE, stream()),
                   "conv3d_bwd_data_wino_xv")
         else:
-            check(L.m3d_conv3d_bwd_data_wino_vy(*args, v_ready, ty, stream()), "conv3d_bwd_data_wino")
+            check(L.m3d_conv3d_bwd_data_wino_rs(*args, v_ready, ty, None, ROWSPARSE, stream()),
+                  "conv3d_bwd_data_wino")
         _shared_wino_release(ctx.wshare)
     if LAYER_LOG is not None:
         _log("wino_dgrad", direct, _wino_exec(B, OH, OW, OD, Cin, Cout, int(L.m3d_conv3d_wino_dgrad_tile_z()),
diff --git a/include/m3d.h b/include/m3d.h
--- a/include/m3d.h
+++ b/include/m3d.h
@@ -185,6 +185,19 @@
 int m3d_conv3d_bwd_weight_wino_u(const float* u, const float* dz, int64_t B, int64_t H, int64_t W,
                                  int64_t D, int64_t Cin, int64_t Cout, int64_t OD, int32_t pz,
                                  float* dw, void* workspace, size_t ws_bytes, const m3d_det_t* det, m3d_stream_t s);
+int m3d_conv3d_bwd_weight_wino_ux(const float* u, const float* x, const float* dz, int64_t B, int64_t H,
+                                  int64_t W, int64_t D, int64_t Cin, int64_t Cout, int64_t OD, int32_t pz,
+                                  float* dw, void* workspace, size_t ws_bytes, int32_t rs_mode,
+                                  const m3d_det_t* det, m3d_stream_t s);
+int m3d_conv3d_bwd_data_wino_rs(const float* dz, const float* w, int64_t B, int64_t H, int64_t W, int64_t D,
+                                int64_t Cin, int64_t Cout, int64_t OD, int32_t pz, float* dx, int32_t accumulate,
+                                void* workspace, size_t ws_bytes, int32_t v_ready, int32_t tile_y, const void* v,
+                                int32_t rs_mode, m3d_stream_t s);
+size_t m3d_conv3d_rowsparse_scan_bytes(int64_t rows);
+size_t m3d_conv3d_rowsparse_header_offset(int64_t B, int64_t H, int64_t W, int64_t D, int64_t OD, int32_t pz,
+                                          int64_t Cin, int64_t Cout, int32_t pass, int32_t tile_y);
+int m3d_conv3d_rowsparse_scan(const float* dz, int64_t rows, int64_t C, int32_t cap, void* ws, size_t ws_bytes,
+                              m3d_stream_t s);
 int m3d_conv3d_fwd_wino_halo(const float* x, const float* x_halo, int32_t has_lo, int32_t has_hi, int64_t B,
                              int64_t H, int64_t W, int64_t Dl, int64_t Cin, const float* w, int64_t Cout,
                              const float* bias, const float* bn_scale, const float* bn_shift,
```
